# jrectorb/decagon

Measured on AMD Instinct MI355X. Metric: GCN-layer edges/sec + achieved HBM GB/s, 5-relation synthetic, 1/2/4/8 GPU, higher is better.
Workload: dtype f32; 1 GPU; S: main.py 5-relation / 10-matrix synthetic (reference-normalised, 105,974 nnz per relation set), 2 GCN layers d=64/32 + DEDICOM decoder B=512+512; nnz_per_layer_total=105974, parallelism=1 GPU, hipgraph=True, launch=one hipGraph per 30 steps, steps_per_graph=30

## Files before the change

decagon_amd/_lib.py:

```python
from __future__ import annotations

import ctypes
import threading
from pathlib import Path
from ctypes import POINTER, c_float, c_int32, c_int64, c_uint64, c_void_p

from . import _build
from .tuning import knob

DG_OK = 0
DG_EINVAL = -1
DG_EALIGN = -2
DG_ETOOMANY = -3
DG_MAX_GROUPS = 8
DG_STAGED_MAX_CHUNKS = 128
DG_EPI_L2NORM = 1
DG_EPI_RELU = 2
DG_EPI_CHUNK_RELU = 4
ABI_VERSION = 39
DG_HINGE_WS_BYTES = 16 + 4 * 256
DG_RANK_LOGIT, DG_RANK_SIGMOID64, DG_RANK_SIGMOID32 = 0, 1, 2
DG_TOPK_MAX_K, DG_TOPK_UPPER, DG_TOPK_NO_DIAG = 1024, 1, 2
DG_GROUP_SHARED_PATTERN = 1
DG_GROUP_DROPOUT = 2
# ... 35 lines not shown
    _fields_ = [
        ("pairs", c_void_p),
        ("jm", c_void_p),
        ("jmoff", c_void_p),
        ("slab", c_void_p),
        ("x", c_void_p),
        ("out", c_void_p),
        ("x_ld", c_int64),
        ("n_rows", c_int32),
        ("n_cols", c_int32),
        ("n_rels", c_int32),
        ("out_chunk", c_int32),
        ("x_rows", c_int32),
        ("jm_len", c_int32),
        ("chunk_start", c_void_p),
        ("n_chunks", c_int32),
        ("pad", c_int32),
    ]


class DgSegGroup(ctypes.Structure):
    _fields_ = [
        ("rowptr", c_void_p),
        ("seg", c_void_p),
        ("vcol", c_void_p),
        ("val", c_void_p),
        ("slab", c_void_p),
        ("x", c_void_p),
        ("w", c_void_p),
        ("out", c_void_p),
        ("x_ld", c_int64),
        ("n_rows", c_int32),
        ("n_cols", c_int32),
        ("n_chunks", c_int32),
        ("chunk", c_int32),
        ("n_rels", c_int32),
        ("x_rows", c_int32),
    ]


class DgTabDesc(ctypes.Structure):
    _fields_ = [("x", c_void_p), ("w", c_void_p), ("orow", c_void_p), ("cnt", c_int32), ("x_ld", c_int32),
                ("ovf", c_int32), ("role", ctypes.c_uint32), ("wr", ctypes.c_uint32), ("pad", c_int32 * 5)]


class DgWaveTable(ctypes.Structure):
    _fields_ = [("pairs", c_void_p), ("ovf", c_void_p), ("desc", c_void_p), ("n_blocks", c_int32),
                ("nw", c_int32), ("nw_stride", c_int32), ("slot_pairs", c_int32)]


class DgStagedProj(ctypes.Structure):
    _fields_ = [("h", c_void_p), ("w", c_void_p), ("h_ld", c_int64), ("din", c_int32), ("pad", c_int32)]


class DgProj(ctypes.Structure):
    _fields_ = [("w", c_void_p), ("rel_map", c_void_p), ("out", c_void_p), ("n_rels", c_int32),
                ("target", c_int32), ("d_out", c_int32), ("reserved", c_int32)]


class DgFusedTarget(ctypes.Structure):
    _fields_ = [("out", c_void_p), ("n_rows", c_int32), ("g_begin", c_int32), ("g_count", c_int32),
                ("flags", c_int32)]


class DgEpiGroup(ctypes.Structure):
    _fields_ = [("partial", c_void_p), ("sum_out", c_void_p), ("n_chunks", c_int32), ("group_flags", c_int32)]


class DgEpiTarget(ctypes.Structure):
    _fields_ = [
        ("groups", POINTER(DgEpiGroup)),
        ("n_groups", c_int32),
        ("reserved0", c_int32),
        ("out", c_void_p),
        ("n_rows", c_int32),
        ("target_flags", c_int32),
        ("reserved", c_int32 * 2),
    ]


class DgPeerXchg(ctypes.Structure):
    _fields_ = [
        ("delta", c_int64 * DG_PEER_MAX),
        ("flags", c_void_p * DG_PEER_MAX),
        ("state", c_void_p),
        ("timeout_ticks", c_int64),
        ("rank", c_int32),
        ("world", c_int32),
        ("slot", c_int32),
        ("loopback", c_int32),
    ]


class DgGemmDesc(ctypes.Structure):
    _fields_ = [
        ("a", c_void_p),
        ("b", c_void_p),
        ("c", c_void_p),
        ("sa", c_void_p),
        ("sc", c_void_p),
        ("b_map", c_void_p),
        ("a_bs", c_int64),
        ("a_sm", c_int64),
        ("a_sk", c_int64),
        ("b_bs", c_int64),
        ("b_sk", c_int64),
        ("b_sn", c_int64),
        ("c_bs", c_int64),
        ("c_sm", c_int64),
        ("c_sn", c_int64),
        ("m", c_int32),
        ("n", c_int32),
        ("k", c_int32),
        ("batch", c_int32),
        ("reduce", c_int32),
        ("drop_tag", ctypes.c_uint32),
        ("drop_state", c_void_p),
        ("drop_keep", c_float),
        ("reserved", c_int32),
    ]


class DgL2gGroup(ctypes.Structure):
    _fields_ = [("s", c_void_p), ("ds", c_void_p)]


class DgAdamSeg(ctypes.Structure):
    _fields_ = [("param", c_void_p), ("grad", c_void_p), ("m", c_void_p), ("v", c_void_p), ("n", c_int64)]


SIGNATURES = {
    "dg_abi_version": (c_int32, []),
    "dg_spmm_groups_f32": (c_int32, [POINTER(DgRelGroup), c_int32, c_int32, c_void_p]),
    "dg_spmm_groups_lds_f32": (c_int32, [POINTER(DgRelGroup), c_int32, c_int32, c_void_p]),
    "dg_spmm_seg_f32": (c_int32, [POINTER(DgSegGroup), c_int32, c_int32, c_int32, c_void_p]),
    "dg_gcn_fused_seg_f32": (c_int32, [POINTER(DgSegGroup), c_int32, POINTER(DgFusedTarget), c_int32, c_int32,
                                       c_int32, c_void_p]),
    "dg_spmm_csr_f32": (
        c_int32,
        [c_void_p, c_void_p, c_void_p, c_int32, c_int32, c_void_p, c_int64, c_void_p, c_int64, c_int32,
         c_float, c_void_p],
    ),
    "dg_rownorm_l2_f32": (c_int32, [c_void_p, c_void_p, c_int32, c_int32, c_int32, c_void_p]),
    "dg_gcn_fused_f32": (
        c_int32,
        [POINTER(DgRelGroup), c_int32, POINTER(DgFusedTarget), c_int32, POINTER(DgProj), c_int32, c_int32,
         c_int32, c_void_p],
    ),
    "dg_gcn_epilogue_multi_f32": (c_int32, [POINTER(DgEpiTarget), c_int32, c_int32, c_int32, c_void_p]),
    "dg_gcn_epilogue_peer_f32": (c_int32, [POINTER(DgEpiTarget), c_int32, c_int32, c_int32, POINTER(DgPeerXchg),
                                           c_void_p]),
    "dg_gcn_fused_tab_f32": (c_int32, [POINTER(DgWaveTable), c_int32, c_int32, c_void_p]),
    "dg_gcn_fused_tab_post_f32": (c_int32, [POINTER(DgWaveTable), c_int32, c_int32, c_void_p]),
    "dg_gcn_fused_tab_peer_f32": (c_int32, [POINTER(DgWaveTable), c_int32, c_int32, POINTER(DgPeerXchg), c_void_p]),
    "dg_spmm_seg_tab_f32": (c_int32, [POINTER(DgWaveTable), c_int32, c_int32, c_void_p]),
    "dg_gcn_epilogue_tab_f32": (c_int32, [c_void_p, c_int32, c_int32, c_int32, POINTER(DgPeerXchg), c_void_p]),
    "dg_gcn_fused_seg_peer_f32": (c_int32, [POINTER(DgSegGroup), c_int32, POINTER(DgFusedTarget), c_int32, c_int32,
                                            c_int32, POINTER(DgPeerXchg), c_void_p]),
    "dg_peer_alloc": (c_int32, [c_int64, c_int32, POINTER(c_void_p)]),
    "dg_peer_free": (c_int32, [c_void_p]),
    "dg_ipc_get_handle": (c_int32, [c_void_p, c_void_p, POINTER(c_int64)]),
    "dg_ipc_open": (c_int32, [c_void_p, POINTER(c_void_p)]),
    "dg_ipc_close": (c_int32, [c_void_p]),
    "dg_peer_read": (c_int32, [c_void_p, c_void_p, c_int64]),
    "dg_peer_allgather": (c_int32, [POINTER(DgPeerXchg), c_void_p, POINTER(c_int64), POINTER(c_int64), c_int32,
                                    c_void_p]),
    "dg_gcn_epilogue_f32": (
        c_int32,
        [POINTER(DgEpiGroup), c_int32, c_void_p, c_int32, c_int32, c_int32, c_void_p],
    ),
    "dg_gemm_f32": (c_int32, [POINTER(DgGemmDesc), c_int32, c_void_p]),
    "dg_gemm_tn_f32": (c_int32, [c_void_p, c_int64, c_int64, c_void_p, c_int64, c_int64, c_void_p, c_int32,
                                 c_int32, c_int32, c_int32, c_int32, c_void_p, c_void_p]),
    "dg_dropout_rows_f32": (c_int32, [c_void_p, c_void_p, c_int64, c_int32, c_void_p, ctypes.c_uint32, c_float,
                                      c_void_p]),
    "dg_dropout_elems_f32": (c_int32, [c_void_p, c_void_p, c_int32, c_int32, c_int32, c_void_p,
                                       ctypes.c_uint32, c_float, c_void_p]),
    "dg_dropout_rows_map_f32": (c_int32, [c_void_p, c_void_p, c_void_p, c_int32, c_int64, c_int32, c_int32, c_void_p,
                                          ctypes.c_uint32, ctypes.c_float, c_void_p]),
    "dg_dropout_elems_map_f32": (c_int32, [c_void_p, c_void_p, c_void_p, c_int32, c_int32, c_int32, c_void_p,
                                           ctypes.c_uint32, ctypes.c_float, c_void_p]),
    "dg_dropout_advance": (c_int32, [c_void_p, c_void_p]),
    "dg_spmm_staged_f32": (c_int32, [POINTER(DgStagedGroup), c_int32, c_int32, c_void_p]),
    "dg_spmm_staged_proj_f32": (c_int32, [POINTER(DgStagedGroup), POINTER(DgStagedProj), c_int32, c_int32, c_void_p]),
    "dg_staged_block": (c_int32, [c_void_p, c_void_p, c_void_p, c_int32, c_void_p, c_int32, c_void_p]),
    "dg_decoder_score_bf16": (c_int32, [c_void_p, c_int64, c_void_p, c_int64, c_void_p, c_void_p, c_void_p,
                                        c_int32, c_void_p, c_void_p, c_int32, c_void_p, c_void_p]),
    "dg_slot_score_hinge_bf16": (c_int32, [c_void_p, c_int64, c_int64, c_void_p, c_int64, c_int64, c_void_p, c_void_p,
                                           c_void_p, c_int32,
                                           c_int64, c_int32, c_int32, c_int32, c_uint64, c_void_p, c_void_p,
                                           c_int32, c_float, c_void_p, c_void_p, c_void_p, c_void_p, c_void_p]),
    "dg_decoder_score_bf16_paired": (c_int32, [c_void_p, c_int64, c_int64, c_void_p, c_int64, c_int64, c_void_p,
                                               c_void_p, c_void_p, c_int32, c_void_p, c_void_p, c_int32, c_void_p,
                                               c_void_p]),
    "dg_decoder_hinge_f32": (
        c_int32,
        [c_void_p, c_int64, c_void_p, c_int64, c_void_p, c_void_p, c_void_p, c_void_p, c_int32,
         c_uint64, c_uint64, c_int32, c_void_p, c_void_p, c_int32, c_float, c_void_p, c_void_p,
         c_void_p, c_void_p, c_void_p, c_void_p],
    ),
    "dg_decoder_score_f32": (
        c_int32,
        [c_void_p, c_int64, c_void_p, c_int64, c_void_p, c_void_p, c_int32, c_void_p, c_void_p,
         c_int32, c_void_p, c_void_p],
    ),
    "dg_hinge_loss_f32": (c_int32, [c_void_p, c_void_p, c_int32, c_float, c_void_p, c_void_p]),
    "dg_hinge_loss_ws_f32": (c_int32, [c_void_p, c_void_p, c_int32, c_float, c_void_p, c_void_p, c_void_p]),
    "dg_xent_loss_f32": (c_int32, [c_void_p, c_void_p, c_int32, c_float, c_void_p, c_void_p]),
    "dg_decoder_grad_workspace": (c_int64, [c_int32, c_int32]),
    "dg_decoder_grad_f32": (
        c_int32,
        [c_void_p, c_int64, c_void_p, c_int64, c_void_p, c_void_p, c_void_p, c_int32, c_void_p, c_void_p,
         c_void_p, c_void_p, c_int32, c_float, c_void_p, c_void_p, c_void_p, c_void_p, c_void_p, c_void_p,
         c_int64, c_void_p],
    ),
    "dg_scatter_rows_f32": (c_int32, [c_void_p, c_int32, c_void_p, c_int32, c_void_p, c_int64, c_int32,
                                      c_void_p]),
    "dg_l2norm_grad_f32": (c_int32, [POINTER(DgL2gGroup), c_int32, c_void_p, c_void_p, c_int32, c_int32,
                                     c_void_p]),
    "dg_adam_f32": (c_int32, [POINTER(DgAdamSeg), c_int32, c_float, c_float, c_float, c_float, c_void_p,
                              c_void_p]),
    "dg_adam_advance": (c_int32, [c_void_p, c_float, c_float, c_float, c_void_p]),
    "dg_rank_metrics_workspace": (c_int64, [c_int32]),
    "dg_rank_metrics_ex_workspace": (c_int64, [c_int32, c_int32]),
    "dg_rank_metrics_ex_f32": (c_int32, [c_void_p, c_int32, c_void_p, c_int32, c_int32, c_int32, c_void_p, c_void_p,
                                         c_int64, c_void_p]),
    "dg_rank_metrics_f32": (c_int32, [c_void_p, c_int32, c_void_p, c_int32, c_int32, c_void_p, c_void_p, c_int64,
                                      c_void_p]),
    "dg_decoder_topk_workspace": (c_int64, [c_int32, c_int32, c_int32, c_int32]),
    "dg_decoder_topk_f32": (
        c_int32,
        [c_void_p, c_int64, c_int32, c_void_p, c_int64, c_int32, c_void_p, c_int64, c_void_p, c_int64,
         c_int32, c_int32, c_int32, c_void_p, c_void_p, c_int32, c_void_p, c_void_p, c_void_p, c_void_p,
         c_void_p, c_int64, c_void_p],
    ),
    "dg_unigram_sample_slots": (c_int32, [c_void_p, c_int32, c_int64, c_int32, c_int32, c_int32, ctypes.c_uint64,
                                          c_void_p, c_void_p]),
    "dg_unigram_sample": (
        c_int32,
        [c_void_p, c_int32, c_int32, c_uint64, c_uint64, c_void_p, c_void_p],
    ),
}

_LIB = None
_LOAD_LOCK = threading.Lock()


class KernelError(RuntimeError):
    pass


def load(build_if_missing: bool = True) -> ctypes.CDLL:
    global _LIB
    if _LIB is not None:
        return _LIB
    with _LOAD_LOCK:
        if _LIB is None:
            _LIB = _load(build_if_missing)
    return _LIB


def _load(build_if_missing: bool) -> ctypes.CDLL:
    override = knob("DG_LIB", "")
    path = Path(override) if override else _build.lib_path()
    if not override and (not path.exists() or (build_if_missing and _build.needs_build())):
        if not build_if_missing:
            raise ImportError(f"{path} missing: run __graft_entry__.build() or python -m decagon_amd._build")
        _build.build()
    lib = ctypes.CDLL(str(path))
    for name, (res, args) in SIGNATURES.items():
        fn = getattr(lib, name)
        fn.restype = res
        fn.argtypes = args
    got = lib.dg_abi_version()
    if got != ABI_VERSION:
        raise ImportError(f"libdecagon_hip ABI {got} != expected {ABI_VERSION}; rebuild")
    return lib


def check(rc: int, what: str) -> None:
    if rc != DG_OK:
        name = _ERRS.get(rc, f"hipError_t {rc}")
        raise KernelError(f"{what} failed: {name}")
```

decagon_amd/csrc/decoder.hip:

```cpp
#include "common.h"
#include "decoder_tile.h"

namespace {

using dg::DecTab;
using dg::f32x16;
using dg::score_tile;
using dg::splitmix64;
using dg::unigram_draw;

struct DecArgs {
    DecTab t;
    const int32_t* row_idx;
    const int32_t* col_idx;
    float* out;
    int32_t n_pairs;
};

__global__ __launch_bounds__(256) void decoder_score_kernel(const DecArgs a) {
    const int lane = threadIdx.x & 63;
    const int wave = threadIdx.x >> 6;
    const int p0 = (blockIdx.x * 4 + wave) * 32;
    if (p0 >= a.n_pairs) return;
    const int i = lane & 31;
    const int h = lane >> 5;
    const int p = p0 + i;
    const bool valid = p < a.n_pairs;
    float part[16];
    score_tile(a.t, valid ? a.row_idx[p] : 0, valid ? a.col_idx[p] : 0, valid, part);
    if ((i & 1) == 0) {
        const int r = i >> 1;
        const int pp = p0 + (r & 3) + 8 * (r >> 2) + 4 * h;
        if (pp < a.n_pairs) a.out[pp] = part[0];
    }
}

#ifdef DG_DEC_PROF
extern "C" int64_t dg_dec_prof_copy(unsigned long long* host) {
    if (hipDeviceSynchronize() != hipSuccess) return -1;
    if (hipMemcpyFromSymbol(host, HIP_SYMBOL(dg::g_dec_prof), sizeof(dg::g_dec_prof), 0, hipMemcpyDeviceToHost) !=
        hipSuccess)
        return -1;
    return 256;
}
#endif

struct HingeArgs {
    DecTab t;
    const int32_t* rows;
    const int32_t* cols;
    const int32_t* neg_given;
    const uint2* alias;
    float* pos;
    float* neg;
    int32_t* neg_rows_out;
    float* loss;
    float* partial;
    uint32_t* ticket;
    unsigned long long* word;
    uint64_t seed;
    uint64_t offset;
    int32_t range;
    int32_t n;
    float margin;
};

template <bool PACKED>
__global__ __launch_bounds__(128) void decoder_hinge_kernel(const HingeArgs a) {
    __shared__ float sc[2][32];
    __shared__ float red[128];
    __shared__ int last;
    __shared__ unsigned long long total;
    const int lane = threadIdx.x & 63;
    const int side = threadIdx.x >> 6;
    const int i = lane & 31;
    const int h = lane >> 5;
    const int b0 = blockIdx.x * 32;
    const int b = b0 + i;
    const bool valid = b < a.n;
    DG_DEC_STAMP(0);
    int ridx = 0, cidx = 0;
    if (valid) {
        cidx = a.cols[b];
        if (side == 0)
            ridx = a.rows[b];
        else if (a.neg_given)
            ridx = a.neg_given[b];
        else
            ridx = unigram_draw(a.alias, a.range, a.seed, a.offset + (uint64_t)b);
        if (side == 1 && a.neg_rows_out && h == 0) a.neg_rows_out[b] = ridx;
    }
    DG_DEC_STAMP(1);
    float part[16];
    score_tile(a.t, ridx, cidx, valid, part);
    if ((i & 1) == 0) {
        const int r = i >> 1;
        const int q = (r & 3) + 8 * (r >> 2) + 4 * h;
        const float v = (b0 + q < a.n) ? part[0] : 0.f;
        sc[side][q] = v;
        if (b0 + q < a.n) (side == 0 ? a.pos : a.neg)[b0 + q] = v;
    }
    __syncthreads();
    if (threadIdx.x < 64) {
        float term = 0.f;
        if (lane < 32 && b0 + lane < a.n) term = fmaxf(sc[1][lane] - (sc[0][lane] - a.margin), 0.f);
        term = dg::xor_add<1>(dg::xor_add<2>(dg::xor_add<4>(dg::xor_add<8>(dg::xor_add<16>(dg::xor_add<32>(term))))));
        if (lane == 0 && PACKED) {
            unsigned long long add = 1ull << 56;
            if (term < 256.0f) {
                add += static_cast<unsigned long long>(static_cast<double>(term) * 4294967296.0 + 0.5);
            } else {
                __hip_atomic_store(a.partial + blockIdx.x, term, __ATOMIC_RELAXED, __HIP_MEMORY_SCOPE_AGENT);
                asm volatile("s_waitcnt vmcnt(0)" ::: "memory");
                add += 1ull << 48;
            }
            const unsigned long long old =
                __hip_atomic_fetch_add(a.word, add, __ATOMIC_RELAXED, __HIP_MEMORY_SCOPE_AGENT);
            last = (old >> 56) == gridDim.x - 1 ? 1 : 0;
            total = old + add;
        } else if (lane == 0) {
            __hip_atomic_store(a.partial + blockIdx.x, term, __ATOMIC_RELAXED, __HIP_MEMORY_SCOPE_AGENT);
            asm volatile("s_waitcnt vmcnt(0)" ::: "memory");
            const uint32_t t = __hip_atomic_fetch_add(a.ticket, 1u, __ATOMIC_RELAXED, __HIP_MEMORY_SCOPE_AGENT);
            last = (t == gridDim.x - 1) ? 1 : 0;
        }
    }
    __syncthreads();
    DG_DEC_STAMP(5);
    if (!last) return;
    if constexpr (PACKED) {
        if (threadIdx.x == 0) {
            double s = static_cast<double>(total & ((1ull << 48) - 1)) * (1.0 / 4294967296.0);
            if ((total >> 48) & 0xFF) {
                for (int k = 0; k < (int)gridDim.x; ++k) {
                    const float v = __hip_atomic_load(a.partial + k, __ATOMIC_RELAXED, __HIP_MEMORY_SCOPE_AGENT);
                    if (v != 0.f) {
                        s += static_cast<double>(v);
                        __hip_atomic_store(a.partial + k, 0.f, __ATOMIC_RELAXED, __HIP_MEMORY_SCOPE_AGENT);
                    }
                }
            }
            a.loss[0] = static_cast<float>(s);
            __hip_atomic_store(a.word, 0ull, __ATOMIC_RELAXED, __HIP_MEMORY_SCOPE_AGENT);
        }
        DG_DEC_STAMP(6);
        return;
    }
    float s = 0.f;
    for (int k = threadIdx.x; k < (int)gridDim.x; k += 128)
        s += __hip_atomic_load(a.partial + k, __ATOMIC_RELAXED, __HIP_MEMORY_SCOPE_AGENT);
    red[threadIdx.x] = s;
    __syncthreads();
#pragma unroll
    for (int w = 64; w > 0; w >>= 1) {
        if (threadIdx.x < w) red[threadIdx.x] += red[threadIdx.x + w];
        __syncthreads();
    }
    for (int k = threadIdx.x; k < (int)gridDim.x; k += 128) a.partial[k] = 0.f;
    if (threadIdx.x == 0) {
        a.loss[0] = red[0];
        atomicExch(a.ticket, 0u);
    }
}

template <typename F>
__device__ float block_sum_256(int n, F term) {
    __shared__ float red[256];
    float s = 0.f;
    for (int idx = threadIdx.x; idx < n; idx += 256) s += term(idx);
    __syncthreads();
    red[threadIdx.x] = s;
    __syncthreads();
#pragma unroll
    for (int w = 128; w > 0; w >>= 1) {
        if (threadIdx.x < w) red[threadIdx.x] += red[threadIdx.x + w];
        __syncthreads();
    }
    return red[0];
}

__global__ __launch_bounds__(256) void hinge_kernel(const float* pos, const float* neg, int n,
                                                    float margin, float* loss) {
    const float s = block_sum_256(n, [&](int p) { return fmaxf(neg[p] - (pos[p] - margin), 0.f); });
    if (threadIdx.x == 0) loss[0] = s;
}

__global__ __launch_bounds__(256) void hinge_multi_kernel(const float* pos, const float* neg, int n,
                                                          float margin, float* loss, float* partial,
                                                          uint32_t* ticket) {
    __shared__ int last;
    const int chunk = (n + (int)gridDim.x - 1) / (int)gridDim.x;
    const int p0 = blockIdx.x * chunk;
    const int cnt = max(0, min(n, p0 + chunk) - p0);
    const float s = block_sum_256(cnt, [&](int q) {
        return fmaxf(neg[p0 + q] - (pos[p0 + q] - margin), 0.f);
    });
    if (threadIdx.x == 0) {
        __hip_atomic_store(partial + blockIdx.x, s, __ATOMIC_RELAXED, __HIP_MEMORY_SCOPE_AGENT);
        asm volatile("s_waitcnt vmcnt(0)" ::: "memory");
        last = __hip_atomic_fetch_add(ticket, 1u, __ATOMIC_RELAXED, __HIP_MEMORY_SCOPE_AGENT) == gridDim.x - 1;
    }
    __syncthreads();
    if (!last) return;
    const float t = block_sum_256((int)gridDim.x, [&](int b) {
        return __hip_atomic_load(partial + b, __ATOMIC_RELAXED, __HIP_MEMORY_SCOPE_AGENT);
    });
    if (threadIdx.x == 0) {
        loss[0] = t;
        atomicExch(ticket, 0u);
    }
}

__device__ __forceinline__ float softplus_neg_abs(float x) { return (float)log1p((double)expf(-fabsf(x))); }

__global__ __launch_bounds__(256) void xent_kernel(const float* pos, const float* neg, int n,
                                                   float w, float* loss) {
    const float sp = block_sum_256(n, [&](int p) {
        const float x = pos[p];
        return fmaxf(x, 0.f) - x + softplus_neg_abs(x);
    });
    const float sn = block_sum_256(n, [&](int p) {
        const float x = neg[p];
        return fmaxf(x, 0.f) + softplus_neg_abs(x);
    });
    if (threadIdx.x == 0) loss[0] = sp + w * sn;
}

__global__ __launch_bounds__(256) void unigram_sample_kernel(const uint2* table, int range, int n,
                                                             uint64_t seed, uint64_t offset,
                                                             int32_t* out) {
    const int idx = blockIdx.x * 256 + threadIdx.x;
    if (idx >= n) return;
    out[idx] = unigram_draw(table, range, seed, offset + (uint64_t)idx);
}

__global__ __launch_bounds__(256) void unigram_sample_slots_kernel(const uint2* table, int range, int64_t stride,
                                                                   int slot0, int batch, int n, uint64_t seed,
                                                                   int32_t* out) {
    const int idx = blockIdx.x * 256 + threadIdx.x;
    if (idx >= n) return;
    const int slot = slot0 + idx / batch;
    out[idx] = unigram_draw(table + (int64_t)slot * stride, range, seed,
                            (uint64_t)slot0 * (uint64_t)batch + (uint64_t)idx);
}

}

extern "C" int dg_decoder_score_f32(const float* row_table, int64_t ld_row, const float* col_table,
                                    int64_t ld_col, const int32_t* row_idx, const int32_t* col_idx,
                                    int32_t n_pairs, const float* G, const float* l, int32_t d,
                                    float* out, void* stream) {
    if (n_pairs < 0 || d <= 0 || (d % 32) || d > 256) return DG_EINVAL;
    if (n_pairs == 0) return DG_OK;
    if (!row_table || !col_table || !row_idx || !col_idx || !G || !out) return DG_EINVAL;
    if (ld_row < d || ld_col < d) return DG_EINVAL;
    DecArgs a{};
    a.t = DecTab{row_table, col_table, G, l, ld_row, ld_col, d,
                 dg::aligned16(row_table) && (ld_row & 3) == 0 && (!l || dg::aligned16(l))};
    a.row_idx = row_idx;
    a.col_idx = col_idx;
    a.out = out;
    a.n_pairs = n_pairs;
    dim3 grid(dg::ceil_div(n_pairs, 128)), block(256);
    hipLaunchKernelGGL(decoder_score_kernel, grid, block, 0, reinterpret_cast<hipStream_t>(stream), a);
    return dg::launch_status();
}

extern "C" int dg_hinge_loss_f32(const float* pos, const float* neg, int32_t n, float margin,
                                 float* loss, void* stream) {
    if (n < 0 || !loss || (n > 0 && (!pos || !neg))) return DG_EINVAL;
    hipLaunchKernelGGL(hinge_kernel, dim3(1), dim3(256), 0, reinterpret_cast<hipStream_t>(stream),
                       pos, neg, n, margin, loss);
    return dg::launch_status();
}

extern "C" int dg_hinge_loss_ws_f32(const float* pos, const float* neg, int32_t n, float margin,
                                    float* loss, void* workspace, void* stream) {
    if (n < 0 || !loss || !workspace || (n > 0 && (!pos || !neg))) return DG_EINVAL;
    if (!dg::aligned16(workspace)) return DG_EALIGN;
    const int blocks = max(1, min(DG_HINGE_WS_BLOCKS, dg::ceil_div(n, 4096)));
    hipLaunchKernelGGL(hinge_multi_kernel, dim3(blocks), dim3(256), 0, reinterpret_cast<hipStream_t>(stream),
                       pos, neg, n, margin, loss, reinterpret_cast<float*>(workspace) + 4,
                       reinterpret_cast<uint32_t*>(workspace));
    return dg::launch_status();
}

extern "C" int dg_xent_loss_f32(const float* pos, const float* neg, int32_t n, float neg_weight,
                                float* loss, void* stream) {
    if (n < 0 || !loss || (n > 0 && (!pos || !neg))) return DG_EINVAL;
    hipLaunchKernelGGL(xent_kernel, dim3(1), dim3(256), 0, reinterpret_cast<hipStream_t>(stream),
                       pos, neg, n, neg_weight, loss);
    return dg::launch_status();
}

extern "C" int dg_unigram_sample(const uint32_t* alias_table, int32_t range, int32_t n,
                                 uint64_t seed, uint64_t offset, int32_t* out, void* stream) {
    if (range < 1 || n < 0 || !alias_table || (n > 0 && !out)) return DG_EINVAL;
    if (n == 0) return DG_OK;
    hipLaunchKernelGGL(unigram_sample_kernel, dim3(dg::ceil_div(n, 256)), dim3(256), 0,
                       reinterpret_cast<hipStream_t>(stream),
                       reinterpret_cast<const uint2*>(alias_table), range, n, seed, offset, out);
    return dg::launch_status();
}

extern "C" int dg_unigram_sample_slots(const uint32_t* alias_table, int32_t range, int64_t alias_stride,
                                       int32_t slot0, int32_t batch, int32_t n, uint64_t seed, int32_t* out,
                                       void* stream) {
    if (range < 1 || n < 0 || batch < 1 || slot0 < 0 || alias_stride < 0 || !alias_table || (n > 0 && !out))
        return DG_EINVAL;
    if (alias_stride > 0 && alias_stride < range) return DG_EINVAL;
    if (n == 0) return DG_OK;
    hipLaunchKernelGGL(unigram_sample_slots_kernel, dim3(dg::ceil_div(n, 256)), dim3(256), 0,
                       reinterpret_cast<hipStream_t>(stream), reinterpret_cast<const uint2*>(alias_table), range,
                       alias_stride, slot0, batch, n, seed, out);
    return dg::launch_status();
}

extern "C" int dg_decoder_hinge_f32(const float* row_table, int64_t ld_row, const float* col_table,
                                    int64_t ld_col, const int32_t* rows, const int32_t* cols,
                                    const int32_t* neg_rows, const uint32_t* alias_table,
                                    int32_t range, uint64_t seed, uint64_t offset, int32_t n,
                                    const float* G, const float* l, int32_t d, float margin,
                                    float* pos, float* neg, int32_t* neg_rows_out, float* loss,
                                    void* workspace, void* stream) {
    if (n < 1 || d <= 0 || (d % 32) || d > 256) return DG_EINVAL;
    if (!row_table || !col_table || !rows || !cols || !G || !pos || !neg || !loss || !workspace)
        return DG_EINVAL;
    if (!neg_rows && (!alias_table || range < 1)) return DG_EINVAL;
    if (ld_row < d || ld_col < d) return DG_EINVAL;
    if (!dg::aligned16(workspace)) return DG_EALIGN;
    const int blocks = dg::ceil_div(n, 32);
    HingeArgs a{};
    a.t = DecTab{row_table, col_table, G, l, ld_row, ld_col, d,
                 dg::aligned16(row_table) && (ld_row & 3) == 0 && (!l || dg::aligned16(l))};
    a.rows = rows;
    a.cols = cols;
    a.neg_given = neg_rows;
    a.alias = reinterpret_cast<const uint2*>(alias_table);
    a.pos = pos;
    a.neg = neg;
    a.neg_rows_out = neg_rows_out;
    a.loss = loss;
    a.ticket = reinterpret_cast<uint32_t*>(workspace);
    a.word = reinterpret_cast<unsigned long long*>(workspace) + 1;
    a.partial = reinterpret_cast<float*>(workspace) + 4;
    a.seed = seed;
    a.offset = offset;
    a.range = range;
    a.n = n;
    a.margin = margin;
    if (blocks <= 255)
        hipLaunchKernelGGL(decoder_hinge_kernel<true>, dim3(blocks), dim3(128), 0,
                           reinterpret_cast<hipStream_t>(stream), a);
    else
        hipLaunchKernelGGL(decoder_hinge_kernel<false>, dim3(blocks), dim3(128), 0,
                           reinterpret_cast<hipStream_t>(stream), a);
    return dg::launch_status();
}
```

decagon_amd/csrc/segspmm.hip:

```cpp
#include <vector>

#include "common.h"
#include "peer.h"

constexpr int kSegU = 8;
constexpr int kSegUP = 4;
constexpr int kFsegU = 4;
constexpr int kFsegUP = 4;
constexpr int kSegMinNW = 1;
constexpr int kTabU = 4;
constexpr int kTabUP = 4;

namespace {

struct SegGroupK {
    const int32_t* rowptr;
    const int32_t* seg;
    const int32_t* vcol;
    const float* val;
    const int32_t* slab;
    const float* x;
    const float* w;
    float* out;
    int32_t x_ld;
// ... 348 lines not shown
    }
#ifdef DG_FSEG_PROF
    asm volatile("s_waitcnt vmcnt(0)" ::: "memory");
    DG_FS_STAMP(6);
    if (lane == 0 && blockIdx.x < kFsProfMaxBlocks) {
        uint32_t xcc;
        asm volatile("s_getreg_b32 %0, hwreg(HW_REG_XCC_ID)" : "=s"(xcc));
        g_fs_prof[kFsForm][blockIdx.x][wave][7] = xcc;
    }
#endif
    if constexpr (PEER) dg::peer_arrive(a.P);
}

static_assert(sizeof(dg_tab_desc) == 64, "dg_tab_desc: one s_load_dwordx16");
template <bool PROJ, int U, int LP = 16>
__device__ __forceinline__ float4 tab_wave(const dg_tab_desc& D, const uint2 first, const uint2* __restrict__ ovf,
                                           float4* ybuf, const int S) {
    static_assert(LP == 16 || (LP == 8 && !PROJ), "tab_wave: 64-float rows, or 32-float plain sums");
    constexpr int G = dg::kWave / LP;
    [[maybe_unused]] constexpr int kFsForm = 1;
    const int lane = threadIdx.x & 63;
    float4 res = make_float4(0.f, 0.f, 0.f, 0.f);
    if (D.cnt > 0) {
        const float* xq = D.x + (lane % LP) * 4;
        const int sub = lane / LP;
        int vc = (int)first.x;
        int vb = (int)first.y;
        const uint2* nx = ovf + D.ovf;
        float4 acc = make_float4(0.f, 0.f, 0.f, 0.f);
        int bsz = S;
#pragma unroll 1
        for (int base = 0; base < D.cnt; base += bsz, bsz = 64) {
            const int n = min(bsz, D.cnt - base);
            const int eoff = vc * D.x_ld;
            const int vbits = vb;
            vc = 0;
            vb = 0;
            if (base + bsz < D.cnt) {
                const uint2 q = nx[lane];
                vc = (int)q.x;
                vb = (int)q.y;
                nx += 64;
            }
            constexpr int S = dg::kWave / G;
            static_assert(U >= 1 && U <= S && S % U == 0, "tab_wave: the unroll must divide the steps of a batch");
#pragma unroll
            for (int it = 0; it < S / U; ++it) {
                if (it * U * G >= n) break;
                int o[U];
                float w[U];
#pragma unroll
                for (int u = 0; u < U; ++u) {
                    const int m = it * U + u;
                    if constexpr (LP == 16) {
                        o[u] = row_bcast_rt(eoff, m);
                        w[u] = __int_as_float(row_bcast_rt(vbits, m));
                    } else {
                        const bool odd = (lane >> 3) & 1;
                        const int o0 = row_bcast_rt(eoff, m), o1 = row_bcast_rt(eoff, 8 + m);
                        const int w0 = row_bcast_rt(vbits, m), w1 = row_bcast_rt(vbits, 8 + m);
                        o[u] = odd ? o1 : o0;
                        w[u] = __int_as_float(odd ? w1 : w0);
                    }
                }
                float4 xv[U];
#pragma unroll
                for (int u = 0; u < U; ++u) {
                    const bool ok = (it * U + u) * G + sub < n;
                    xv[u] = ok ? *reinterpret_cast<const float4*>(xq + o[u]) : make_float4(0.f, 0.f, 0.f, 0.f);
                    if (!ok) w[u] = 0.f;
                }
#pragma unroll
                for (int u = 0; u < U; ++u) dg::fma4(acc, w[u], xv[u]);
            }
        }
        acc = dg::xor_sum4_from<LP>(acc);
#ifdef DG_FSEG_PROF
        if constexpr (PROJ) {
            asm volatile("s_waitcnt vmcnt(0) lgkmcnt(0)" ::: "memory");
            const int wave = __builtin_amdgcn_readfirstlane(threadIdx.x >> 6);
            DG_FS_STAMP(2);
        }
#endif
        if constexpr (PROJ) {
            const int ms = lane >> 3;
            const float4* w = reinterpret_cast<const float4*>(D.w) + (8 * ms) * 8 + (lane & 7);
            float4 wv[8];
#pragma unroll
            for (int i = 0; i < 8; ++i) wv[i] = w[8 * i];
            if (lane < 16) ybuf[lane] = acc;
            __builtin_amdgcn_wave_barrier();
            const float4 ya = ybuf[2 * ms];
            const float4 yb = ybuf[2 * ms + 1];
            float4 z = make_float4(0.f, 0.f, 0.f, 0.f);
            dg::fma4(z, ya.x, wv[0]);
            dg::fma4(z, ya.y, wv[1]);
            dg::fma4(z, ya.z, wv[2]);
            dg::fma4(z, ya.w, wv[3]);
            dg::fma4(z, yb.x, wv[4]);
            dg::fma4(z, yb.y, wv[5]);
            dg::fma4(z, yb.z, wv[6]);
            dg::fma4(z, yb.w, wv[7]);
            z = dg::xor_sum4_from<8>(z);
            res = z;
        } else {
            res = acc;
        }
    }
    return res;
}

template <int M>
__device__ __forceinline__ float xor_get_any(float x) {
    if constexpr (M == 0) {
        return x;
    } else {
        constexpr int LOW = M & -M;
        return xor_get_any<M - LOW>(dg::xor_get<LOW>(x));
    }
}
template <int M>
__device__ __forceinline__ float4 xor_get4_any(const float4& v) {
    return make_float4(xor_get_any<M>(v.x), xor_get_any<M>(v.y), xor_get_any<M>(v.z), xor_get_any<M>(v.w));
}
template <int W, int V, int SETS>
__device__ __forceinline__ void add_lane_sets(float4& tot, const float4& v, int n) {
    if constexpr (V < SETS) {
        if (V < n) dg::add4(tot, xor_get4_any<W * V>(v));
        add_lane_sets<W, V + 1, SETS>(tot, v, n);
    }
}

template <int W>
__device__ __forceinline__ float4 lds_ordered_sum(const float4 (*rows)[W], int K, int q) {
    float4 s = rows[0][q];
#pragma unroll 1
    for (int u = 1; u < K; ++u) dg::add4(s, rows[u][q]);
    return s;
}

template <int LP = 16>
__device__ __forceinline__ uint32_t slot_lane_offset(int lane, int S) {
    constexpr int G = dg::kWave / LP;
    const int q = S / G, m = lane & (LP - 1);
    return 8u * (uint32_t)((lane / LP) * q + (m < q ? m : q - 1));
}

__device__ __forceinline__ float4 load4_global(const float* p) {
    typedef float v4f __attribute__((ext_vector_type(4)));
    const v4f v = *(const v4f __attribute__((address_space(1)))*)(uintptr_t)p;
    return make_float4(v.x, v.y, v.z, v.w);
}

template <bool PROJ, int NW, bool PEER, int LP = 16, bool POST = false>
__global__ __launch_bounds__(64 * NW) void gcn_tab_kernel(const uint2* __restrict__ pairs,
                                                          const dg_tab_desc* __restrict__ desc,
                                                          const uint2* __restrict__ ovf, const int S,
                                                          const dg::PeerK P) {
    static_assert(LP == 16 || (LP == 8 && !PROJ && !PEER), "gcn_tab_kernel: 32-float rows in the plain one-GPU form");
    static_assert(!POST || (LP == 16 && !PROJ && !PEER), "gcn_tab_kernel: the projecting tail follows a 64 -> 64 layer");
    constexpr int DOUT4 = PROJ ? 8 : LP;
    [[maybe_unused]] constexpr int kFsForm = (PROJ || LP == 8) ? 1 : 0;
    __shared__ float4 ybuf[NW][16];
    __shared__ float4 zbuf[NW][DOUT4];
    __shared__ float4 hbuf[POST ? kFsMaxRpb : 1][16];
    const int lane = threadIdx.x & 63;
    const int wave = __builtin_amdgcn_readfirstlane(threadIdx.x >> 6);
    const int64_t wi = (int64_t)blockIdx.x * NW + wave;
    DG_FS_STAMP(0);
    const dg_tab_desc D = desc[wi];
    uint2 first;
    asm volatile("global_load_dwordx2 %0, %1, %2\n\ts_waitcnt vmcnt(0)"
                 : "=&v"(first) : "v"(slot_lane_offset<LP>(lane, S)), "s"(pairs + wi * S) : "memory");
    asm volatile("" ::"s"(D.x), "s"(D.w), "s"(D.orow), "s"(D.cnt), "s"(D.x_ld), "s"(D.ovf), "s"(D.role), "s"(D.wr),
                 "s"(ovf));
    if constexpr (POST) asm volatile("" ::"s"(D.pad[0]), "s"(D.pad[1]));
#ifdef DG_FSEG_PROF
    asm volatile("s_waitcnt vmcnt(0) lgkmcnt(0)" ::: "memory");
#endif
    DG_FS_STAMP(1);
    if constexpr (!PROJ) DG_FS_STAMP(2);
    const float4 res = tab_wave<PROJ, PROJ ? kTabUP : kTabU, LP>(D, first, ovf, ybuf[wave], S);
    const bool pjob = POST && ((D.role >> 30) & 1u);
    const int ms = lane >> 3;
    float4 wv[POST ? 8 : 1];
    if constexpr (POST) {
        if (pjob) {
            const float* w = D.w + 4 * ((8 * ms) * 8 + (lane & 7));
#pragma unroll
            for (int i = 0; i < 8; ++i) wv[i] = load4_global(w + 4 * 8 * i);
        }
    }
#ifdef DG_FSEG_PROF
    asm volatile("s_waitcnt vmcnt(0) lgkmcnt(0)" ::: "memory");
#endif
    DG_FS_STAMP(3);
    if (lane < DOUT4) zbuf[wave][lane] = res;
    __syncthreads();
    DG_FS_STAMP(4);
    if (D.orow != nullptr) {
        constexpr int SETS = 64 / DOUT4;
        const int gc = D.wr & 0xff;
        const uint32_t kc = (uint32_t)D.pad[2];
        const int u = lane / DOUT4, q = lane % DOUT4;
        int gb = D.pad[3];
#pragma unroll
        for (int v = 0; v + 1 < SETS; ++v)
            if (v < u && v < gc) gb += (int)((kc >> (4 * v)) & 15u) + 1;
        const bool mine = u < gc;
        const int K = mine ? (int)((kc >> (4 * u)) & 15u) + 1 : 1;
        const float4 sum = lds_ordered_sum<DOUT4>(&zbuf[mine ? gb : 0], K, q);
        float ss = sum.x * sum.x + sum.y * sum.y + sum.z * sum.z + sum.w * sum.w;
        ss = dg::xor_sum_below<DOUT4>(ss);
        const float inv = 1.0f / sqrtf(fmaxf(ss, 1e-12f));
        const float4 nv = make_float4(sum.x * inv, sum.y * inv, sum.z * inv, sum.w * inv);
        float4 tot = nv;
        add_lane_sets<DOUT4, 1, SETS>(tot, nv, gc);
        DG_FS_STAMP(5);
        if (lane < DOUT4) {
            if ((D.wr >> 8) & 1) {
                tot.x = fmaxf(tot.x, 0.f);
                tot.y = fmaxf(tot.y, 0.f);
                tot.z = fmaxf(tot.z, 0.f);
                tot.w = fmaxf(tot.w, 0.f);
            }
            reinterpret_cast<float4*>(D.orow)[lane] = tot;
            if constexpr (POST) hbuf[(D.wr >> 16) & (kFsMaxRpb - 1)][lane] = tot;
            if constexpr (PEER)
                dg::peer_store4(P, reinterpret_cast<const float*>(reinterpret_cast<const char*>(D.orow) - D.pad[0]),
                                (uint32_t)D.pad[1], (uint32_t)D.pad[0] + 16u * lane, tot);
        }
    }
    if constexpr (POST) {
        __syncthreads();
        if (pjob) {
            float4* prow = reinterpret_cast<float4*>(((uint64_t)(uint32_t)D.pad[1] << 32) | (uint32_t)D.pad[0]);
            const uint32_t slots = (D.role >> 24) & ((1u << kFsMaxRpb) - 1u);
#pragma unroll
            for (int sl = 0; sl < kFsMaxRpb; ++sl) {
                if (!((slots >> sl) & 1u)) continue;
                const float4 ya = hbuf[sl][2 * ms];
                const float4 yb = hbuf[sl][2 * ms + 1];
                float4 z = make_float4(0.f, 0.f, 0.f, 0.f);
                dg::fma4(z, ya.x, wv[0]);
                dg::fma4(z, ya.y, wv[1]);
                dg::fma4(z, ya.z, wv[2]);
                dg::fma4(z, ya.w, wv[3]);
                dg::fma4(z, yb.x, wv[4]);
                dg::fma4(z, yb.y, wv[5]);
                dg::fma4(z, yb.z, wv[6]);
                dg::fma4(z, yb.w, wv[7]);
                z = dg::xor_sum4_from<8>(z);
                if (lane < 8) prow[8 * sl + lane] = z;
            }
        }
    }
#ifdef DG_FSEG_PROF
    asm volatile("s_waitcnt vmcnt(0)" ::: "memory");
    DG_FS_STAMP(6);
    if (lane == 0 && blockIdx.x < kFsProfMaxBlocks) {
        uint32_t xcc;
        asm volatile("s_getreg_b32 %0, hwreg(HW_REG_XCC_ID)" : "=s"(xcc));
        g_fs_prof[kFsForm][blockIdx.x][wave][7] = xcc;
    }
#endif
    if constexpr (PEER) dg::peer_arrive(P);
}

template <bool PROJ, int NW>
__global__ __launch_bounds__(64 * NW) void seg_tab_kernel(const uint2* __restrict__ pairs,
                                                          const dg_tab_desc* __restrict__ desc,
                                                          const uint2* __restrict__ ovf, const int S) {
    constexpr int DOUT4 = PROJ ? 8 : 16;
    __shared__ float4 ybuf[NW][16];
    __shared__ float4 zbuf[NW][DOUT4];
    const int lane = threadIdx.x & 63;
    const int wave = __builtin_amdgcn_readfirstlane(threadIdx.x >> 6);
    const int64_t wi = (int64_t)blockIdx.x * NW + wave;
    const dg_tab_desc D = desc[wi];
    uint2 first;
    asm volatile("global_load_dwordx2 %0, %1, %2\n\ts_waitcnt vmcnt(0)"
                 : "=&v"(first) : "v"(slot_lane_offset(lane, S)), "s"(pairs + wi * S) : "memory");
    asm volatile("" ::"s"(D.x), "s"(D.w), "s"(D.orow), "s"(D.cnt), "s"(D.x_ld), "s"(D.ovf), "s"(D.role), "s"(ovf));
    const float4 res = tab_wave<PROJ, PROJ ? kSegUP : kSegU>(D, first, ovf, ybuf[wave], S);
    if (lane < DOUT4) zbuf[wave][lane] = res;
    __syncthreads();
    if (D.orow != nullptr && lane < DOUT4) {
        const int K = (D.role >> 8) & 0xff;
        reinterpret_cast<float4*>(D.orow)[lane] = lds_ordered_sum<DOUT4>(&zbuf[wave], K, lane);
    }
}

}

namespace {
int convert_seg(const dg_seg_group& s, bool proj, int d_in, SegGroupK& k, bool& skip) {
    if (s.n_rows < 0 || s.n_chunks < 1 || s.chunk < 1 || s.chunk > 16 || s.n_rels < 0 || s.n_cols < 0 ||
        s.x_rows < 0)
        return DG_EINVAL;
    if ((int64_t)s.n_chunks * s.chunk < s.n_rels || (int64_t)(s.n_chunks - 1) * s.chunk >= s.n_rels)
        return DG_EINVAL;
    if ((s.w != nullptr) != proj) return DG_EINVAL;
    skip = s.n_rows == 0 || s.n_rels == 0;
    if (skip) return DG_OK;
    if (!s.rowptr || !s.seg || !s.x) return DG_EINVAL;
    if (!dg::aligned16(s.x) || (s.x_ld & 3)) return DG_EALIGN;
    if (proj && !dg::aligned16(s.w)) return DG_EALIGN;
    if (s.x_ld < d_in) return DG_EINVAL;
    if ((int64_t)s.x_rows * s.x_ld > 0x7fffffffLL) return DG_EINVAL;
    k = SegGroupK{};
    k.rowptr = s.rowptr;
    k.seg = s.seg;
    k.vcol = s.vcol;
    k.val = s.val;
    k.slab = s.slab;
    k.x = s.x;
    k.w = s.w;
    k.out = s.out;
    k.x_ld = static_cast<int32_t>(s.x_ld);
    k.n_rows = s.n_rows;
    k.n_cols = s.n_cols;
    k.n_chunks = s.n_chunks;
    k.chunk = s.chunk;
    k.n_rels = s.n_rels;
    return DG_OK;
}

int seg_shape(int32_t d_in, int32_t d_out, bool& proj) {
    proj = d_in == 64 && d_out == 32;
    return proj || (d_in == d_out && (d_in == 32 || d_in == 64)) ? DG_OK : DG_EINVAL;
}
}

namespace {
template <int NW>
void launch_seg(bool proj, int d_in, dim3 grid, dim3 block, hipStream_t st, const SegArgs& a) {
    if (proj)
        hipLaunchKernelGGL((spmm_seg_kernel<16, true, NW>), grid, block, 0, st, a);
    else if (d_in == 64)
        hipLaunchKernelGGL((spmm_seg_kernel<16, false, NW>), grid, block, 0, st, a);
    else
        hipLaunchKernelGGL((spmm_seg_kernel<8, false, NW>), grid, block, 0, st, a);
}

template <int NW, bool PEER>
void launch_fs(bool proj, int d_in, dim3 grid, dim3 block, hipStream_t st, const FsArgs& a) {
    if (proj)
        hipLaunchKernelGGL((gcn_fused_seg_kernel<16, true, NW, PEER>), grid, block, 0, st, a);
    else if (d_in == 64)
        hipLaunchKernelGGL((gcn_fused_seg_kernel<16, false, NW, PEER>), grid, block, 0, st, a);
    else
        hipLaunchKernelGGL((gcn_fused_seg_kernel<8, false, NW, PEER>), grid, block, 0, st, a);
}

int seg_launch(const dg_seg_group* groups, int32_t n_groups, int32_t d_in, int32_t d_out, void* stream) {
    if (n_groups < 0 || (n_groups > 0 && groups == nullptr)) return DG_EINVAL;
    if (n_groups > DG_MAX_GROUPS) return DG_ETOOMANY;
    bool proj = false;
    if (seg_shape(d_in, d_out, proj) != DG_OK) return DG_EINVAL;
    SegArgs args{};
    int64_t blocks = 0;
    int ng = 0;
    int nw = kSegMinNW;
    for (int i = 0; i < n_groups; ++i)
        if (groups[i].chunk > nw && groups[i].n_rows > 0 && groups[i].n_rels > 0) nw = groups[i].chunk;
    if (nw > 16) return DG_EINVAL;
    args.nw = nw;
    for (int i = 0; i < n_groups; ++i) {
        const dg_seg_group& s = groups[i];
        bool skip = false;
        const int rc = convert_seg(s, proj, d_in, args.g[ng], skip);
        if (rc != DG_OK) return rc;
        if (skip) continue;
        SegGroupK& k = args.g[ng++];
        if (!s.out) return DG_EINVAL;
        if (!dg::aligned16(s.out)) return DG_EALIGN;
        k.rpb = nw / s.chunk;
        k.row_blocks = dg::ceil_div(s.n_rows, k.rpb);
        const int64_t items = (int64_t)s.n_chunks * k.row_blocks;
        k.n_blocks = static_cast<int32_t>(8 * ((items + 7) / 8));
        k.block_begin = static_cast<int32_t>(blocks);
        blocks += k.n_blocks;
        if (blocks > 0x7fffffff) return DG_EINVAL;
    }
    args.n_groups = ng;
    if (blocks == 0) return DG_OK;
    hipStream_t st = reinterpret_cast<hipStream_t>(stream);
    dim3 grid(static_cast<unsigned>(blocks)), block(64 * nw);
    if (nw <= 8)
        launch_seg<8>(proj, d_in, grid, block, st, args);
    else
        launch_seg<16>(proj, d_in, grid, block, st, args);
    return dg::launch_status();
}

int fused_seg_launch(const dg_seg_group* groups, int32_t n_groups, const dg_fused_target* targets, int32_t n_targets,
                     int32_t d_in, int32_t d_out, const dg_peer_xchg* xchg, void* stream) {
    if (n_groups < 1 || !groups || n_targets < 1 || !targets) return DG_EINVAL;
    if (n_groups > DG_MAX_GROUPS || n_targets > DG_MAX_GROUPS) return DG_ETOOMANY;
    bool proj = false;
    if (seg_shape(d_in, d_out, proj) != DG_OK) return DG_EINVAL;
    FsArgs a{};
    for (int i = 0; i < n_groups; ++i) {
        bool skip = false;
        const int rc = convert_seg(groups[i], proj, d_in, a.g[i], skip);
        if (rc != DG_OK) return rc;
        if (groups[i].n_rels < 1 || groups[i].n_rows < 1) return DG_EINVAL;
    }
    int64_t blocks = 0;
    int nw = 1;
    for (int t = 0; t < n_targets; ++t) {
        const dg_fused_target& s = targets[t];
        if (!s.out || !dg::aligned16(s.out) || s.n_rows < 0 || s.g_count < 1 || s.g_begin < 0 ||
            s.g_begin + s.g_count > n_groups || (s.flags & ~DG_EPI_RELU))
            return DG_EINVAL;
        int items = 0;
        for (int g = s.g_begin; g < s.g_begin + s.g_count; ++g) {
            if (groups[g].n_rows != s.n_rows) return DG_EINVAL;
            items += groups[g].n_rels;
        }
        if (items > 16) return DG_EINVAL;
        const int waves = items;
        nw = waves > nw ? waves : nw;
        FsTargetK& k = a.t[t];
        k.out = s.out;
        k.n_rows = s.n_rows;
        k.g_begin = s.g_begin;
        k.g_count = s.g_count;
        k.relu = (s.flags & DG_EPI_RELU) ? 1 : 0;
        k.waves = waves;
    }
    for (int t = 0; t < n_targets; ++t) {
        FsTargetK& k = a.t[t];
        k.rpb = nw / k.waves < kFsMaxRpb ? nw / k.waves : kFsMaxRpb;
        k.block_begin = static_cast<int32_t>(blocks);
        blocks += dg::ceil_div(k.n_rows, k.rpb);
    }
    if (blocks > 0x7fffffff) return DG_EINVAL;
    a.n_targets = n_targets;
    a.nw = nw;
    if (xchg) {
        const int rc = dg::peer_convert(xchg, a.P);
        if (rc != DG_OK) return rc;
        for (int t = 0; t < n_targets; ++t)
            if ((int64_t)targets[t].n_rows * d_out * 4 > 0x7fffffffLL) return DG_EINVAL;
        if (blocks == 0) blocks = 1;
    }
    if (blocks == 0) return DG_OK;
    hipStream_t st = reinterpret_cast<hipStream_t>(stream);
    dim3 grid(static_cast<unsigned>(blocks)), block(64 * nw);
    if (xchg) {
        if (nw <= 8)
            launch_fs<8, true>(proj, d_in, grid, block, st, a);
        else
            launch_fs<16, true>(proj, d_in, grid, block, st, a);
    } else if (nw <= 8) {
        launch_fs<8, false>(proj, d_in, grid, block, st, a);
    } else {
        launch_fs<16, false>(proj, d_in, grid, block, st, a);
    }
    return dg::launch_status();
}
}

#ifdef DG_FSEG_PROF
extern "C" int64_t dg_fseg_prof_copy(int proj, unsigned long long* host, int64_t max_blocks) {
    const int64_t n = max_blocks < kFsProfMaxBlocks ? max_blocks : kFsProfMaxBlocks;
    if (hipDeviceSynchronize() != hipSuccess) return -1;
    if (hipMemcpyFromSymbol(host, HIP_SYMBOL(g_fs_prof), n * 16 * kFsProfSlots * 8, (size_t)(proj ? 1 : 0) *
                            kFsProfMaxBlocks * 16 * kFsProfSlots * 8, hipMemcpyDeviceToHost) != hipSuccess)
        return -1;
    return n;
}
extern "C" int dg_fseg_prof_clear() {
    static unsigned long long zero[2 * kFsProfMaxBlocks * 16 * kFsProfSlots] = {};
    return hipMemcpyToSymbol(HIP_SYMBOL(g_fs_prof), zero, sizeof(zero)) == hipSuccess ? 0 : -1;
}
#endif

extern "C" int dg_spmm_seg_f32(const dg_seg_group* groups, int32_t n_groups, int32_t d_in, int32_t d_out,
                               void* stream) {
    return seg_launch(groups, n_groups, d_in, d_out, stream);
}

extern "C" int dg_gcn_fused_seg_f32(const dg_seg_group* groups, int32_t n_groups, const dg_fused_target* targets,
                                    int32_t n_targets, int32_t d_in, int32_t d_out, void* stream) {
    return fused_seg_launch(groups, n_groups, targets, n_targets, d_in, d_out, nullptr, stream);
}

namespace {
int fused_tab_launch(const dg_wave_table* t, int32_t d_in, int32_t d_out, const dg_peer_xchg* xchg, bool post,
                     void* stream) {
    if (!t) return DG_EINVAL;
    bool proj = false;
    if (seg_shape(d_in, d_out, proj) != DG_OK) return DG_EINVAL;
    const bool narrow = !proj && d_in == 32;
    if (narrow && xchg) return DG_EINVAL;
    if (post && (xchg || proj || d_in != 64)) return DG_EINVAL;
    if (t->n_blocks < 0 || t->nw < 1 || t->nw > 16 || t->nw_stride != (t->nw <= 8 ? 8 : 16)) return DG_EINVAL;
    if (t->n_blocks == 0) return xchg ? DG_EINVAL : DG_OK;
    if (!t->pairs || !t->desc || !dg::aligned16(t->pairs) || (reinterpret_cast<uintptr_t>(t->desc) & 63))
        return DG_EALIGN;
    const int S = t->slot_pairs ? t->slot_pairs : 64;
    if (S != 16 && S != 32 && S != 48 && S != 64) return DG_EINVAL;
    if ((int64_t)t->n_blocks * t->nw_stride * S > 0x7fffffffLL) return DG_EINVAL;
    dg::PeerK P{};
    if (xchg) {
        const int rc = dg::peer_convert(xchg, P);
        if (rc != DG_OK) return rc;
    }
    const uint2* pr = reinterpret_cast<const uint2*>(t->pairs);
    const uint2* ov = reinterpret_cast<const uint2*>(t->ovf);
    hipStream_t st = reinterpret_cast<hipStream_t>(stream);
    dim3 grid(static_cast<unsigned>(t->n_blocks)), block(64 * t->nw);
#define DG_TAB_LAUNCH(PR, NWV, PE, ...) \
    hipLaunchKernelGGL((gcn_tab_kernel<PR, NWV, PE, ##__VA_ARGS__>), grid, block, 0, st, pr, t->desc, ov, S, P)
    if (narrow) {
        if (t->nw_stride == 8) DG_TAB_LAUNCH(false, 8, false, 8); else DG_TAB_LAUNCH(false, 16, false, 8);
    } else if (post) {
        if (t->nw_stride == 8) DG_TAB_LAUNCH(false, 8, false, 16, true); else DG_TAB_LAUNCH(false, 16, false, 16, true);
    } else if (xchg) {
        if (t->nw_stride == 8) {
            if (proj) DG_TAB_LAUNCH(true, 8, true); else DG_TAB_LAUNCH(false, 8, true);
        } else {
            if (proj) DG_TAB_LAUNCH(true, 16, true); else DG_TAB_LAUNCH(false, 16, true);
        }
    } else {
        if (t->nw_stride == 8) {
            if (proj) DG_TAB_LAUNCH(true, 8, false); else DG_TAB_LAUNCH(false, 8, false);
        } else {
            if (proj) DG_TAB_LAUNCH(true, 16, false); else DG_TAB_LAUNCH(false, 16, false);
        }
    }
#undef DG_TAB_LAUNCH
    return dg::launch_status();
}
}

extern "C" int dg_gcn_fused_tab_f32(const dg_wave_table* t, int32_t d_in, int32_t d_out, void* stream) {
    return fused_tab_launch(t, d_in, d_out, nullptr, false, stream);
}

extern "C" int dg_gcn_fused_tab_post_f32(const dg_wave_table* t, int32_t d_in, int32_t d_out, void* stream) {
    return fused_tab_launch(t, d_in, d_out, nullptr, true, stream);
}

extern "C" int dg_gcn_fused_tab_peer_f32(const dg_wave_table* t, int32_t d_in, int32_t d_out,
                                         const dg_peer_xchg* xchg, void* stream) {
    if (!xchg) return DG_EINVAL;
    return fused_tab_launch(t, d_in, d_out, xchg, false, stream);
}

extern "C" int dg_spmm_seg_tab_f32(const dg_wave_table* t, int32_t d_in, int32_t d_out, void* stream) {
    if (!t) return DG_EINVAL;
    bool proj = false;
    if (seg_shape(d_in, d_out, proj) != DG_OK || (!proj && d_in != 64)) return DG_EINVAL;
    if (t->n_blocks < 0 || t->nw < 1 || t->nw > 16 || t->nw_stride != (t->nw <= 8 ? 8 : 16)) return DG_EINVAL;
    if (t->n_blocks == 0) return DG_OK;
    if (!t->pairs || !t->desc || !dg::aligned16(t->pairs) || (reinterpret_cast<uintptr_t>(t->desc) & 63))
        return DG_EALIGN;
    const int S = t->slot_pairs ? t->slot_pairs : 64;
    if (S != 16 && S != 32 && S != 48 && S != 64) return DG_EINVAL;
    if ((int64_t)t->n_blocks * t->nw_stride * S > 0x7fffffffLL) return DG_EINVAL;
    const uint2* pr = reinterpret_cast<const uint2*>(t->pairs);
    const uint2* ov = reinterpret_cast<const uint2*>(t->ovf);
    hipStream_t st = reinterpret_cast<hipStream_t>(stream);
    dim3 grid(static_cast<unsigned>(t->n_blocks)), block(64 * t->nw);
    if (t->nw_stride == 8) {
        if (proj)
            hipLaunchKernelGGL((seg_tab_kernel<true, 8>), grid, block, 0, st, pr, t->desc, ov, S);
        else
            hipLaunchKernelGGL((seg_tab_kernel<false, 8>), grid, block, 0, st, pr, t->desc, ov, S);
    } else {
        if (proj)
            hipLaunchKernelGGL((seg_tab_kernel<true, 16>), grid, block, 0, st, pr, t->desc, ov, S);
        else
            hipLaunchKernelGGL((seg_tab_kernel<false, 16>), grid, block, 0, st, pr, t->desc, ov, S);
    }
    return dg::launch_status();
}

extern "C" int dg_gcn_fused_seg_peer_f32(const dg_seg_group* groups, int32_t n_groups,
                                         const dg_fused_target* targets, int32_t n_targets, int32_t d_in,
                                         int32_t d_out, const dg_peer_xchg* xchg, void* stream) {
    if (!xchg) return DG_EINVAL;
    return fused_seg_launch(groups, n_groups, targets, n_targets, d_in, d_out, xchg, stream);
}
```

decagon_amd/engine.py:

```python
from __future__ import annotations

import heapq
import math
from dataclasses import dataclass
from typing import Callable, Dict, List, Optional, Sequence, Tuple

import numpy as np
import torch

from . import kernels
from ._lib import DG_EPI_L2NORM, DG_EPI_RELU, DG_MAX_GROUPS
from .sparse import HostCSR, MergedCSR, chunk_segments, merge_chunks, merge_windows, staged_layout
from .tuning import knob

EdgeType = Tuple[int, int]


STAGED_MIN_RELS = knob("DG_STAGED_MIN_RELS", 32)
STAGED_MAX_COLS = 1024
STAGED_MAX_ROWS = 1022
STAGED_BINS = knob("DG_STAGED_BINS", 128)


def drop_tag(layer: int, group: int) -> int:
# ... 229 lines not shown
    rel_map: Optional[torch.Tensor] = None
    staged: bool = False
    out_chunk: int = 1
    var_chunks: Optional[Tuple[np.ndarray, np.ndarray]] = None
    staged_slab: Optional[torch.Tensor] = None
    layout: Optional["kernels.StagedDevice"] = None
    host: Optional[List[HostCSR]] = None
    seg: Optional[torch.Tensor] = None
    seg2: Optional[tuple] = None

    @property
    def n_rels(self) -> int:
        return int(self.rel_ids.shape[0])


class DeviceGraph:

    def __init__(self, edge_types: Dict[EdgeType, int], adj: Dict[EdgeType, Sequence[Optional[HostCSR]]],
                 device: torch.device, local: Optional[Dict[EdgeType, Sequence[int]]] = None,
                 chunk=None, target_waves: int = 32768, d_policy: int = 64,
                 row_block: Optional[Dict[int, Tuple[int, int, int]]] = None, segments: bool = True):
        self.edge_types = dict(edge_types)
        self.device = device
        self.groups: Dict[EdgeType, DeviceGroup] = {}
        self.n_nodes: Dict[int, int] = {}
        self.sharded = local is not None
        self.row_block = dict(row_block or {})
        for et, K in self.edge_types.items():
            rels = list(adj[et])
            if len(rels) != K:
                raise ValueError(f"edge type {et}: {len(rels)} matrices fed, {K} expected")
            known = [r for r in rels if r is not None]
            if not known:
                raise ValueError(f"edge type {et}: no relation given")
            n_r, n_c = known[0].shape
            for t, n in ((et[0], n_r), (et[1], n_c)):
                if self.n_nodes.setdefault(t, n) != n:
                    raise ValueError(f"node type {t}: inconsistent sizes {self.n_nodes[t]} vs {n}")
            ids = np.arange(K, dtype=np.int32) if local is None else np.asarray(local[et], np.int32)
            if any(rels[k] is None for k in ids):
                raise ValueError(f"edge type {et}: a local relation was not given")
            loc = [rels[k] for k in ids]
            if et[0] in self.row_block:
                a, b, _ = self.row_block[et[0]]
                loc = [row_slice(c, a, b) for c in loc]
                n_r = b - a
            nnz = int(sum(c.nnz for c in loc))
            ch = chunk.get(et) if isinstance(chunk, dict) else chunk
            staged = ch is None and stageable(len(loc), n_r, n_c)
            out_chunk = 1
            if staged:
                out_chunk = max(1, -(-len(loc) // STAGED_BINS))
                costs = [c.nnz + STAGED_REL_OVERHEAD for c in loc]
                var, pieces = None, None
                n_top = max(1, STAGED_TARGET_BLOCKS // -(-d_policy // 16))
                if STAGED_VAR:
                    pieces = staged_pieces(loc, costs, n_top, STAGED_PIECE)
                    if len(pieces) == len(loc):
                        pieces = None
                n_v = len(pieces) if pieces is not None else len(loc)
                if STAGED_VAR and n_v <= 65535 and n_v <= 64 * n_top:
                    vcosts = costs if pieces is None else [c.nnz + STAGED_REL_OVERHEAD for _, c in pieces]
                    perm, tops, subs = staged_var_chunks(vcosts, n_top)
                    var = (tops, subs)
                else:
                    pieces = None
                    perm = snake_bins(costs, out_chunk)
                if pieces is None:
                    ids = ids[perm]
                    loc = [loc[i] for i in perm]
                    stage_loc, stage_slab = loc, None
                else:
                    stage_loc = [pieces[i][1] for i in perm]
                    stage_slab = ids[np.asarray([pieces[i][0] for i in perm], np.int64)].astype(np.int32)
                ch = 1
            if ch is None:
                ch = choose_chunk(len(loc), n_r, nnz, d_policy, target_waves)
            windows = (not staged and loc and ch >= len(loc) and n_r >= WINDOW_MIN_ROWS
                       and N_WINDOWS > 1 and (chunk is None))
            if windows:
                m = merge_windows(loc, ids, N_WINDOWS if n_r >= WINDOW_FULL_ROWS else 2 * N_WINDOWS, K)
            elif loc:
                m = merge_chunks(loc, ids, ch, K)
            else:
                m = MergedCSR(np.zeros(n_r + 1, np.int32), np.zeros(0, np.int32), np.zeros(0, np.float32),
                              n_r, n_c, 1, 1, K * n_c)
            g = DeviceGroup(
                et, n_r, n_c, K, ids, m.chunk, m.n_chunks,
                torch.from_numpy(m.rowptr).to(device), torch.from_numpy(m.vcol).to(device),
                torch.from_numpy(m.val).to(device), m.nnz,
                int(m.vcol.max()) if m.nnz else -1)
            if ids.size and not np.array_equal(ids, np.arange(K)):
                g.rel_map = torch.from_numpy(ids).to(device)
            g.staged, g.out_chunk = staged, out_chunk
            if staged:
                g.var_chunks = var
                if stage_slab is not None:
                    g.staged_slab = torch.from_numpy(stage_slab).to(device)
            g.host = loc
            if segments and loc and not staged and not windows and m.chunk <= 16:
                g.seg = torch.from_numpy(chunk_segments(loc, m)).to(device)
            elif windows and et[0] in self.row_block and len(loc) <= 16 and REASSOC_ROWS:
                m2 = merge_chunks(loc, ids, len(loc), K)
                up = lambda a: torch.from_numpy(a).to(device)
                g.seg2 = (up(m2.rowptr), up(m2.vcol), up(m2.val), up(chunk_segments(loc, m2)), m2.chunk, m2.n_chunks,
                          int(m2.vcol.max()) if m2.nnz else -1)
            if staged:
                lay = staged_layout(stage_loc, kernels.staged_block,
                                    lanes=knob("DG_STAGED_LANES", 1024),
                                    split=knob("DG_STAGED_SPLIT", True))
                g.layout = kernels.StagedDevice.upload(lay, device)
            self.groups[et] = g

    @property
    def total_nnz(self) -> int:
        return sum(g.nnz for g in self.groups.values())


@dataclass
class LayerWeights:

    stacks: Dict[EdgeType, torch.Tensor]


class ForwardPlan:

    FUSED_PROJ_MAX_RELS = knob("DG_FUSED_PROJ_MAX", 64)

    def __init__(self, dgraph: DeviceGraph, features: Dict[int, Optional[HostCSR]],
                 w1: LayerWeights, w2: LayerWeights, h1: int, h2: int,
                 allreduce: Optional[Callable[[torch.Tensor], None]] = None, keep_sums: bool = False,
                 dropout: Optional[Tuple[float, torch.Tensor]] = None, shard=None):
        self.g = dgraph
        self.h1, self.h2 = h1, h2
        self.shard = shard
        if shard is not None:
            allreduce = shard.allreduce
        self.allreduce = allreduce
        self.row_block = dict(dgraph.row_block)
        self.world = shard.world_size if shard is not None else 1
        self.allgather = shard.allgather if shard is not None else None
        if self.row_block and (shard is None or shard.row_block != self.row_block
                               or (self.allgather is None and getattr(shard, "peer", None) is None)):
            raise ValueError("a row-split device graph needs its RelationShard (with an all-gather or a peer exchange)")
        if shard is not None and allreduce is None:
            raise ValueError("a RelationShard needs its all-reduce")
        self.keep, self.drop_state = 1.0, None
        if dropout is not None and float(dropout[0]) < 1.0:
            self.keep, self.drop_state = float(dropout[0]), dropout[1]
        self.flat_mode = allreduce is not None or keep_sums
        self.keep_sums = keep_sums
        self.sums_mode = False
        self.launch_groups: Dict[int, List[EdgeType]] = {}
        dev = dgraph.device
        f32 = dict(device=dev, dtype=torch.float32)
        self.edge_types = list(dgraph.edge_types)
        self.targets: Dict[int, List[EdgeType]] = {}
        for et in self.edge_types:
            self.targets.setdefault(et[0], []).append(et)
        if any(len(v) > DG_MAX_GROUPS for v in self.targets.values()):
            raise ValueError(f"more than {DG_MAX_GROUPS} edge types into one node type")
        if keep_sums and allreduce is None:
            self.flat_mode = False
            if not self._fused_targets():
                self.sums_mode = True
            else:
                self.flat_mode = True
        n = dgraph.n_nodes
        self.seg_mode = (shard is not None and getattr(shard, "seg_rows", False) and not keep_sums
                         and self.drop_state is None and h1 == 64 and h2 == 32
                         and all(et[0] in self.row_block for et in self.edge_types)
                         and all(g.seg is not None or not g.n_rels for g in dgraph.groups.values()))

        self._pre: List[Callable[[], None]] = []
        x1: Dict[EdgeType, torch.Tensor] = {}
        self.et_index = {et: n for n, et in enumerate(self.edge_types)}
        if self.drop_state is not None:
            self._pre.append(lambda st=self.drop_state: kernels.dropout_advance(st))
        for et in self.edge_types:
            i, j = et
            grp = dgraph.groups[et]
            W = w1.stacks[et]
            K, F, dh = W.shape
            if dh != h1 or K != grp.K:
                raise ValueError(f"layer-1 weights of {et} are {tuple(W.shape)}, expected ({grp.K}, *, {h1})")
            fj = features.get(j)
            if fj is None:
                if F != n[j]:
                    raise ValueError(f"identity features of type {j} need {n[j]} weight rows, got {F}")
                x1[et] = W
                if self.drop_state is not None:
                    xd = torch.empty_like(W)
                    t = drop_tag(1, self.et_index[et])
                    if grp.rel_map is None:
                        self._pre.append(lambda W=W, xd=xd, t=t: kernels.dropout_rows(W, xd, self.drop_state, t,
                                                                                      self.keep))
                    elif grp.n_rels:
                        self._pre.append(lambda W=W, xd=xd, t=t, m=grp.rel_map, F=F, mx=int(grp.rel_ids.max()):
                                         kernels.dropout_rows_map(W, xd, m, F, self.drop_state, t, self.keep, True,
                                                                  True, rel_map_max=mx))
                    x1[et] = xd
                continue
            if fj.shape[0] != n[j] or fj.shape[1] != F:
                raise ValueError(f"features of type {j} have shape {fj.shape}, weights expect (*, {F})")
            xw = torch.empty((K, n[j], h1), **f32)
            drop = (None if self.drop_state is None
                    else (self.drop_state, drop_tag(1, self.et_index[et]), self.keep))
            spec = kernels.RelGroupSpec(torch.from_numpy(fj.rowptr).to(dev), torch.from_numpy(fj.col).to(dev),
                                        torch.from_numpy(fj.val).to(dev), W, xw, n[j], K, h1, F,
                                        vcol_max=int(fj.col.max()) if fj.nnz else -1, shared=True, drop=drop)
            self._pre.append(kernels.PreparedSpmm([spec], h1))
            x1[et] = xw

        self._pad: Dict[Tuple[int, int], torch.Tensor] = {}
        self.xregion: Optional[torch.Tensor] = None
        self.peer = None
        split_nodes = [i for i in self.targets if i in self.row_block]
        pc = getattr(shard, "peer", None)
        self.peer_reduce = (pc is not None and pc.mode == "fused" and self.flat_mode and not keep_sums
                            and self.drop_state is None and bool(split_nodes) and not self.seg_mode
                            and not self._fused_targets() and self._peer_reduce_fits(dgraph, split_nodes))
        self._red_slots: Dict[Tuple[int, EdgeType], torch.Tensor] = {}
        if split_nodes:
            layout, off = {}, 0
            for layer, d in ((1, h1), (2, h2)):
                for i in split_nodes:
                    nb = self.world * self.row_block[i][2] * d
                    layout[i, layer] = (off, nb, d)
                    off += -(-nb // 64) * 64
            red_layout = {}
            if self.peer_reduce:
                for layer, d in ((1, h1), (2, h2)):
                    red = [et for et in self.edge_types if et[0] not in self.row_block]
                    per = sum(n[et[0]] * d for et in red)
                    per = -(-per // 64) * 64
                    o2 = 0
                    for et in red:
                        red_layout[layer, et] = (off, o2, per, n[et[0]], d)
                        o2 += n[et[0]] * d
                    off += self.world * per
            if pc is not None and pc.region_kind:
                from .peer import device_tensor

                self.xregion = device_tensor(max(off, 64), pc.region_kind, dev)
            else:
                self.xregion = torch.zeros(max(off, 64), **f32)
            for (i, layer), (o, nb, d) in layout.items():
                self._pad[i, layer] = self.xregion[o:o + nb].view(-1, d)
            for key, (base, o2, per, rows, d) in red_layout.items():
                self._red_slots[key] = torch.as_strided(self.xregion, (self.world, rows, d), (per, d, 1),
                                                        base + o2)
            if pc is not None:
                from .peer import PeerExchange

                self.peer = PeerExchange(self.xregion, shard.rank, self.world, pc)

        def out_buf(i, d, layer):
            if i not in self.row_block:
                return torch.empty((n[i], d), **f32)
            return self._pad[i, layer][:n[i]]

        self.hidden1 = {i: out_buf(i, h1, 1) for i in self.targets}
        self.embeddings = {i: out_buf(i, h2, 2) for i in self.targets}

        self.staged_proj = {et for et in self.edge_types
                            if dgraph.groups[et].staged and dgraph.groups[et].n_rels and h1 == 64
                            and self.drop_state is None and STAGED_PROJ}
        self.fused_seg = (FUSED_SEG and not self.flat_mode and not self.row_block and self.drop_state is None
                          and h1 == 64 and h2 == 32
                          and all(g.seg is not None and g.n_chunks == 1 and g.chunk == g.n_rels >= 1
                                  and not g.staged for g in dgraph.groups.values())
                          and all(sum(dgraph.groups[et].n_rels for et in ets) <= 16
                                  for ets in self.targets.values()))
        self.preproj = set(self.edge_types) if self._preproject_fits(keep_sums) else set()
        self.seg_proj = {et for et in self.edge_types
                         if (self.seg_mode or self.fused_seg) and dgraph.groups[et].n_rels and h1 == 64 and h2 == 32
                         and et not in self.preproj}
        self.seg_proj |= {et for et in self.edge_types
                          if REASSOC_ROWS and shard is not None and not keep_sums and self.drop_state is None
                          and h1 == 64 and h2 == 32 and dgraph.groups[et].n_rels and not dgraph.groups[et].staged
                          and (dgraph.groups[et].seg is not None or dgraph.groups[et].seg2 is not None)}
        self.seg_l1 = {et for et in self.edge_types
                       if SEG_ROWS_L1 and shard is not None and not self.seg_mode and not keep_sums
                       and self.drop_state is None and h1 in (32, 64) and et[0] in self.row_block
                       and dgraph.groups[et].n_rels and not dgraph.groups[et].staged
                       and dgraph.groups[et].seg is not None}
        self.proj: Dict[EdgeType, torch.Tensor] = {}
        for et in self.edge_types:
            grp = dgraph.groups[et]
            K, din, dout = w2.stacks[et].shape
            if din != h1 or dout != h2 or K != grp.K:
                raise ValueError(f"layer-2 weights of {et} are {(K, din, dout)}, expected ({grp.K}, {h1}, {h2})")
            if et[1] not in self.hidden1:
                raise ValueError(f"node type {et[1]} has no incoming edge type; layer 2 needs hidden1[{et[1]}]")
            if et not in self.staged_proj and et not in self.seg_proj:
                self.proj[et] = torch.empty((K, n[et[1]], h2), **f32)

        self.side_stream = (torch.cuda.Stream(dev) if dev.type == "cuda" and CONCURRENT_LAUNCHES else None)

        self.fused = list(self.targets) if self.fused_seg else self._fused_targets()
        rels_from: Dict[int, int] = {}
        for et in self.edge_types:
            rels_from[et[1]] = rels_from.get(et[1], 0) + dgraph.groups[et].n_rels
        finished = (set(self.targets) - set(self.row_block)) if self.flat_mode else set(self.fused)
        proj_fused = [et for et in self.edge_types
                      if dgraph.groups[et].n_rels and et[1] in finished and et not in self.staged_proj
                      and et not in self.seg_proj and et not in self.preproj
                      and rels_from[et[1]] <= self.FUSED_PROJ_MAX_RELS and self.drop_state is None]
        if len(proj_fused) > DG_MAX_GROUPS:
            proj_fused = []
        projs = []
        for et in proj_fused:
            grp = dgraph.groups[et]
            projs.append((et[1], kernels.ProjSpec(
                w2.stacks[et], self.proj[et], grp.n_rels, -1, rel_map=grp.rel_map,
                rel_map_max=int(grp.rel_ids.max()) if grp.rel_map is not None else None)))
        self._layer1 = self._build_layer(x1, h1, True, f32, projs,
                                         post={et: w2.stacks[et] for et in self.edge_types if et in self.preproj})

        gemms, drops = [], []
        self.hdrop: Dict[EdgeType, torch.Tensor] = {}
        for et in self.edge_types:
            grp = dgraph.groups[et]
            if not grp.n_rels or et in proj_fused or et in self.staged_proj or et in self.seg_proj \
                    or et in self.preproj:
                continue
            j = et[1]
            W = w2.stacks[et]
            if self.drop_state is not None:
                hd = torch.empty((grp.n_rels, n[j], h1), **f32)
                self.hdrop[et] = hd
                t = drop_tag(2, self.et_index[et])
                sids = np.sort(grp.rel_ids).astype(np.int32)
                smap = None if np.array_equal(sids, np.arange(grp.K)) else torch.from_numpy(sids).to(dev)
                if smap is None:
                    drops.append(lambda j=j, hd=hd, t=t: kernels.dropout_elems(self.hidden1[j], hd, self.drop_state,
                                                                               t, self.keep))
                else:
                    drops.append(lambda j=j, hd=hd, t=t, m=smap, mx=int(sids.max()): kernels.dropout_elems_map(
                        self.hidden1[j], hd, m, self.drop_state, t, self.keep, rel_map_max=mx))
                gemms.append(kernels.PreparedGemm(
                    hd, (n[j] * h1, h1, 1), W, (h1 * h2, h2, 1), self.proj[et], (n[j] * h2, h2, 1),
                    n[j], h2, h1, grp.n_rels, b_map=smap, b_batches=W.shape[0],
                    b_map_max=int(sids.max()) if smap is not None else None))
                continue
            gemms.append(kernels.PreparedGemm(
                self.hidden1[j], (0, h1, 1), W, (h1 * h2, h2, 1), self.proj[et], (n[j] * h2, h2, 1),
                n[j], h2, h1, grp.n_rels, b_map=grp.rel_map, b_batches=W.shape[0],
                b_map_max=int(grp.rel_ids.max()) if grp.rel_map is not None else None))
        self._gemm2 = drops + [kernels.PreparedGemmMulti(gemms[s:s + DG_MAX_GROUPS])
                               for s in range(0, len(gemms), DG_MAX_GROUPS)]
        self._layer2 = self._build_layer(self.proj, h2, False, f32,
                                         staged_proj={et: (self.hidden1[et[1]], w2.stacks[et])
                                                      for et in self.staged_proj},
                                         seg_w={et: (self.hidden1[et[1]], w2.stacks[et]) for et in self.seg_proj})

    def _fused_targets(self) -> List[int]:
        if self.flat_mode and (self.keep_sums or not self.row_block
                               or not getattr(self.shard, "fused_rows", False)):
            return []

        def rows(i):
            if i in self.row_block:
                return self.row_block[i][1] - self.row_block[i][0]
            return self.g.n_nodes[i]

        return [i for i, ets in self.targets.items()
                if (not self.flat_mode or i in self.row_block)
                and 0 < rows(i) <= FUSED_MAX_ROWS
                and all(self.g.groups[et].n_chunks == 1 and self.g.groups[et].n_rels > 0
                        and not self.g.groups[et].staged for et in ets)]

    def _preproject_fits(self, keep_sums: bool) -> bool:
        if not (L2_PREPROJECT and self.fused_seg and WAVE_TABLE and not keep_sums and self.drop_state is None
                and self.shard is None):
            return False
        order = list(self.targets)
        if any(et[1] not in self.targets for et in self.edge_types):
            return False
        if any(len(self.targets[i]) > 64 // (self.h1 // 4) for i in order):
            return False
        rels = {et: self.g.groups[et].n_rels for et in self.edge_types}
        waves_t = [sum(rels[et] for et in self.targets[i]) for i in order]
        sourced_t = [sum(k for et, k in rels.items() if et[1] == i) for i in order]
        return kernels.tab_proj_fit(waves_t, sourced_t, _tab_balance(self.h1, self.h1), L2_PREPROJECT_SHARE)

    def _spec(self, et, x: torch.Tensor, out, d) -> kernels.RelGroupSpec:
        grp = self.g.groups[et]
        return kernels.RelGroupSpec(grp.rowptr, grp.vcol, grp.val, x, out, grp.n_rows, grp.n_chunks, d,
                                    grp.K * grp.n_cols, vcol_max=grp.vcol_max)

    def _seg_spec(self, et, x: torch.Tensor, out=None, w=None) -> kernels.SegSpec:
        grp = self.g.groups[et]
        if grp.seg is None and grp.seg2 is not None:
            rp, vc, vv, sg, ch, nc, vmax = grp.seg2
        else:
            rp, vc, vv, sg, ch, nc, vmax = grp.rowptr, grp.vcol, grp.val, grp.seg, grp.chunk, grp.n_chunks, grp.vcol_max
        return kernels.SegSpec(rp, sg, vc, vv, x, out, grp.n_rows, grp.n_cols, nc, ch, grp.n_rels, x.stride(-2),
                               grp.K * grp.n_cols, vcol_max=vmax, w=w, slab=grp.rel_map,
                               slab_max=int(grp.rel_ids.max()) if grp.n_rels else -1)

    def _seg_chunks(self, et) -> int:
        grp = self.g.groups[et]
        return grp.seg2[5] if (grp.seg is None and grp.seg2 is not None) else grp.n_chunks

    def _build_layer(self, xs: Dict[EdgeType, torch.Tensor], d, relu, f32, projs=(), staged_proj=None, seg_w=None,
                     post=None):
        g = self.g
        n = g.n_nodes
        outs = self.hidden1 if relu else self.embeddings
        launches: List[Callable[[], None]] = []
        fused_t = self.fused
        gathers = []
        if self.seg_mode and SEG_FUSED and all(sum(g.groups[et].n_rels for et in ets) <= SEG_FUSED_MAX_ITEMS
                                               for ets in self.targets.values()):
            seg_w = seg_w or {}
            tgts = []
            for i in self.targets:
                a, b, blk = self.row_block[i]
                pad = self._pad[i, 1 if relu else 2]
                r0 = self.shard.rank * blk
                gathers.append((pad, pad[r0:r0 + blk]))
                tgts.append((pad[r0:r0 + (b - a)], b - a,
                             [self._seg_spec(et, seg_w[et][0], None, seg_w[et][1]) if et in seg_w
                              else self._seg_spec(et, xs[et]) for et in self.targets[i]], relu))
            fused_peer = self._peer_fused(relu)
            d_in = self.h1 if seg_w else d
            if WAVE_TABLE and d_in == 64 and (d == 64 or seg_w) and _tab_groups_fit(tgts, d):
                launches.append(kernels.PreparedFusedTab(tgts, d_in, d, peer=fused_peer, balance=False))
            else:
                launches.append(kernels.PreparedFusedSeg(tgts, d_in, d, peer=fused_peer))
            self.launch_groups[id(launches[-1])] = [et for i in self.targets for et in self.targets[i]]
            if fused_peer is not None:
                gathers = []
            return _Layer(launches, None, False, self.allreduce, [], [], {}, self.side_stream, None, (), gathers,
                          self.allgather, self._peer_gather_all(gathers, relu))
        if self.fused_seg:
            seg_w = seg_w or {}
            tgts = [(outs[i], n[i], [self._seg_spec(et, seg_w[et][0], None, seg_w[et][1]) if et in seg_w
                                     else self._seg_spec(et, xs[et]) for et in self.targets[i]], relu)
                    for i in fused_t]
            d_in = self.h1 if seg_w else d
            if WAVE_TABLE and d_in == 64 and (d == 64 or seg_w) and _tab_groups_fit(tgts, d):
                pj = []
                for et, W2 in (post or {}).items():
                    grp = g.groups[et]
                    pj.append(kernels.TabProjSpec(fused_t.index(et[1]), W2, self.proj[et], grp.n_rels,
                                                  None if grp.rel_map is None else grp.rel_map.cpu().numpy()))
                launches.append(kernels.PreparedFusedTab(tgts, d_in, d, balance=_tab_balance(d_in, d), projs=pj,
                                                         share_proj=L2_PREPROJECT_SHARE))
            elif WAVE_TABLE and self.preproj and d_in == d == 32 and _tab_groups_fit(tgts, d):
                launches.append(kernels.PreparedFusedTab(tgts, d_in, d, balance=_tab_balance(d_in, d)))
            else:
                launches.append(kernels.PreparedFusedSeg(tgts, d_in, d))
            self.launch_groups[id(launches[-1])] = [et for i in fused_t for et in self.targets[i]]
        elif fused_t:
            avg = max(g.groups[et].nnz / max(1, g.groups[et].n_rows) for i in fused_t for et in self.targets[i])
            max_groups = max(len(self.targets[i]) for i in fused_t)
            rows = sum(g.groups[self.targets[i][0]].n_rows for i in fused_t)
            cap = 16 // max_groups if self.row_block else 2
            wpg = 1 if rows >= 4096 else int(max(1, min(cap, 16 // max_groups, math.ceil(avg / 64.0))))
            if knob("DG_WPG", 0):
                wpg = max(1, min(knob("DG_WPG", 0), 16 // max_groups))
            pspecs = []
            for tgt_node, pj in projs:
                if tgt_node in fused_t:
                    pj.target = fused_t.index(tgt_node)
                    pspecs.append(pj)
            tgts = []
            for i in fused_t:
                out, rows_i = outs[i], n[i]
                if i in self.row_block:
                    a, b, blk = self.row_block[i]
                    pad = self._pad[i, 1 if relu else 2]
                    r0 = self.shard.rank * blk
                    out, rows_i = pad[r0:r0 + (b - a)], b - a
                    gathers.append((pad, pad[r0:r0 + blk]))
                tgts.append((out, rows_i, [self._spec(et, xs[et], None, d) for et in self.targets[i]], relu))
            launches.append(kernels.PreparedFused(tgts, d, pspecs, wpg))
            self.launch_groups[id(launches[-1])] = [et for i in fused_t for et in self.targets[i]]
        rest = [et for et in self.edge_types if et[0] not in fused_t]
        flags = DG_EPI_L2NORM | (DG_EPI_RELU if relu else 0)
        split_t = [i for i in self.targets if i in self.row_block and i not in fused_t]
        red = [et for et in rest if et[0] not in self.row_block]
        flat, views, send, sviews = None, {}, None, {}
        layer_no = 1 if relu else 2
        peer_red = self.peer_reduce and bool(red) and bool(split_t)
        if peer_red:
            for et in red:
                sviews[et] = self._red_slots[layer_no, et][self.shard.rank]
        elif self.flat_mode and red:
            sizes = [g.groups[et].n_rows * d for et in red]
            flat = torch.zeros(int(sum(sizes)), **f32)
            send = torch.zeros_like(flat) if self.allreduce is not None else flat
            off = 0
            for et, sz in zip(red, sizes):
                views[et] = flat[off:off + sz]
                sviews[et] = send[off:off + sz]
                off += sz
        partials, specs, staged, reduces, segs = {}, [], [], [], []
        reassoc = (set(seg_w or {}) | (self.seg_l1 if relu else set())) if not self.seg_mode else set()
        for et in rest:
            grp = g.groups[et]
            cst = staged_chunk_starts(grp, d) if grp.staged else None
            n_out = ((len(cst) - 1 if cst is not None else -(-_staged_n(grp) // staged_out_chunk(grp, d)))
                     if grp.staged else grp.n_chunks)
            if et in reassoc:
                n_out = self._seg_chunks(et)
            if flat is not None and et in views and n_out == 1:
                part = sviews[et]
            else:
                part = torch.zeros((max(1, n_out), grp.n_rows, d), **f32)
                if flat is not None and et in views and grp.n_rels:
                    reduces.append(kernels.PreparedEpilogue([(part, n_out)], sviews[et], grp.n_rows, d, 0))
            partials[et] = (part, max(1, n_out))
            if not grp.n_rels:
                continue
            if grp.staged:
                sp = (staged_proj or {}).get(et)
                staged.append(kernels.StagedSpec(
                    grp.layout, grp.staged_slab if grp.staged_slab is not None else grp.rel_map, xs.get(et), part, staged_out_chunk(grp, d), d, grp.K * grp.n_cols,
                    slab_max=int(grp.rel_ids.max()), proj=sp, chunk_start=cst))
            elif self.seg_mode or et in reassoc:
                if et in (seg_w or {}):
                    segs.append(self._seg_spec(et, seg_w[et][0], part, seg_w[et][1]))
                else:
                    segs.append(self._seg_spec(et, xs[et], part))
            else:
                specs.append(self._spec(et, xs[et], part, d))
        spmm_ets = [et for et in rest if g.groups[et].n_rels and not g.groups[et].staged
                    and not (self.seg_mode or et in reassoc)]
        seg_ets = [et for et in rest if g.groups[et].n_rels and not g.groups[et].staged
                   and (self.seg_mode or et in reassoc)]
        if segs:
            d_in = self.h1 if seg_w else d
            for s in range(0, len(segs), DG_MAX_GROUPS):
                part = segs[s:s + DG_MAX_GROUPS]
                if WAVE_TABLE and kernels._tab_shape(d_in, d, part):
                    launches.append(kernels.PreparedSegTab(part, d_in, d))
                else:
                    launches.append(kernels.PreparedSeg(part, d_in, d))
                self.launch_groups[id(launches[-1])] = seg_ets[s:s + DG_MAX_GROUPS]
        staged_ets = [et for et in rest if g.groups[et].n_rels and g.groups[et].staged]
        for s in range(0, len(staged), DG_MAX_GROUPS):
            launches.append(kernels.PreparedStaged(staged[s:s + DG_MAX_GROUPS], d))
            self.launch_groups[id(launches[-1])] = staged_ets[s:s + DG_MAX_GROUPS]
        for s in range(0, len(specs), DG_MAX_GROUPS):
            launches.append(kernels.PreparedSpmm(specs[s:s + DG_MAX_GROUPS], d))
            self.launch_groups[id(launches[-1])] = spmm_ets[s:s + DG_MAX_GROUPS]
        need_zero = send is flat and flat is not None and any(g.groups[et].n_rels == 0 for et in red)
        epis, local_epis = [], []
        epi_peer = self._peer_fused(relu) if split_t else None
        if split_t:
            blocks = []
            for i in split_t:
                a, b, blk = self.row_block[i]
                pad = self._pad[i, 1 if relu else 2]
                r0 = self.shard.rank * blk
                parts = [partials[et] for et in self.targets[i]]
                if self.keep_sums:
                    for n_, et in enumerate(self.targets[i]):
                        views[et] = torch.empty((b - a) * d, **f32)
                        parts[n_] = (parts[n_][0], parts[n_][1], views[et])
                blocks.append((parts, pad[r0:r0 + (b - a)], b - a))
                if epi_peer is None:
                    gathers.append((pad, pad[r0:r0 + blk]))
            n_push = len(blocks)
            if peer_red:
                red_t = [i for i in self.targets if i not in self.row_block
                         and any(g.groups[et].n_rels for et in self.targets[i])]
            else:
                red_t = [i for i in self.targets if i not in self.row_block
                         and any(et in views and g.groups[et].n_rels and partials[et][1] > 1
                                 for et in self.targets[i])]
            n_groups = sum(len(self.targets[i]) for i in split_t + red_t)
            fits = len(split_t) + len(red_t) <= 8 and n_groups <= DG_MAX_GROUPS
            assert fits or not peer_red
            if (reduces or peer_red) and fits:
                for i in red_t:
                    grp_parts = []
                    for et in self.targets[i]:
                        part, nc = partials[et][:2]
                        if peer_red:
                            grp_parts.append((part, nc, sviews[et] if g.groups[et].n_rels else None, True))
                            continue
                        reduced = et in views and g.groups[et].n_rels and nc > 1
                        grp_parts.append((part, nc, sviews[et] if reduced else None))
                    blocks.append((grp_parts, torch.empty((n[i], d), **f32), n[i]))
                reduces = []
            local_epis.append(_epilogue(blocks, d, flags, peer=epi_peer, push=[t < n_push for t in range(len(blocks))]))
        launches += reduces
        if peer_red:
            tl = [i for i in self.targets if i not in self.row_block]
            pspecs = []
            for tgt_node, pj in projs:
                pj.target = tl.index(tgt_node)
                pspecs.append(pj)

            def slots_spec(i, et):
                sl = self._red_slots[layer_no, et]
                per = sl.stride(0)
                x = torch.as_strided(self.xregion, ((self.world - 1) * per + n[i] * d,), (1,), sl.storage_offset())
                return kernels.RelGroupSpec(None, None, None, x, None, n[i], self.world, d, per // d, dense=True)

            epis.append(kernels.PreparedFused(
                [(outs[i], n[i], [slots_spec(i, et) for et in self.targets[i]], relu) for i in tl], d, pspecs, 1))
        elif flat is not None:
            tl = [i for i in self.targets if i not in self.row_block]
            pspecs = []
            for tgt_node, pj in projs:
                pj.target = tl.index(tgt_node)
                pspecs.append(pj)
            epis.append(kernels.PreparedFused(
                [(outs[i], n[i], [self._identity_spec(i, views[et], d) for et in self.targets[i]], relu)
                 for i in tl], d, pspecs, 1))
        elif not split_t:
            if self.sums_mode:
                for et in rest:
                    views[et] = torch.empty(g.groups[et].n_rows * d, **f32)
                    partials[et] = partials[et] + (views[et],)
            tl = [i for i in self.targets if i not in fused_t]
            tl.sort(key=lambda i: -sum(partials[et][1] for et in self.targets[i]))
            if tl:
                epis.append(_epilogue([([partials[et] for et in self.targets[i]], outs[i], n[i]) for i in tl], d, flags))
        return _Layer(launches, flat, need_zero, self.allreduce, epis, fused_t, views, self.side_stream, send,
                      local_epis, gathers, self.allgather, self._peer_gather_all(gathers, relu))

    def _peer_reduce_fits(self, dgraph, split_nodes) -> bool:
        red_t = [i for i in self.targets if i not in self.row_block
                 and any(dgraph.groups[et].n_rels for et in self.targets[i])]
        t = list(split_nodes) + red_t
        return len(t) <= 8 and sum(len(self.targets[i]) for i in t) <= DG_MAX_GROUPS

    def _peer_fused(self, layer1: bool):
        if self.peer is None or self.peer.cfg.mode != "fused":
            return None
        from .peer import SLOT_FUSED

        return self.peer, SLOT_FUSED + (0 if layer1 else 1)

    def _peer_gather_all(self, gathers, layer1: bool):
        if self.peer is None or not gathers:
            return None
        from .peer import SLOT_KERNEL

        return self.peer.allgather_fn([blk for _, blk in gathers], SLOT_KERNEL + (0 if layer1 else 1))

    def peer_probe(self):
        from .peer import SLOT_PROBE

        out = []
        for layer in (1, 2):
            blks = [self._pad[i, layer][self.shard.rank * self.row_block[i][2]:
                                        (self.shard.rank + 1) * self.row_block[i][2]]
                    for i in self.targets if i in self.row_block]
            if blks:
                out.append(self.peer.allgather_fn(blks, SLOT_PROBE + layer - 1))
        return out

    def _identity_spec(self, i: int, x: torch.Tensor, d: int) -> kernels.RelGroupSpec:
        n_i = self.g.n_nodes[i]
        return kernels.RelGroupSpec(None, None, None, x, None, n_i, 1, d, n_i, dense=True)

    def run_layer1(self) -> None:
        for p in self._pre:
            p()
        self._layer1.run()

    def run_layer2(self) -> None:
        for gm in self._gemm2:
            gm()
        self._layer2.run()

    def run(self) -> None:
        if self.peer is not None:
            self.peer.ensure_ok()
        self.run_layer1()
        self.run_layer2()

    def phases(self) -> List[Tuple[str, Callable[[], None]]]:
        out: List[Tuple[str, Callable[[], None]]] = []
        cur: List[Callable[[], None]] = []

        def close():
            if cur:
                fns = list(cur)
                out.append(("compute", lambda: [f() for f in fns]))
                cur.clear()

        cur.extend(self._pre)
        for layer, before in ((self._layer1, []), (self._layer2, self._gemm2)):
            cur.extend(before)
            if layer.need_zero:
                cur.append(layer.flat.zero_)
            cur.append(layer.run_spmm)
            cur.extend(layer.local_epilogues)
            if layer.has_exchange:
                close()
                out.append(("exchange", layer.exchange))
            cur.extend(layer.epilogues)
        close()
        return out

    def parallelism(self, backend: str = "nccl") -> str:
        return "1 GPU" if self.shard is None else self.shard.describe(backend)

    @property
    def spmm_launches(self):
        kinds = (kernels.PreparedSpmm, kernels.PreparedFused, kernels.PreparedStaged, kernels.PreparedSeg,
                 kernels.PreparedFusedSeg)
        pick = lambda L: [l for l in L.launches if isinstance(l, kinds)]
        return pick(self._layer1), pick(self._layer2)

    def _out_rows(self, i: int) -> int:
        if i in self.row_block:
            return self.row_block[i][1] - self.row_block[i][0]
        return self.g.n_nodes[i]

    def group_bytes(self, et: EdgeType, d: int, fused: bool, layer: int = 1) -> int:
        grp = self.g.groups[et]
        if not grp.n_rels:
            return 0
        tot = 4 * (grp.n_rels * grp.n_rows + 1) + 8 * grp.nnz
        if layer == 2 and (et in self.staged_proj or et in self.seg_proj):
            tot += 4 * self.h1 * (grp.n_cols + d * grp.n_rels)
        else:
            tot += 4 * d * grp.n_cols * grp.n_rels
        return tot if fused else tot + 4 * d * grp.n_rows

    def launch_bytes(self, launch, layer: int) -> int:
        L = self._layer1 if layer == 1 else self._layer2
        d = self.h1 if layer == 1 else self.h2
        ets = self.launch_groups.get(id(launch), [])
        fused = isinstance(launch, (kernels.PreparedFused, kernels.PreparedFusedSeg))
        tot = sum(self.group_bytes(et, d, fused, layer) for et in ets)
        if fused:
            tot += sum(4 * d * self._out_rows(i) for i in L.fused_targets)
            if layer == 1 and isinstance(launch, kernels.PreparedFused):
                for pj in launch._keep[2]:
                    K, din, dout = pj.w.shape
                    tot += 4 * pj.n_rels * (din * dout + pj.out.shape[1] * dout)
            if layer == 1:
                tot += self._post_bytes(launch)
        return tot

    @staticmethod
    def _post_bytes(launch) -> int:
        tot = 0
        for pj in getattr(launch, "projs", ()):
            K, din, dout = pj.w.shape
            tot += 4 * pj.n_rels * (din * dout + pj.out.shape[1] * dout)
        return tot

    def layer_bytes(self, layer: int) -> int:
        L = self._layer1 if layer == 1 else self._layer2
        d = self.h1 if layer == 1 else self.h2
        tot = 0
        for et, grp in self.g.groups.items():
            if not grp.n_rels:
                continue
            tot += 4 * (grp.n_rels * grp.n_rows + 1) + 8 * grp.nnz
            if layer == 2 and (et in self.staged_proj or et in self.seg_proj):
                tot += 4 * self.h1 * (grp.n_cols + d * grp.n_rels)
            else:
                tot += 4 * d * grp.n_cols * grp.n_rels
            if et[0] not in L.fused_targets:
                tot += 4 * d * grp.n_rows
        for i in L.fused_targets:
            tot += 4 * d * self._out_rows(i)
        if layer == 1:
            for f in L.launches:
                if isinstance(f, kernels.PreparedFused):
                    for pj in f._keep[2]:
                        K, din, dout = pj.w.shape
                        rows = pj.out.shape[1]
                        tot += 4 * pj.n_rels * (din * dout + rows * dout)
                tot += self._post_bytes(f)
        return tot


class _Layer:

    def __init__(self, launches, flat, need_zero, allreduce, epilogues, fused_targets, views=None,
                 side_stream=None, send=None, local_epilogues=(), gathers=(), allgather=None, gather_all=None):
        self.launches = launches
        self.side_stream = side_stream
        self.flat = flat
        self.send = flat if send is None else send
        self.views = views or {}
        self.need_zero = need_zero
        self.allreduce = allreduce
        self.epilogues = epilogues
        self.fused_targets = fused_targets
        self.local_epilogues = list(local_epilogues)
        self.gathers = list(gathers)
        self.allgather = allgather
        self.gather_all = gather_all

    @property
    def has_exchange(self) -> bool:
        return (self.flat is not None and self.allreduce is not None) or bool(self.gathers)

    def exchange(self) -> None:
        if self.flat is not None and self.allreduce is not None:
            self.allreduce(self.send, self.flat)
        if self.gather_all is not None:
            self.gather_all()
            return
        for out, blk in self.gathers:
            self.allgather(out, blk)

    def run(self) -> None:
        if self.need_zero:
            self.flat.zero_()
        self.run_spmm()
        for e in self.local_epilogues:
            e()
        if self.has_exchange:
            self.exchange()
        for e in self.epilogues:
            e()

    def run_spmm(self) -> None:
        side = [l for l in self.launches if isinstance(l, kernels.PreparedSpmm)]
        main = [l for l in self.launches if not isinstance(l, kernels.PreparedSpmm)]
        if (self.side_stream is not None and side
                and any(isinstance(l, kernels.PreparedStaged) for l in main)):
            cur = torch.cuda.current_stream()
            self.side_stream.wait_stream(cur)
            if STAGED_FIRST:
                for l in main:
                    if not isinstance(l, kernels.PreparedEpilogue):
                        l()
            with torch.cuda.stream(self.side_stream):
                for l in side:
                    l()
            if not STAGED_FIRST:
                for l in main:
                    if not isinstance(l, kernels.PreparedEpilogue):
                        l()
            cur.wait_stream(self.side_stream)
            for l in main:
                if isinstance(l, kernels.PreparedEpilogue):
                    l()
        else:
            for l in self.launches:
                l()
```

decagon_amd/kernels.py:

```python
from __future__ import annotations

import ctypes
from dataclasses import dataclass
from typing import List, Optional, Sequence, Tuple

import numpy as np
import torch

from . import _lib
from .tuning import knob
from ._lib import (DgAdamSeg, DgEpiGroup, DgFusedTarget, DgGemmDesc, DgL2gGroup, DgProj, DgRelGroup,
                   DgStagedGroup, DgStagedProj, check)


def _stream_ptr(stream: Optional[torch.cuda.Stream] = None) -> int:
    s = torch.cuda.current_stream() if stream is None else stream
    return s.cuda_stream


def _dev(t: torch.Tensor, dtype: torch.dtype, what: str) -> torch.Tensor:
    if not isinstance(t, torch.Tensor):
        raise TypeError(f"{what}: expected a torch.Tensor, got {type(t).__name__}")
    if not t.is_cuda:
        raise ValueError(f"{what}: must be a device (HIP) tensor")
# ... 246 lines not shown
            tarr[t].out, tarr[t].n_rows = out.data_ptr(), n_rows
            tarr[t].g_begin, tarr[t].g_count = len(specs), len(gspecs)
            tarr[t].flags = _lib.DG_EPI_RELU if relu else 0
            for s in gspecs:
                if s.n_rows != n_rows or s.n_rels < 1:
                    raise ValueError("fused seg groups: the target's rows, at least one relation")
                specs.append(s)
        if len(targets) > _lib.DG_MAX_GROUPS:
            raise ValueError(f"at most {_lib.DG_MAX_GROUPS} targets per launch")
        self._garr = _seg_array(specs, d_in, d_out, False)
        self._keep = (specs, [t[0] for t in targets])
        self._tarr, self._ng, self._nt, self.d_in, self.d_out = tarr, len(specs), len(targets), d_in, d_out
        self._xchg = None
        if peer is not None:
            ex, slot = peer
            for out, *_ in targets:
                ex.offset(out)
            self._xchg = ctypes.byref(ex.xchg(slot))
            self._keep = self._keep + (ex,)
            self._fn = _lib.load().dg_gcn_fused_seg_peer_f32
        else:
            self._fn = _lib.load().dg_gcn_fused_seg_f32

    def __call__(self, stream=None) -> None:
        if self._xchg is not None:
            check(self._fn(self._garr, self._ng, self._tarr, self._nt, self.d_in, self.d_out, self._xchg,
                           _stream_ptr(stream)), "dg_gcn_fused_seg_peer_f32")
            return
        check(self._fn(self._garr, self._ng, self._tarr, self._nt, self.d_in, self.d_out, _stream_ptr(stream)),
              "dg_gcn_fused_seg_f32")


class _WaveTable:

    SLOT_COVER = 0.97

    DESC = np.dtype([("x", "<u8"), ("w", "<u8"), ("orow", "<u8"), ("cnt", "<i4"), ("x_ld", "<i4"), ("ovf", "<i4"),
                     ("role", "<u4"), ("wr", "<u4"), ("pad", "<i4", 5)])

    def __init__(self, specs: Sequence[SegSpec], n_slots: int, proj: bool, lp: int = 16):
        assert self.DESC.itemsize == 64 and lp in (8, 16) and not (proj and lp == 8)
        self.specs, self.proj = list(specs), proj
        self.G = 64 // lp
        self.host = [(s.rowptr.cpu().numpy(), s.seg.cpu().numpy(), s.vcol.cpu().numpy(), s.val.cpu().numpy(),
                      None if s.slab is None else s.slab.cpu().numpy()) for s in specs]
        self.n_slots = n_slots
        self.pv: dict = {}
        self.desc = np.zeros(n_slots, self.DESC)
        m = np.arange(64)
        self.lane_of = (64 // self.G) * (m % self.G) + m // self.G

    def bounds(self, g: int, k: int, r: int) -> Tuple[int, int]:
        s = self.specs[g]
        rowptr, seg = self.host[g][:2]
        c, t = divmod(k, s.chunk)
        si = (c * s.n_rows + r) * s.chunk + t
        beg = int(seg[si])
        end = int(seg[si + 1]) if t + 1 < s.chunk else int(rowptr[c * s.n_rows + r + 1])
        return beg, end

    def seg_len(self, g: int, k: int, r: int) -> int:
        beg, end = self.bounds(g, k, r)
        return end - beg

    def relation(self, i: int, g: int, k: int, r: int) -> None:
        beg, end = self.bounds(g, k, r)
        self.wave(i, g, r, [(k, 0, end - beg)])

    def wave(self, i: int, g: int, r: int, pieces) -> None:
        s = self.specs[g]
        vcol, val, slab = self.host[g][2:]
        d = self.desc
        vcs, vvs = [], []
        for k, a, b in pieces:
            beg, _ = self.bounds(g, k, r)
            vc = vcol[beg + a:beg + b].astype(np.int64)
            if self.proj:
                sl = int(slab[k]) if slab is not None else k
                vc = vc - sl * s.n_cols
                d["w"][i] = s.w.data_ptr() + sl * 64 * 32 * 4
            vcs.append(vc)
            vvs.append(val[beg + a:beg + b])
        if self.proj and len({k for k, _, _ in pieces}) > 1:
            raise ValueError("a reassociated wave gathers one relation")
        vc = np.concatenate(vcs) if vcs else np.zeros(0, np.int64)
        vv = np.concatenate(vvs) if vvs else np.zeros(0, np.float32)
        cnt = len(vc)
        d["x"][i], d["x_ld"][i], d["cnt"][i] = s.x.data_ptr(), s.x_ld, cnt
        self.pv[i] = np.stack([vc.astype(np.int32), vv.astype(np.float32).view(np.int32)], 1)

    def slot_pairs(self) -> int:
        fixed = knob("DG_TAB_SLOT", 0)
        if fixed:
            if fixed not in (16, 32, 48, 64):
                raise ValueError("DG_TAB_SLOT: 16, 32, 48 or 64")
            return fixed
        cnts = np.array([len(p) for p in self.pv.values() if len(p)], np.int64)
        if not len(cnts):
            return 16
        need = float(np.quantile(cnts, self.SLOT_COVER))
        return next(S for S in (16, 32, 48, 64) if S >= need or S == 64)

    def layout(self, S: int):
        pairs = np.zeros((self.n_slots * S, 2), np.int32)
        ovf: List[np.ndarray] = []
        n_ovf = 0
        m = np.arange(S)
        compact = (m % self.G) * (S // self.G) + m // self.G
        for i, pv in self.pv.items():
            cnt = len(pv)
            m0 = min(cnt, S)
            pairs[i * S + compact[:m0]] = pv[:m0]
            if cnt > S:
                self.desc["ovf"][i] = n_ovf
                for q0 in range(S, cnt, 64):
                    blk = np.zeros((64, 2), np.int32)
                    n = min(64, cnt - q0)
                    blk[self.lane_of[:n]] = pv[q0:q0 + n]
                    ovf.append(blk)
                    n_ovf += 64
        return pairs, (np.concatenate(ovf) if ovf else np.zeros((64, 2), np.int32))

    def upload(self, owner, n_blocks: int, nw: int, stride: int, dev) -> "_lib.DgWaveTable":
        S = self.slot_pairs()
        pairs, ovf = self.layout(S)
        owner._pairs = torch.from_numpy(pairs).to(dev)
        owner._ovf = torch.from_numpy(ovf).to(dev)
        owner.slot_pairs = S
        raw = torch.from_numpy(self.desc.view(np.uint8).copy())
        owner._desc = torch.empty(raw.numel() + 64, dtype=torch.uint8, device=dev)
        off = (-owner._desc.data_ptr()) % 64
        owner._desc_v = owner._desc[off:off + raw.numel()]
        owner._desc_v.copy_(raw.to(dev))
        tab = _lib.DgWaveTable()
        tab.pairs, tab.ovf, tab.desc = owner._pairs.data_ptr(), owner._ovf.data_ptr(), owner._desc_v.data_ptr()
        tab.n_blocks, tab.nw, tab.nw_stride, tab.slot_pairs = n_blocks, nw, stride, S
        return tab


def _tab_shape(d_in: int, d_out: int, specs) -> bool:
    return d_in == 64 and (d_out == 64 or (d_out == 32 and all(s.w is not None for s in specs)))


@dataclass
class TabProjSpec:

    target: int
    w: torch.Tensor
    out: torch.Tensor
    n_rels: int
    slab: Optional[Sequence[int]] = None


def _tab_geometry(waves_t: Sequence[int], balance: bool) -> Tuple[int, int, List[int]]:
    nw = max([1] + list(waves_t))
    stride = 8 if nw <= 8 else 16
    if balance:
        nw = stride
    return nw, stride, [min(nw // max(1, w), 4) for w in waves_t]


def _proj_jobs(rows_present: Sequence[bool], n_rels: int, nw: int, share: bool = False):
    rpb = len(rows_present)
    if (n_rels if share else rpb * n_rels) > nw:
        return None
    jobs: List[Optional[Tuple[Tuple[int, ...], int]]] = [None] * nw
    order = list(range(rpb, nw)) + list(range(min(rpb, nw)))
    present = tuple(slot for slot in range(rpb) if rows_present[slot])
    if share:
        todo = [(present, k) for k in range(n_rels)] if present else []
    else:
        todo = [((slot,), k) for slot in present for k in range(n_rels)]
    for w, job in zip(order, todo):
        jobs[w] = job
    return jobs


def tab_proj_fit(waves_t: Sequence[int], sourced_t: Sequence[int], balance: bool, share: bool = False) -> bool:
    nw, _, rpbs = _tab_geometry(waves_t, balance)
    return all(_proj_jobs([True] * rpb, k, nw, share) is not None for rpb, k in zip(rpbs, sourced_t))


class PreparedFusedTab(PreparedFusedSeg):

    def __init__(self, targets, d_in: int, d_out: int, peer=None, balance: bool = False,
                 projs: Sequence[TabProjSpec] = (), share_proj: bool = True):
        super().__init__(targets, d_in, d_out, peer=peer)
        specs = self._keep[0]
        narrow = d_in == d_out == 32 and all(s.w is None for s in specs) and peer is None
        if not (_tab_shape(d_in, d_out, specs) or narrow):
            raise ValueError("dg_gcn_fused_tab_f32: d_in = d_out = 64, 64 -> 32 with weight stacks, or "
                             "d_in = d_out = 32 without an exchange")
        proj = d_out != d_in
        if any(len(gs) > 64 // (d_out // 4) for _, _, gs, _ in targets):
            raise ValueError("dg_gcn_fused_tab_f32: at most 64 / (d_out / 4) groups a target (one lane set each)")
        self.projs = list(projs)
        if self.projs and (d_in != 64 or d_out != 64 or peer is not None):
            raise ValueError("dg_gcn_fused_tab_post_f32: projection jobs follow a 64 -> 64 layer without an exchange")
        for pj in self.projs:
            _dev(pj.w, torch.float32, "w")
            _dev(pj.out, torch.float32, "P")
            K, rows = pj.w.shape[0], targets[pj.target][1]
            slabs = list(range(pj.n_rels)) if pj.slab is None else [int(x) for x in pj.slab[:pj.n_rels]]
            if (tuple(pj.w.shape[1:]) != (64, 32) or tuple(pj.out.shape) != (K, rows, 32) or len(slabs) != pj.n_rels
                    or any(not 0 <= x < K for x in slabs) or pj.out.data_ptr() % 16 or pj.w.data_ptr() % 16):
                raise ValueError("projection jobs: w [K, 64, 32], P [K, target rows, 32], slabs inside both")
        waves_t = [sum(s.n_rels for s in gs) for _, _, gs, _ in targets]
        nw, stride, rpbs = _tab_geometry(waves_t, balance)
        self.balance = balance
        plan = []
        for t, (_, n_rows, _, _) in enumerate(targets):
            rpb = rpbs[t]
            plan += [(t, r0, rpb) for r0 in range(0, n_rows, rpb)]
        tb = _WaveTable(specs, len(plan) * stride, proj, lp=d_in // 4)
        g_first = np.cumsum([0] + [len(gs) for _, _, gs, _ in targets])
        for b, (t, r0, rpb) in enumerate(plan):
            out, n_rows, gspecs, relu = targets[t]
            gc = len(gspecs)
            nr = [s.n_rels for s in gspecs]
            per_row = nw // rpb if balance else waves_t[t]
            counts = [[1] * gc for _ in range(rpb)]
            for slot in range(rpb):
                r = r0 + slot
                if r >= n_rows:
                    continue
                gs = [int(g_first[t]) + gl for gl in range(gc)]
                if balance:
                    waves = _balanced_waves(tb, gs, nr, r, per_row, proj)
                else:
                    waves = [[[(k, 0, None)] for k in range(nr[gl])] for gl in range(gc)]
                counts[slot] = [len(wg) for wg in waves]
                w = slot * per_row
                for gl, wg in enumerate(waves):
                    for pieces in wg:
                        tb.wave(b * stride + w, gs[gl], r,
                                [(k, a, e if e is not None else tb.seg_len(gs[gl], k, r)) for k, a, e in pieces])
                        w += 1
            for w in range(nw):
                i = b * stride + w
                if w < rpb * gc:
                    s2, gg = divmod(w, gc)
                    gb = s2 * per_row + sum(counts[s2][:gg])
                    tb.desc["role"][i] = ((1 << 31) | ((s2 * DG_MAX_GROUPS_TAB + gg) << 16) | (counts[s2][gg] << 8)
                                          | gb)
                if w < rpb and r0 + w < n_rows:
                    tb.desc["orow"][i] = out.data_ptr() + (r0 + w) * d_out * 4
                    tb.desc["wr"][i] = gc | ((1 if relu else 0) << 8) | (w << 16)
                    tb.desc["pad"][i, 0] = (r0 + w) * d_out * 4
                    tb.desc["pad"][i, 1] = n_rows * d_out * 4
                    tb.desc["pad"][i, 2] = np.int32(np.uint32(sum((c - 1) << (4 * u)
                                                                  for u, c in enumerate(counts[w]))))
                    tb.desc["pad"][i, 3] = w * per_row
            rels = [(pj, k) for pj in self.projs if pj.target == t for k in range(pj.n_rels)]
            if rels:
                jobs = _proj_jobs([r0 + slot < n_rows for slot in range(rpb)], len(rels), nw, share_proj)
                if jobs is None:
                    raise ValueError(f"{rpb} rows x {len(rels)} projection jobs for {nw} wave slots")
                for w, job in enumerate(jobs):
                    if job is None:
                        continue
                    slots, (pj, k) = job[0], rels[job[1]]
                    sl = k if pj.slab is None else int(pj.slab[k])
                    i = b * stride + w
                    addr = pj.out.data_ptr() + (sl * n_rows + r0) * 32 * 4
                    tb.desc["role"][i] |= np.uint32((1 << 30) | (sum(1 << x for x in slots) << 24))
                    tb.desc["w"][i] = pj.w.data_ptr() + sl * 64 * 32 * 4
                    tb.desc["pad"][i, 0] = np.uint32(addr & 0xffffffff).astype(np.int32)
                    tb.desc["pad"][i, 1] = np.uint32(addr >> 32).astype(np.int32)
        if not plan and peer is not None:
            raise ValueError("dg_gcn_fused_tab_peer_f32: the exchange needs at least one row a rank")
        self._tab = tb.upload(self, len(plan), nw, stride, specs[0].x.device)
        self.n_blocks, self.nw = len(plan), nw
        if self._xchg is not None:
            self._tfn, self._tname = _lib.load().dg_gcn_fused_tab_peer_f32, "dg_gcn_fused_tab_peer_f32"
        elif self.projs:
            self._keep = self._keep + (self.projs,)
            self._tfn, self._tname = _lib.load().dg_gcn_fused_tab_post_f32, "dg_gcn_fused_tab_post_f32"
        else:
            self._tfn, self._tname = _lib.load().dg_gcn_fused_tab_f32, "dg_gcn_fused_tab_f32"

    def __call__(self, stream=None) -> None:
        if self._xchg is not None:
            check(self._tfn(ctypes.byref(self._tab), self.d_in, self.d_out, self._xchg, _stream_ptr(stream)),
                  self._tname)
        else:
            check(self._tfn(ctypes.byref(self._tab), self.d_in, self.d_out, _stream_ptr(stream)), self._tname)

    def seg_form(self, stream=None) -> None:
        PreparedFusedSeg.__call__(self, stream)


def _split_even(n: int, parts: int) -> List[Tuple[int, int]]:
    q, rem = divmod(n, parts)
    out, a = [], 0
    for p in range(parts):
        e = a + q + (1 if p < rem else 0)
        out.append((a, e))
        a = e
    return out


def _balanced_waves(tb: "_WaveTable", gs, nr, r: int, slots: int, proj: bool):
    if proj:
        jobs = [(gl, k) for gl in range(len(gs)) for k in range(nr[gl])]
        sizes = [tb.seg_len(gs[gl], k, r) for gl, k in jobs]
    else:
        jobs = [(gl, None) for gl in range(len(gs))]
        sizes = [sum(tb.seg_len(gs[gl], k, r) for k in range(nr[gl])) for gl in range(len(gs))]
    if len(jobs) > slots:
        raise ValueError(f"{len(jobs)} jobs for {slots} wave slots")
    parts = [1] * len(jobs)
    for _ in range(slots - len(jobs)):
        j = max(range(len(jobs)), key=lambda x: (-(-sizes[x] // parts[x]), -x))
        if sizes[j] <= parts[j]:
            break
        parts[j] += 1
    waves = [[] for _ in gs]
    for (gl, k), n, p in zip(jobs, sizes, parts):
        if k is not None:
            waves[gl] += [[(k, a, e)] for a, e in _split_even(n, p)]
            continue
        lens = [tb.seg_len(gs[gl], kk, r) for kk in range(nr[gl])]
        starts = np.cumsum([0] + lens)
        for a, e in _split_even(n, p):
            pieces = []
            for kk in range(nr[gl]):
                lo, hi = max(a, starts[kk]), min(e, starts[kk + 1])
                if lo < hi:
                    pieces.append((kk, int(lo - starts[kk]), int(hi - starts[kk])))
            waves[gl].append(pieces)
    return waves


class PreparedSegTab(PreparedSeg):

    def __init__(self, specs: Sequence[SegSpec], d_in: int, d_out: int):
        super().__init__(specs, d_in, d_out)
        if not _tab_shape(d_in, d_out, specs):
            raise ValueError("dg_spmm_seg_tab_f32: d_in = d_out = 64, or 64 -> 32 with weight stacks")
        live = [g for g, s in enumerate(specs) if s.n_rows > 0 and s.n_rels > 0]
        nw = max([1] + [specs[g].chunk for g in live])
        stride = 8 if nw <= 8 else 16
        blocks = []
        for g in live:
            s = specs[g]
            rpb = nw // s.chunk
            row_blocks = -(-s.n_rows // rpb)
            items = s.n_chunks * row_blocks
            n_blocks = 8 * (-(-items // 8))
            per = n_blocks >> 3
            for lb in range(n_blocks):
                item = (lb & 7) * per + (lb >> 3)
                blocks.append(None if item >= items else (g, item // row_blocks, (item % row_blocks) * rpb, rpb))
        tb = _WaveTable(specs, len(blocks) * stride, d_out != d_in)
        for b, blk in enumerate(blocks):
            if blk is None:
                continue
            g, c, r0, rpb = blk
            s = specs[g]
            for w in range(nw):
                i = b * stride + w
                slot, t = divmod(w, s.chunk)
                r = r0 + slot
                if not (slot < rpb and r < s.n_rows):
                    continue
                k = c * s.chunk + t
                if k < s.n_rels:
                    tb.relation(i, g, k, r)
                if t == 0:
                    tb.desc["orow"][i] = s.out.data_ptr() + (c * s.n_rows + r) * d_out * 4
                    tb.desc["role"][i] = s.chunk << 8
        self._tab = tb.upload(self, len(blocks), nw, stride, specs[0].x.device)
        self.n_blocks, self.nw = len(blocks), nw
        self._tfn = _lib.load().dg_spmm_seg_tab_f32

    def __call__(self, stream=None) -> None:
        check(self._tfn(ctypes.byref(self._tab), self.d_in, self.d_out, _stream_ptr(stream)), "dg_spmm_seg_tab_f32")

    def seg_form(self, stream=None) -> None:
        PreparedSeg.__call__(self, stream)


DG_MAX_GROUPS_TAB = 8


@dataclass
class ProjSpec:

    w: torch.Tensor
    out: torch.Tensor
    n_rels: int
    target: int
    rel_map: Optional[torch.Tensor] = None
    rel_map_max: Optional[int] = None


class PreparedFused:

    def __init__(self, targets, d: int, projs: Sequence[ProjSpec] = (), waves_per_group: int = 1):
        specs, tarr = [], (DgFusedTarget * len(targets))()
        max_groups = 1
        for t, (out, n_rows, gspecs, relu) in enumerate(targets):
            _dev(out, torch.float32, "out")
            if out.numel() < n_rows * d:
                raise ValueError("fused output too small")
            tarr[t].out = out.data_ptr()
            tarr[t].n_rows = n_rows
            tarr[t].g_begin = len(specs)
            tarr[t].g_count = len(gspecs)
            tarr[t].flags = _lib.DG_EPI_RELU if relu else 0
            max_groups = max(max_groups, len(gspecs))
            for s in gspecs:
                if s.n_rows != n_rows:
                    raise ValueError("group rows != target rows")
                s.validate(d, need_out=False)
                specs.append(s)
        if len(specs) > _lib.DG_MAX_GROUPS or len(targets) > _lib.DG_MAX_GROUPS:
            raise ValueError(f"at most {_lib.DG_MAX_GROUPS} groups / targets per fused launch")
        if not 1 <= waves_per_group or max_groups * waves_per_group > 16:
            raise ValueError("groups x waves_per_group must be <= 16")
        if len(projs) > _lib.DG_MAX_GROUPS:
            raise ValueError(f"at most {_lib.DG_MAX_GROUPS} projections per fused launch")
        parr = (DgProj * max(1, len(projs)))()
        for i, pj in enumerate(projs):
            _dev(pj.w, torch.float32, "proj w")
            _dev(pj.out, torch.float32, "proj out")
            K, din, dout = pj.w.shape
            n_rows = targets[pj.target][1]
            if din != d or pj.out.numel() < pj.n_rels * n_rows * dout:
                raise ValueError("projection shapes do not match the fused layer")
            if pj.rel_map is not None:
                _dev(pj.rel_map, torch.int32, "proj rel_map")
                if pj.rel_map_max is None or not 0 <= pj.rel_map_max < K:
                    raise ValueError("proj rel_map_max must index inside w")
            elif pj.n_rels > K:
# ... 594 lines not shown
        raise ValueError("paired scoring needs an even number of pairs, cols / rel of the same length")
    d = G.shape[0]
    for t, nm in ((row_table, "row_table"), (col_table, "col_table"), (G, "G")):
        _dev(t, torch.bfloat16, nm)
    if l_table is not None:
        _dev(l_table, torch.bfloat16, "l_table")
        if l_table.shape[-1] != d or l_table.stride(-1) != 1 or (l_table.dim() == 2 and l_table.stride(0) != d):
            raise ValueError("l_table must be a contiguous [n_rel, d] bf16 tensor")
    for t, nm in ((rows, "rows"), (cols, "cols")):
        _dev(t, torch.int32, nm)
    if rel is not None:
        _dev(rel, torch.int32, "rel")
    if G.shape != (d, d) or not G.is_contiguous():
        raise ValueError("G must be a contiguous d×d bf16 matrix")
    if row_table.shape[1] != d or col_table.shape[1] != d or row_table.stride(1) != 1 or col_table.stride(1) != 1:
        raise ValueError("tables must have d contiguous columns")
    if out is None:
        out = torch.empty(n, device=rows.device, dtype=torch.float32)
    if paired:
        name = "dg_decoder_score_bf16_paired"
        tabs = (row_table.data_ptr(), row_table.stride(0), row_table.shape[0], col_table.data_ptr(),
                col_table.stride(0), col_table.shape[0])
    else:
        name = "dg_decoder_score_bf16"
        tabs = (row_table.data_ptr(), row_table.stride(0), col_table.data_ptr(), col_table.stride(0))
    check(getattr(_lib.load(), name)(
        *tabs, rows.data_ptr(), cols.data_ptr(), rel.data_ptr() if rel is not None else None,
        n // 2 if paired else n, G.data_ptr(), l_table.data_ptr() if l_table is not None else None, d,
        out.data_ptr(), _stream_ptr(stream)), name)
    return out


def hinge_loss(pos: torch.Tensor, neg: torch.Tensor, margin: float,
               out: Optional[torch.Tensor] = None, stream=None,
               workspace: Optional[torch.Tensor] = None) -> torch.Tensor:
    _dev(pos, torch.float32, "pos")
    _dev(neg, torch.float32, "neg")
    if pos.numel() != neg.numel():
        raise ValueError("pos/neg length mismatch")
    if out is None:
        out = torch.empty(1, device=pos.device, dtype=torch.float32)
    if workspace is not None:
        if workspace.numel() * workspace.element_size() < _lib.DG_HINGE_WS_BYTES or not workspace.is_cuda:
            raise ValueError("hinge workspace too small")
        check(_lib.load().dg_hinge_loss_ws_f32(pos.data_ptr(), neg.data_ptr(), pos.numel(), float(margin),
                                                out.data_ptr(), workspace.data_ptr(), _stream_ptr(stream)),
              "dg_hinge_loss_ws_f32")
        return out
    check(_lib.load().dg_hinge_loss_f32(pos.data_ptr(), neg.data_ptr(), pos.numel(), float(margin),
                                         out.data_ptr(), _stream_ptr(stream)), "dg_hinge_loss_f32")
    return out


def hinge_workspace(device) -> torch.Tensor:
    return torch.zeros(_lib.DG_HINGE_WS_BYTES // 4, dtype=torch.int32, device=device)


def xent_loss(pos: torch.Tensor, neg: torch.Tensor, neg_weight: float,
              out: Optional[torch.Tensor] = None, stream=None) -> torch.Tensor:
    _dev(pos, torch.float32, "pos")
    _dev(neg, torch.float32, "neg")
    if pos.numel() != neg.numel():
        raise ValueError("pos/neg length mismatch")
    if out is None:
        out = torch.empty(1, device=pos.device, dtype=torch.float32)
    check(_lib.load().dg_xent_loss_f32(pos.data_ptr(), neg.data_ptr(), pos.numel(), float(neg_weight),
                                        out.data_ptr(), _stream_ptr(stream)), "dg_xent_loss_f32")
    return out


def unigram_sample(table: torch.Tensor, n: int, seed: int, offset: int,
                   out: Optional[torch.Tensor] = None, stream=None) -> torch.Tensor:
    _dev(table, torch.int32, "alias table")
    if table.dim() != 2 or table.shape[1] != 2:
        raise ValueError("alias table must be [range, 2]")
    if out is None:
        out = torch.empty(n, device=table.device, dtype=torch.int32)
    _dev(out, torch.int32, "out")
    if out.numel() < n:
        raise ValueError("out too small")
    check(_lib.load().dg_unigram_sample(table.data_ptr(), table.shape[0], n, seed & (2**64 - 1),
                                         offset & (2**64 - 1), out.data_ptr(), _stream_ptr(stream)),
          "dg_unigram_sample")
    return out


def unigram_sample_slots(table: torch.Tensor, slot0: int, batch: int, n: int, seed: int,
                         out: Optional[torch.Tensor] = None, stream=None) -> torch.Tensor:
    _dev(table, torch.int32, "alias table")
    if table.dim() == 3 and table.shape[2] == 2 and table.is_contiguous():
        rng, stride = table.shape[1], table.shape[1]
        if slot0 + -(-n // batch) > table.shape[0]:
            raise ValueError("slot range outside the alias tables")
    elif table.dim() == 2 and table.shape[1] == 2:
        rng, stride = table.shape[0], 0
    else:
        raise ValueError("alias tables must be [n_slots, range, 2] (contiguous) or [range, 2]")
    if out is None:
        out = torch.empty(n, device=table.device, dtype=torch.int32)
    _dev(out, torch.int32, "out")
    if out.numel() < n:
        raise ValueError("out too small")
    check(_lib.load().dg_unigram_sample_slots(table.data_ptr(), rng, stride, slot0, batch, n, seed & (2**64 - 1),
                                               out.data_ptr(), _stream_ptr(stream)), "dg_unigram_sample_slots")
    return out


def slot_score_hinge_bf16(E_row: torch.Tensor, E_col: torch.Tensor, pos_rows: torch.Tensor, pos_cols: torch.Tensor,
                          table: torch.Tensor, slot0: int, n_slots: int, batch: int, seed: int, G: torch.Tensor,
                          D: torch.Tensor, margin: float, out: torch.Tensor, neg_rows: torch.Tensor,
                          loss: torch.Tensor, workspace: torch.Tensor, stream=None) -> None:
    n = n_slots * batch
    for t, nm in ((E_row, "E_row"), (E_col, "E_col"), (G, "G"), (D, "D")):
        _dev(t, torch.bfloat16, nm)
    for t, nm in ((pos_rows, "pos_rows"), (pos_cols, "pos_cols"), (neg_rows, "neg_rows"), (table, "alias table")):
        _dev(t, torch.int32, nm)
    _dev(out, torch.float32, "out")
    _dev(loss, torch.float32, "loss")
    d = G.shape[0]
    if d != 256 or G.shape != (256, 256) or D.dim() != 2 or D.shape[1] != d or E_row.shape[1] != d \
            or E_col.shape[1] != d:
        raise ValueError("slot scorer: d = 256 tables, G and D rows")
    if table.dim() == 3 and table.shape[2] == 2:
        rng, stride = table.shape[1], table.shape[1]
        if slot0 + n_slots > table.shape[0]:
            raise ValueError("slot range outside the alias tables")
    elif table.dim() == 2 and table.shape[1] == 2:
        rng, stride = table.shape[0], 0
    else:
        raise ValueError("alias tables must be [n_slots, range, 2] or [range, 2]")
    if rng > E_row.shape[0] or slot0 + n_slots > D.shape[0]:
        raise ValueError("sampler range exceeds the row table, or slots exceed D")
    if pos_rows.numel() < n or pos_cols.numel() < n or neg_rows.numel() < n or out.numel() < 2 * n:
        raise ValueError("pairs / outputs shorter than n_slots·batch")
    if workspace.numel() * workspace.element_size() < _lib.DG_HINGE_WS_BYTES or not workspace.is_cuda:
        raise ValueError("hinge workspace too small")
    check(_lib.load().dg_slot_score_hinge_bf16(
        E_row.data_ptr(), E_row.stride(0), E_row.shape[0], E_col.data_ptr(), E_col.stride(0), E_col.shape[0],
        pos_rows.data_ptr(), pos_cols.data_ptr(),
        table.data_ptr(), rng, stride, slot0, n_slots, batch, seed & (2**64 - 1), G.data_ptr(), D.data_ptr(), d,
        float(margin), out.data_ptr(), neg_rows.data_ptr(), loss.data_ptr(), workspace.data_ptr(),
        _stream_ptr(stream)), "dg_slot_score_hinge_bf16")


def upload_alias(degrees, device) -> torch.Tensor:
    from .sampling import alias_table

    if isinstance(degrees, (list, tuple)) or (isinstance(degrees, np.ndarray) and degrees.ndim == 2):
        tabs = np.stack([alias_table(d) for d in degrees])
        return torch.from_numpy(tabs.view(np.int32)).to(device)
    return torch.from_numpy(alias_table(degrees).view(np.int32)).to(device)


class PreparedDecoderHinge:

    def __init__(self, row_table: torch.Tensor, col_table: torch.Tensor, rows: torch.Tensor,
                 cols: torch.Tensor, G: torch.Tensor, l: Optional[torch.Tensor], margin: float,
                 alias: Optional[torch.Tensor] = None, neg_rows: Optional[torch.Tensor] = None,
                 seed: int = 0, offset: int = 0):
        for t, nm, dt in ((row_table, "row_table", torch.float32), (col_table, "col_table", torch.float32),
                          (rows, "rows", torch.int32), (cols, "cols", torch.int32), (G, "G", torch.float32)):
            _dev(t, dt, nm)
        d = G.shape[0]
        n = rows.numel()
        if n < 1:
            raise ValueError("empty batch")
        if G.shape != (d, d) or row_table.shape[1] != d or col_table.shape[1] != d or cols.numel() != n:
            raise ValueError("decoder_hinge: shape mismatch")
        if l is not None:
            _dev(l, torch.float32, "l")
        if neg_rows is None:
            if alias is None:
                raise ValueError("need either negatives or a sampler alias table")
            _dev(alias, torch.int32, "alias")
            if alias.shape[0] > row_table.shape[0]:
                raise ValueError("sampler range exceeds the row table")
        else:
            _dev(neg_rows, torch.int32, "neg_rows")
        dev = G.device
        self.pos = torch.empty(n, device=dev)
        self.neg = torch.empty(n, device=dev)
        self.neg_rows = torch.empty(n, device=dev, dtype=torch.int32)
        self.loss = torch.empty(1, device=dev)
        self._ws = torch.zeros(4 + -(-n // 32), device=dev)
        self._keep = (row_table, col_table, rows, cols, G, l, alias, neg_rows)
        self.seed, self.offset = seed, offset
        self._args = [row_table.data_ptr(), row_table.shape[1], col_table.data_ptr(), col_table.shape[1],
                      rows.data_ptr(), cols.data_ptr(), neg_rows.data_ptr() if neg_rows is not None else None,
                      alias.data_ptr() if alias is not None else None, alias.shape[0] if alias is not None else 0,
                      seed, offset, n, G.data_ptr(), l.data_ptr() if l is not None else None, d, float(margin),
                      self.pos.data_ptr(), self.neg.data_ptr(), self.neg_rows.data_ptr(), self.loss.data_ptr(),
                      self._ws.data_ptr()]
        self._fn = _lib.load().dg_decoder_hinge_f32

    def __call__(self, stream=None) -> None:
        a = list(self._args)
        a[9], a[10] = self.seed & (2**64 - 1), self.offset & (2**64 - 1)
        check(self._fn(*a, _stream_ptr(stream)), "dg_decoder_hinge_f32")


class PreparedDecoderGrad:

    def __init__(self, row_table, col_table, rows, cols, neg_rows, pos, neg, G, l, margin: float,
                 dG: Optional[torch.Tensor] = None, dl: Optional[torch.Tensor] = None,
                 dG_diag: Optional[torch.Tensor] = None):
        for t, nm, dt in ((row_table, "row_table", torch.float32), (col_table, "col_table", torch.float32),
                          (rows, "rows", torch.int32), (cols, "cols", torch.int32),
                          (neg_rows, "neg_rows", torch.int32), (pos, "pos", torch.float32),
                          (neg, "neg", torch.float32), (G, "G", torch.float32)):
            _dev(t, dt, nm)
        d = G.shape[0]
        n = rows.numel()
        if G.shape != (d, d) or row_table.shape[1] != d or col_table.shape[1] != d:
            raise ValueError("decoder_grad: shape mismatch")
        if cols.numel() != n or neg_rows.numel() != n or pos.numel() != n or neg.numel() != n:
            raise ValueError("decoder_grad: batch sizes differ")
        if l is not None:
            _dev(l, torch.float32, "l")
        if dl is not None and l is None:
            raise ValueError("dl needs a diagonal L")
        for t, nm, sz in ((dG, "dG", d * d), (dl, "dl", d), (dG_diag, "dG_diag", d)):
            if t is not None:
                _dev(t, torch.float32, nm)
                if t.numel() != sz:
                    raise ValueError(f"{nm} must have {sz} elements")
        dev = G.device
        self.grad_rows = torch.empty((2 * n, d), device=dev)
        self.grad_cols = torch.empty((n, d), device=dev)
        lib = _lib.load()
        nbytes = int(lib.dg_decoder_grad_workspace(n, d))
        self._ws = torch.empty(max(1, nbytes // 4), device=dev)
        self.row_idx = torch.empty(2 * n, device=dev, dtype=torch.int32)
        self._rows, self._negs = rows, neg_rows
        self._keep = (row_table, col_table, rows, cols, neg_rows, pos, neg, G, l, dG, dl, dG_diag)
        ptr = lambda t: t.data_ptr() if t is not None else None
        self._args = [row_table.data_ptr(), row_table.shape[1], col_table.data_ptr(), col_table.shape[1],
                      rows.data_ptr(), cols.data_ptr(), neg_rows.data_ptr(), n, pos.data_ptr(), neg.data_ptr(),
                      G.data_ptr(), ptr(l), d, float(margin), self.grad_rows.data_ptr(),
                      self.grad_cols.data_ptr(), ptr(dG), ptr(dl), ptr(dG_diag), self._ws.data_ptr(), nbytes]
        self._fn = lib.dg_decoder_grad_f32

    def __call__(self, stream=None) -> None:
        check(self._fn(*self._args, _stream_ptr(stream)), "dg_decoder_grad_f32")
        n = self._rows.numel()
        self.row_idx[:n].copy_(self._rows)
        self.row_idx[n:].copy_(self._negs)


def scatter_rows(idx: torch.Tensor, src: torch.Tensor, out: torch.Tensor, stream=None) -> None:
    _dev(idx, torch.int32, "idx")
    _dev(src, torch.float32, "src")
    _dev(out, torch.float32, "out")
    n = idx.numel()
    if src.dim() != 2 or src.shape[0] != n or out.dim() != 2 or out.shape[1] != src.shape[1]:
        raise ValueError("scatter_rows: shapes")
    check(_lib.load().dg_scatter_rows_f32(idx.data_ptr(), n, src.data_ptr(), src.shape[1], out.data_ptr(),
                                          out.stride(0), out.shape[0], _stream_ptr(stream)), "dg_scatter_rows_f32")


class PreparedL2Grad:

    def __init__(self, groups: Sequence[Tuple[torch.Tensor, torch.Tensor]], dy: torch.Tensor,
                 mask: Optional[torch.Tensor], n_rows: int, d: int):
        if not 1 <= len(groups) <= _lib.DG_MAX_GROUPS:
            raise ValueError("1..DG_MAX_GROUPS groups")
        for t, nm in [(dy, "dy")] + ([(mask, "mask")] if mask is not None else []):
            _dev(t, torch.float32, nm)
            if t.numel() < n_rows * d:
                raise ValueError(f"{nm} too small")
        arr = (DgL2gGroup * len(groups))()
        for i, (s_, ds) in enumerate(groups):
            _dev(s_, torch.float32, "s")
            _dev(ds, torch.float32, "ds")
            if s_.numel() < n_rows * d or ds.numel() < n_rows * d:
                raise ValueError("l2 grad group too small")
            arr[i].s, arr[i].ds = s_.data_ptr(), ds.data_ptr()
        self._arr, self._n = arr, len(groups)
        self._keep = (list(groups), dy, mask)
        self._args = (dy.data_ptr(), mask.data_ptr() if mask is not None else None, n_rows, d)
        self._fn = _lib.load().dg_l2norm_grad_f32

    def __call__(self, stream=None) -> None:
        check(self._fn(self._arr, self._n, *self._args, _stream_ptr(stream)), "dg_l2norm_grad_f32")


class PreparedAdam:

    def __init__(self, segs: Sequence[Tuple[torch.Tensor, Optional[torch.Tensor], torch.Tensor, torch.Tensor]]):
        self._arrs = []
        for s0 in range(0, len(segs), _lib.DG_MAX_ADAM_SEGS):
            chunk = segs[s0:s0 + _lib.DG_MAX_ADAM_SEGS]
            arr = (DgAdamSeg * len(chunk))()
            for i, (p, g, m, v) in enumerate(chunk):
                for t, nm in ((p, "param"), (m, "m"), (v, "v")) + (((g, "grad"),) if g is not None else ()):
                    _dev(t, torch.float32, nm)
                    if t.numel() != p.numel():
                        raise ValueError(f"adam {nm}: {t.numel()} elements, param has {p.numel()}")
                arr[i].param, arr[i].m, arr[i].v = p.data_ptr(), m.data_ptr(), v.data_ptr()
                arr[i].grad = g.data_ptr() if g is not None else None
                arr[i].n = p.numel()
            self._arrs.append((arr, len(chunk)))
        self._keep = list(segs)
        self._fn = _lib.load().dg_adam_f32

    def __call__(self, alpha: float, beta1: float, beta2: float, eps: float,
                 state: Optional[torch.Tensor] = None, stream=None) -> None:
        sp = None
        if state is not None:
            _dev(state, torch.float32, "adam state")
            sp = state.data_ptr()
        for arr, n in self._arrs:
            check(self._fn(arr, n, alpha, beta1, beta2, eps, sp, _stream_ptr(stream)), "dg_adam_f32")


def adam_advance(state: torch.Tensor, lr: float, beta1: float, beta2: float, stream=None) -> None:
    _dev(state, torch.float32, "adam state")
    check(_lib.load().dg_adam_advance(state.data_ptr(), lr, beta1, beta2, _stream_ptr(stream)), "dg_adam_advance")


def _drop_state(state: torch.Tensor) -> None:
    if not (isinstance(state, torch.Tensor) and state.is_cuda and state.dtype == torch.int64
            and state.numel() >= 2):
        raise ValueError("dropout state must be an int64 device tensor {seed, step}")


def dropout_rows(inp: torch.Tensor, out: torch.Tensor, state: torch.Tensor, tag: int, keep: float,
                 stream=None) -> None:
    _dev(inp, torch.float32, "in")
    _dev(out, torch.float32, "out")
    _drop_state(state)
    d = inp.shape[-1]
    n = inp.numel() // d
    if out.numel() != inp.numel():
        raise ValueError("dropout_rows: shapes")
    check(_lib.load().dg_dropout_rows_f32(inp.data_ptr(), out.data_ptr(), n, d, state.data_ptr(), tag, keep,
                                          _stream_ptr(stream)), "dg_dropout_rows_f32")


def dropout_elems(src: torch.Tensor, out: torch.Tensor, state: torch.Tensor, tag: int, keep: float,
                  stream=None) -> None:
    _dev(src, torch.float32, "src")
    _dev(out, torch.float32, "out")
    _drop_state(state)
    K, n, d = out.shape
    if tuple(src.shape) != (n, d):
        raise ValueError("dropout_elems: shapes")
    check(_lib.load().dg_dropout_elems_f32(src.data_ptr(), out.data_ptr(), K, n, d, state.data_ptr(), tag, keep,
                                           _stream_ptr(stream)), "dg_dropout_elems_f32")


def _map_max(rel_map: torch.Tensor, rel_map_max: Optional[int]) -> int:
# ... 48 lines not shown
```

decagon_amd/optimizer.py:

```python
from __future__ import annotations

from typing import Dict, List, Optional

import numpy as np
import torch

from . import kernels, runtime, train
from .flags import FLAGS
from .graph import InvalidArgumentError, Node, Operation, RunContext


class _Sampler:

    def __init__(self, degrees_list, device):
        self.tables = [kernels.upload_alias(deg, device) for deg in degrees_list]
        self.counter = 0


class DecagonOptimizer:
    def __init__(self, embeddings, latent_inters, latent_varies, degrees, edge_types,
                 edge_type2dim, placeholders, margin=0.1, neg_sample_weights=1., batch_size=100):
        self.embeddings = embeddings
        self.latent_inters = latent_inters
        self.latent_varies = latent_varies
        self.edge_types = edge_types
        self.degrees = degrees
        self.edge_type2dim = edge_type2dim
        self.obj_type2n = {i: self.edge_type2dim[i, j][0][0] for i, j in self.edge_types}
        self.margin = margin
        self.neg_sample_weights = neg_sample_weights
        self.batch_size = batch_size
        self.seed = 0

        self.placeholders = placeholders
        self.inputs = placeholders["batch"]
        self.batch_edge_type_idx = placeholders["batch_edge_type_idx"]
        self.batch_row_edge_type = placeholders["batch_row_edge_type"]
        self.batch_col_edge_type = placeholders["batch_col_edge_type"]

        self._rel_degrees = []
        self._rel_of = []
        for i, j in self.edge_types:
            for k in range(self.edge_types[i, j]):
                self._rel_of.append((i, j, k))
                self._rel_degrees.append(self.degrees[i][k])

        self.row_inputs = Node("optimizer/row_inputs", lambda ctx: self._batch(ctx)[:, 0])
        self.col_inputs = Node("optimizer/col_inputs", lambda ctx: self._batch(ctx)[:, 1])
        obj_type_n = [self.obj_type2n[i] for i in range(len(self.embeddings))]
        self.obj_type_lookup_start = np.cumsum([0] + obj_type_n[:-1])
        self.obj_type_lookup_end = np.cumsum(obj_type_n)

        self._decode = Node("optimizer/decode", self._decode_fn)
        self.neg_samples = Node("optimizer/neg_samples", lambda ctx: ctx.value(self._decode)[3])
        self.outputs = Node("optimizer/outputs", lambda ctx: ctx.value(self._decode)[0])
        self.neg_outputs = Node("optimizer/neg_outputs", lambda ctx: ctx.value(self._decode)[1])
        self.preds = Node("optimizer/preds", lambda ctx: self._full(ctx, self.row_inputs))
        self.neg_preds = Node("optimizer/neg_preds", lambda ctx: self._full(ctx, self.neg_samples))
        self.predict()
        self._build()

    def _batch(self, ctx: RunContext) -> np.ndarray:
        b = np.asarray(ctx.value(self.inputs))
        if b.ndim != 2 or b.shape[1] != 2:
            raise InvalidArgumentError(f"batch must be [B, 2], got {b.shape}")
        return b.astype(np.int32, copy=False)

    def _edge(self, ctx):
        e = int(np.asarray(ctx.value(self.batch_edge_type_idx)))
        rt = int(np.asarray(ctx.value(self.batch_row_edge_type)))
        ct = int(np.asarray(ctx.value(self.batch_col_edge_type)))
        if not 0 <= e < len(self._rel_of):
            raise InvalidArgumentError(f"batch_edge_type_idx {e} out of range")
        return e, rt, ct

    def _idx_dev(self, ctx, node: Node, n_max: int) -> torch.Tensor:
        v = ctx.value(node)
        if isinstance(v, torch.Tensor):
            t = v.to(device=ctx.session.device, dtype=torch.int32)
            if t.numel():
                lo, hi = int(t.min()), int(t.max())
                if lo < 0 or hi >= n_max:
                    raise InvalidArgumentError(f"{node.name}: index out of range [0, {n_max})")
            return t.contiguous()
        a = np.asarray(v).astype(np.int64).reshape(-1)
        if a.size and (a.min() < 0 or a.max() >= n_max):
            raise InvalidArgumentError(f"{node.name}: index out of range [0, {n_max})")
        return torch.from_numpy(a.astype(np.int32)).to(ctx.session.device)

    def _tables(self, ctx, rt, ct):
        row = runtime.as_device_f32(ctx.value(self.embeddings[rt]))
        col = runtime.as_device_f32(ctx.value(self.embeddings[ct]))
        return row, col

    def _latent(self, ctx, e):
        gi, gv = self.latent_inters[e], self.latent_varies[e]
        if hasattr(gi, "kind") and hasattr(gv, "kind"):
            return runtime.latent_operands(ctx, gi.kind, gi.var, gv.kind, gv.var, gi.d, gi, gv)
        G = runtime.as_device_f32(ctx.value(gi))
        L = runtime.as_device_f32(ctx.value(gv))
        return kernels.matmul(kernels.matmul(L, G), L), None

    def _sampler(self, ctx) -> _Sampler:
        key = ("sampler", id(self))
        cache = ctx.session.caches
        if key not in cache:
            cache[key] = _Sampler(self._rel_degrees, ctx.session.device)
        return cache[key]

    def _decode_fn(self, ctx: RunContext):
        e, rt, ct = self._edge(ctx)
        row_t, col_t = self._tables(ctx, rt, ct)
        rows = self._idx_dev(ctx, self.row_inputs, row_t.shape[0])
        cols = self._idx_dev(ctx, self.col_inputs, col_t.shape[0])
        G, l = self._latent(ctx, e)
        if ctx.is_fed(self.neg_samples):
            negs = self._idx_dev(ctx, self.neg_samples, row_t.shape[0])
            if negs.numel() != rows.numel():
                raise InvalidArgumentError("neg_samples must have one entry per batch edge")
            op = kernels.PreparedDecoderHinge(row_t, col_t, rows, cols, G, l, self.margin, neg_rows=negs)
        else:
            s = self._sampler(ctx)
            if s.tables[e].shape[0] > row_t.shape[0]:
                raise InvalidArgumentError("degrees list longer than the row embedding table")
            op = kernels.PreparedDecoderHinge(row_t, col_t, rows, cols, G, l, self.margin, alias=s.tables[e],
                                              seed=self.seed, offset=s.counter)
            s.counter += rows.numel()
        op()
        return op.pos, op.neg, op.loss[0], op.neg_rows

    def _scores(self, ctx: RunContext, rows_node: Node) -> torch.Tensor:
        e, rt, ct = self._edge(ctx)
        row_t, col_t = self._tables(ctx, rt, ct)
        rows = self._idx_dev(ctx, rows_node, row_t.shape[0])
        cols = self._idx_dev(ctx, self.col_inputs, col_t.shape[0])
        if rows.numel() != cols.numel():
            raise InvalidArgumentError("row / column index counts differ")
        G, l = self._latent(ctx, e)
        return kernels.decoder_score(row_t, col_t, rows, cols, G, l)

    def _full(self, ctx: RunContext, rows_node: Node) -> torch.Tensor:
        e, rt, ct = self._edge(ctx)
        row_t, col_t = self._tables(ctx, rt, ct)
        rows = self._idx_dev(ctx, rows_node, row_t.shape[0]).long()
        cols = self._idx_dev(ctx, self.col_inputs, col_t.shape[0]).long()
        G, l = self._latent(ctx, e)
        return runtime.full_scores(row_t.index_select(0, rows).contiguous(),
                                   col_t.index_select(0, cols).contiguous(), G, l)

    def batch_predict(self, row_inputs, col_inputs):
        return Node("optimizer/batch_predict", lambda ctx: self._full(ctx, row_inputs))

    def predict(self):
        def fn(ctx):
            e, rt, ct = self._edge(ctx)
            row_t, col_t = self._tables(ctx, rt, ct)
            G, l = self._latent(ctx, e)
            return runtime.full_scores(row_t, col_t, G, l)
        self.predictions = Node("optimizer/predictions", fn)

    def _build(self):
        self.cost = self._hinge_loss(self.outputs, self.neg_outputs)
        self.optimizer = "adam"
        self.opt_op = Operation("optimizer/opt_op", lambda ctx: self._train(ctx, apply=True), training=True)
        self.grads_vars = Node("optimizer/grads_vars", lambda ctx: self._train(ctx, apply=False))
        self.grads_vars.training = True

    def _model(self):
        for e in self.embeddings:
            m = getattr(e, "model", None)
            if m is not None:
                return m
        raise NotImplementedError("opt_op needs the embeddings of a DecagonModel")

    def _train_plan(self, ctx: RunContext, model):
        fwd = model._forward(ctx)
        plans = fwd.__dict__.setdefault("_train_plans", {})
        if id(self) not in plans:
            feats = {j: runtime.feature_csr(ctx, model.inputs[j]) if j in model.inputs else None
                     for j in fwd.g.n_nodes}
            w1, w2 = model.weight_stacks()
            before = torch.cuda.memory_allocated(ctx.session.device)
            plans[id(self)] = train.TrainPlan(fwd, w1, w2, feats)
            ref = getattr(fwd, "cache_ref", None)
            if ref is not None:
                ref[0].add_bytes(ref[1], torch.cuda.memory_allocated(ctx.session.device) - before)
        return fwd, plans[id(self)]

    def _decoder_grads(self, ctx: RunContext, model, e: int, rt: int, ct: int):
        key = ("dec_grads", id(self))
        cache = ctx.session.caches
        if key not in cache:
            cache[key] = {et: torch.zeros_like(d.flat) for et, d in model.edge_type2decoder.items()}
        grads = cache[key]
        for t in grads.values():
            t.zero_()
        i, j, k = self._rel_of[e]
        dec = model.edge_type2decoder[i, j]
        gflat = grads[i, j]

        def gview(var):
            off = (var.tensor.data_ptr() - dec.flat.data_ptr()) // 4
            return gflat[off:off + var.tensor.numel()]

        gk, gv, lk, lv = model._latent_spec[e]
        fed = ctx.is_fed(self.latent_inters[e]) or ctx.is_fed(self.latent_varies[e])
        out = {"dG": None, "dl": None, "dG_diag": None}
        if not fed:
            if gk == "dense":
                out["dG"] = gview(gv)
            elif gk == "diag":
                out["dG_diag"] = gview(gv)
            if lk == "diag":
                out["dl"] = gview(lv)
        return grads, out

    def _train(self, ctx: RunContext, apply: bool):
        if not ctx.training:
            raise RuntimeError("training ops must be fetched through Session.run")
        for nd in (self.outputs, self.neg_outputs, self.cost):
            if ctx.is_fed(nd):
                raise InvalidArgumentError(f"{nd.name} is fed: the cost's gradient does not reach the model")
        model = self._model()
        fwd, tp = self._train_plan(ctx, model)
        pos, neg, _, negs_dev = ctx.value(self._decode)
        e, rt, ct = self._edge(ctx)
        row_t, col_t = self._tables(ctx, rt, ct)
        rows = self._idx_dev(ctx, self.row_inputs, row_t.shape[0])
        cols = self._idx_dev(ctx, self.col_inputs, col_t.shape[0])
        negs = (self._idx_dev(ctx, self.neg_samples, row_t.shape[0]) if ctx.is_fed(self.neg_samples)
                else negs_dev)
        G, l = self._latent(ctx, e)
        dec_grads, outs = self._decoder_grads(ctx, model, e, rt, ct)
        if outs["dl"] is not None and l is None:
            raise RuntimeError("DEDICOM decoder without its diagonal")
        op = kernels.PreparedDecoderGrad(row_t, col_t, rows, cols, negs, pos, neg, G, l, self.margin, **outs)

        def decoder_grad(dE):
            op()
            kernels.scatter_rows(op.row_idx, op.grad_rows, dE[rt])
            kernels.scatter_rows(cols, op.grad_cols, dE[ct])

        tp.backward(decoder_grad)
        w1, w2 = model.weight_stacks()
        ets = list(model.edge_types)
        pairs = tp.adam_pairs(w1, w2)
        params = [p for p, _ in pairs] + [model.edge_type2decoder[et].flat for et in ets]
        grads = [g for _, g in pairs] + [dec_grads[et] for et in ets]
        if not apply:
            gW1, gW2 = tp.full_grads()
            return self._grads_vars(model, gW1, gW2, dec_grads)
        key = ("adam", id(self))
        cache = ctx.session.caches
        if key not in cache:
            cache[key] = train.AdamState(params, lr=float(FLAGS.learning_rate))
        st = cache[key]
        prep = getattr(tp, "adam_prepared", None)
        if prep is None or prep[0] is not st:
            tp.adam_prepared = prep = (st, st.prepared(grads))
        st.apply(prep[1])
        return None

    def _grads_vars(self, model, gW1, gW2, dec_grads):
        out = []
        for et, lay in model.layers1.items():
            for k in range(lay.num_types):
                out.append((gW1[et][k], lay.vars["weights_%d" % k].tensor))
        for et, lay in model.layers2.items():
            for k in range(lay.num_types):
                out.append((gW2[et][k], lay.vars["weights_%d" % k].tensor))
        for et, dec in model.edge_type2decoder.items():
            for var in dec.vars.values():
                off = (var.tensor.data_ptr() - dec.flat.data_ptr()) // 4
                out.append((dec_grads[et][off:off + var.tensor.numel()].view(var.tensor.shape).clone(),
                            var.tensor.clone()))
        return [(g.clone(), v.clone()) for g, v in out]

    def _hinge_loss(self, aff, neg_aff):
        def fn(ctx):
# ... 25 lines not shown
```

include/decagon_hip.h:

```cpp
#ifndef DECAGON_HIP_H
#define DECAGON_HIP_H

#include <stdint.h>

#ifdef __cplusplus
extern "C" {
#endif

#define DG_OK 0
#define DG_EINVAL (-1)
#define DG_EALIGN (-2)
#define DG_ETOOMANY (-3)

#define DG_MAX_GROUPS 8

int32_t dg_abi_version(void);

typedef struct dg_rel_group {
    const int32_t* rowptr;
    const int32_t* vcol;
    const float* val;
    const float* x;
    float* out;
    int64_t x_ld;
    int32_t n_rows;
    int32_t n_chunks;
    int32_t x_rows;
    int32_t flags;
    uint32_t drop_tag;
    float drop_keep;
    int32_t drop_stride;
    const uint64_t* drop_state;
    const int32_t* drop_index;
} dg_rel_group;

#define DG_GROUP_SHARED_PATTERN 1

#define DG_GROUP_DROPOUT 2

#define DG_GROUP_DENSE_ROWS 4

int dg_spmm_groups_f32(const dg_rel_group* groups , int32_t n_groups,
                       int32_t d, void* stream);

int dg_spmm_groups_lds_f32(const dg_rel_group* groups , int32_t n_groups, int32_t d,
                           void* stream);

int dg_spmm_csr_f32(const int32_t* rowptr, const int32_t* col, const float* val,
                    int32_t n_rows, int32_t n_cols, const float* x, int64_t ldx, float* y,
                    int64_t ldy, int32_t d, float beta, void* stream);

int dg_rownorm_l2_f32(const float* x, float* y, int32_t n_rows, int32_t d, int32_t flags, void* stream);

typedef struct dg_fused_target {
    float* out;
    int32_t n_rows;
    int32_t g_begin;
    int32_t g_count;
    int32_t flags;
} dg_fused_target;

typedef struct dg_proj {
    const float* w;
    const int32_t* rel_map;
    float* out;
    int32_t n_rels;
    int32_t target;
    int32_t d_out;
    int32_t reserved;
} dg_proj;

int dg_gcn_fused_f32(const dg_rel_group* groups , int32_t n_groups,
                     const dg_fused_target* targets , int32_t n_targets,
                     const dg_proj* projs , int32_t n_projs,
                     int32_t waves_per_group, int32_t d, void* stream);

typedef struct dg_seg_group {
    const int32_t* rowptr;
    const int32_t* seg;
    const int32_t* vcol;
    const float* val;
    const int32_t* slab;
    const float* x;
    const float* w;
    float* out;
    int64_t x_ld;
    int32_t n_rows;
    int32_t n_cols;
    int32_t n_chunks;
    int32_t chunk;
    int32_t n_rels;
    int32_t x_rows;
} dg_seg_group;

int dg_spmm_seg_f32(const dg_seg_group* groups , int32_t n_groups, int32_t d_in,
                    int32_t d_out, void* stream);

int dg_gcn_fused_seg_f32(const dg_seg_group* groups , int32_t n_groups,
                         const dg_fused_target* targets , int32_t n_targets, int32_t d_in,
                         int32_t d_out, void* stream);

typedef struct dg_tab_desc {
    const float* x;
    const float* w;
    float* orow;
    int32_t cnt;
    int32_t x_ld;
    int32_t ovf;
    uint32_t role;
    uint32_t wr;
    int32_t pad[5];
} dg_tab_desc;

typedef struct dg_wave_table {
    const int32_t* pairs;
    const int32_t* ovf;
    const dg_tab_desc* desc;
    int32_t n_blocks;
    int32_t nw;
    int32_t nw_stride;
    int32_t slot_pairs;
} dg_wave_table;

int dg_gcn_fused_tab_f32(const dg_wave_table* table , int32_t d_in, int32_t d_out, void* stream);

int dg_gcn_fused_tab_post_f32(const dg_wave_table* table , int32_t d_in, int32_t d_out, void* stream);

struct dg_peer_xchg;
int dg_gcn_fused_tab_peer_f32(const dg_wave_table* table , int32_t d_in, int32_t d_out,
                              const struct dg_peer_xchg* xchg , void* stream);

int dg_spmm_seg_tab_f32(const dg_wave_table* table , int32_t d_in, int32_t d_out, void* stream);

typedef struct dg_staged_group {
    const int32_t* pairs;
    const int32_t* jm;
    const int32_t* jmoff;
    const int32_t* slab;
    const float* x;
    float* out;
    int64_t x_ld;
    int32_t n_rows;
    int32_t n_cols;
    int32_t n_rels;
    int32_t out_chunk;
    int32_t x_rows;
    int32_t jm_len;
    const int32_t* chunk_start;
    int32_t n_chunks;
    int32_t pad;
} dg_staged_group;
#define DG_STAGED_MAX_CHUNKS 128

int dg_spmm_staged_f32(const dg_staged_group* groups , int32_t n_groups, int32_t d,
                       void* stream);

typedef struct dg_staged_proj {
    const float* h;
    const float* w;
    int64_t h_ld;
    int32_t din;
    int32_t pad;
} dg_staged_proj;

int dg_spmm_staged_proj_f32(const dg_staged_group* groups , const dg_staged_proj* projs ,
                            int32_t n_groups, int32_t d, void* stream);


int dg_staged_block(const int32_t* lrowptr, const int32_t* lcol, const float* lval, int32_t n_lanes,
                    const int32_t* rlw, int32_t n_cols, int32_t* pairs);

#define DG_EPI_L2NORM 1
#define DG_EPI_RELU 2
#define DG_EPI_CHUNK_RELU 4

typedef struct dg_epi_group {
    const float* partial;
    float* sum_out;
    int32_t n_chunks;
    int32_t group_flags;
} dg_epi_group;

int dg_gcn_epilogue_f32(const dg_epi_group* groups , int32_t n_groups,
                        float* out, int32_t n_rows, int32_t d, int32_t flags, void* stream);

#define DG_EPI_MAX_TARGETS 8
typedef struct dg_epi_target {
    const dg_epi_group* groups;
    int32_t n_groups;
    int32_t reserved0;
    float* out;
    int32_t n_rows;
    int32_t target_flags;
    int32_t reserved[2];
} dg_epi_target;

int dg_gcn_epilogue_multi_f32(const dg_epi_target* targets , int32_t n_targets,
                              int32_t d, int32_t flags, void* stream);

typedef struct dg_epi_row_desc {
    float* out;
    const float* part[4];
    int32_t off;
    int32_t plane;
    uint32_t n_chunks;
    uint32_t info;
    int32_t bytes;
    int32_t pad;
} dg_epi_row_desc;

struct dg_peer_xchg;
int dg_gcn_epilogue_tab_f32(const dg_epi_row_desc* rows, int32_t n_rows, int32_t d, int32_t flags,
                            const struct dg_peer_xchg* xchg , void* stream);

#define DG_PEER_MAX 8
#define DG_PEER_SLOTS 8
#define DG_PEER_SUB_BASE 64
#define DG_PEER_SUB_STRIDE 16
#define DG_PEER_STATE_WORDS (DG_PEER_SUB_BASE + DG_PEER_SLOTS * 8 * DG_PEER_SUB_STRIDE)
#define DG_PEER_ERROR_WORD (2 * DG_PEER_SLOTS)
#define DG_PEER_DIAG_BASE 24
#define DG_PEER_DIAG_WORDS 18
#define DG_PEER_SLOW_TICKS 10000
#define DG_IPC_HANDLE_BYTES 64
#define DG_EPI_PUSH 1

typedef struct dg_peer_xchg {
    int64_t delta[DG_PEER_MAX];
    uint32_t* flags[DG_PEER_MAX];
    uint32_t* state;
    int64_t timeout_ticks;
    int32_t rank, world;
    int32_t slot;
    int32_t loopback;
} dg_peer_xchg;

int dg_peer_alloc(int64_t bytes, int32_t kind, void** ptr );
int dg_peer_free(void* ptr);
int dg_ipc_get_handle(void* ptr, void* handle , int64_t* offset );
int dg_ipc_open(const void* handle , void** ptr );
int dg_ipc_close(void* ptr);
int dg_peer_read(const void* device, void* host , int64_t bytes);

int dg_peer_allgather(const dg_peer_xchg* xchg , const void* region, const int64_t* offsets ,
                      const int64_t* sizes , int32_t n_seg, void* stream);

int dg_gcn_epilogue_peer_f32(const dg_epi_target* targets , int32_t n_targets, int32_t d,
                             int32_t flags, const dg_peer_xchg* xchg , void* stream);

int dg_gcn_fused_seg_peer_f32(const dg_seg_group* groups , int32_t n_groups,
                              const dg_fused_target* targets , int32_t n_targets, int32_t d_in,
                              int32_t d_out, const dg_peer_xchg* xchg , void* stream);

typedef struct dg_gemm_desc {
    const float* a;
    const float* b;
    float* c;
    const float* sa;
    const float* sc;
    const int32_t* b_map;
    int64_t a_bs, a_sm, a_sk;
    int64_t b_bs, b_sk, b_sn;
    int64_t c_bs, c_sm, c_sn;
    int32_t m, n, k, batch;
    int32_t reduce;
    uint32_t drop_tag;
    const uint64_t* drop_state;
    float drop_keep;
    int32_t reserved;
} dg_gemm_desc;

int dg_gemm_f32(const dg_gemm_desc* descs , int32_t n_desc, void* stream);

int dg_gemm_tn_f32(const float* a, int64_t lda, int64_t a_bs, const float* b, int64_t ldb, int64_t b_bs,
                   float* c, int32_t rows, int32_t M, int32_t N, int32_t batch, int32_t n_split,
                   float* partial, void* stream);

int dg_decoder_score_f32(const float* row_table, int64_t ld_row, const float* col_table,
                         int64_t ld_col, const int32_t* row_idx, const int32_t* col_idx,
                         int32_t n_pairs, const float* G, const float* l, int32_t d,
                         float* out, void* stream);

int dg_decoder_score_bf16(const uint16_t* row_table, int64_t ld_row, const uint16_t* col_table,
                          int64_t ld_col, const int32_t* row_idx, const int32_t* col_idx,
                          const int32_t* rel_idx, int32_t n_pairs, const uint16_t* G,
                          const uint16_t* l_table, int32_t d, float* out, void* stream);

int dg_decoder_score_bf16_paired(const uint16_t* row_table, int64_t ld_row, int64_t n_row_table,
                                 const uint16_t* col_table, int64_t ld_col, int64_t n_col_table,
                                 const int32_t* row_idx, const int32_t* col_idx,
                                 const int32_t* rel_idx, int32_t n_half, const uint16_t* G,
                                 const uint16_t* l_table, int32_t d, float* out, void* stream);

int dg_slot_score_hinge_bf16(const uint16_t* row_table, int64_t ld_row, int64_t n_row_table,
                             const uint16_t* col_table, int64_t ld_col, int64_t n_col_table,
                             const int32_t* pos_rows, const int32_t* pos_cols,
                             const uint32_t* alias_table, int32_t range, int64_t alias_stride,
                             int32_t slot0, int32_t n_slots, int32_t batch, uint64_t seed,
                             const uint16_t* G, const uint16_t* l_table, int32_t d, float margin,
                             float* out, int32_t* neg_rows, float* loss, void* workspace, void* stream);

int dg_decoder_hinge_f32(const float* row_table, int64_t ld_row, const float* col_table,
                         int64_t ld_col, const int32_t* rows, const int32_t* cols,
                         const int32_t* neg_rows, const uint32_t* alias_table, int32_t range,
                         uint64_t seed, uint64_t offset, int32_t n, const float* G,
                         const float* l, int32_t d, float margin, float* pos, float* neg,
                         int32_t* neg_rows_out, float* loss, void* workspace, void* stream);

int dg_hinge_loss_f32(const float* pos, const float* neg, int32_t n, float margin,
                      float* loss, void* stream);

#define DG_HINGE_WS_BLOCKS 256
#define DG_HINGE_WS_BYTES (16 + 4 * DG_HINGE_WS_BLOCKS)
int dg_hinge_loss_ws_f32(const float* pos, const float* neg, int32_t n, float margin, float* loss,
                         void* workspace, void* stream);

int dg_xent_loss_f32(const float* pos, const float* neg, int32_t n, float neg_weight,
                     float* loss, void* stream);

int64_t dg_decoder_grad_workspace(int32_t n, int32_t d);
int dg_decoder_grad_f32(const float* row_table, int64_t ld_row, const float* col_table,
                        int64_t ld_col, const int32_t* rows, const int32_t* cols,
                        const int32_t* neg_rows, int32_t n, const float* pos, const float* neg,
                        const float* G, const float* l, int32_t d, float margin,
                        float* grad_rows, float* grad_cols, float* dG, float* dl, float* dG_diag,
                        void* workspace, int64_t workspace_bytes, void* stream);

int dg_scatter_rows_f32(const int32_t* idx, int32_t n, const float* src, int32_t d, float* out,
                        int64_t ld_out, int32_t n_out_rows, void* stream);

typedef struct dg_l2g_group {
    const float* s;
    float* ds;
} dg_l2g_group;

int dg_l2norm_grad_f32(const dg_l2g_group* groups , int32_t n_groups,
                       const float* dy, const float* mask, int32_t n_rows, int32_t d,
                       void* stream);

#define DG_MAX_ADAM_SEGS 32

typedef struct dg_adam_seg {
    float* param;
    const float* grad;
    float* m;
    float* v;
    int64_t n;
} dg_adam_seg;

int dg_adam_f32(const dg_adam_seg* segs , int32_t n_segs, float alpha, float beta1,
                float beta2, float eps, const float* state, void* stream);
int dg_adam_advance(float* state, float lr, float beta1, float beta2, void* stream);

int dg_dropout_rows_f32(const float* in, float* out, int64_t n_rows, int32_t d, const uint64_t* state,
                        uint32_t tag, float keep, void* stream);
int dg_dropout_elems_f32(const float* src, float* out, int32_t K, int32_t n_rows, int32_t d,
                         const uint64_t* state, uint32_t tag, float keep, void* stream);
int dg_dropout_rows_map_f32(const float* in, float* out, const int32_t* rel_map, int32_t n_map,
                            int64_t rows_per_slab, int32_t d, int32_t flags, const uint64_t* state,
                            uint32_t tag, float keep, void* stream);
int dg_dropout_elems_map_f32(const float* src, float* out, const int32_t* rel_map, int32_t K,
                             int32_t n_rows, int32_t d, const uint64_t* state, uint32_t tag, float keep,
                             void* stream);
int dg_dropout_advance(uint64_t* state, void* stream);

int64_t dg_rank_metrics_workspace(int32_t n_pos);
int dg_rank_metrics_f32(const float* pos, int32_t n_pos, const float* neg, int32_t n_neg, int32_t k,
                        double* out, void* workspace, int64_t workspace_bytes, void* stream);

#define DG_RANK_LOGIT 0
#define DG_RANK_SIGMOID64 1
#define DG_RANK_SIGMOID32 2
int64_t dg_rank_metrics_ex_workspace(int32_t n_pos, int32_t n_neg);
int dg_rank_metrics_ex_f32(const float* pos, int32_t n_pos, const float* neg, int32_t n_neg, int32_t k,
                           int32_t mode, double* out, void* workspace, int64_t workspace_bytes, void* stream);

#define DG_TOPK_MAX_K 1024
#define DG_TOPK_UPPER 1
#define DG_TOPK_NO_DIAG 2
int64_t dg_decoder_topk_workspace(int32_t n_rel, int32_t n_rows, int32_t n_cols, int32_t topk);
int dg_decoder_topk_f32(const float* row_table, int64_t ld_row, int32_t n_rows, const float* col_table,
                        int64_t ld_col, int32_t n_cols, const float* G, int64_t g_stride, const float* l,
                        int64_t l_stride, int32_t n_rel, int32_t d, int32_t topk,
                        const int32_t* excl_rowptr, const int32_t* excl_col, int32_t flags,
                        float* out_score, int32_t* out_row, int32_t* out_col, int32_t* out_count,
                        void* workspace, int64_t workspace_bytes, void* stream);

int dg_unigram_sample(const uint32_t* alias_table, int32_t range, int32_t n, uint64_t seed,
                      uint64_t offset, int32_t* out, void* stream);

int dg_unigram_sample_slots(const uint32_t* alias_table, int32_t range, int64_t alias_stride,
                            int32_t slot0, int32_t batch, int32_t n, uint64_t seed, int32_t* out,
                            void* stream);

#ifdef __cplusplus
}
#endif

#endif
```

Before: 14.98 billion edges/s.

## Pre-project decoder row operands inside the final GCN layer and add rows-hinge kernel

The last 32->32 wave-table GCN layer now also writes a decoder-projected row Q = diag(l) G diag(l) e for each output row it produces, using the freshly computed embedding held in LDS. A new hinge kernel then scores positive and negative pairs as plain 32-float dot products between Q rows and column embeddings, which removes the per-pair DEDICOM matrix work and the second gather of row embeddings. A registry links embedding tensors to the plan that produces them so the decoder can attach, and the optimizer path opts out. The cost is added per-row work and writes in the GCN kernel, plus more complex validity tracking for Q.

```diff
diff --git a/decagon_amd/_lib.py b/decagon_amd/_lib.py
--- a/decagon_amd/_lib.py
+++ b/decagon_amd/_lib.py
@@ -211,6 +211,7 @@
                                            c_void_p]),
     "dg_gcn_fused_tab_f32": (c_int32, [POINTER(DgWaveTable), c_int32, c_int32, c_void_p]),
     "dg_gcn_fused_tab_post_f32": (c_int32, [POINTER(DgWaveTable), c_int32, c_int32, c_void_p]),
+    "dg_gcn_fused_tab_dec_f32": (c_int32, [POINTER(DgWaveTable), c_int32, c_int32, c_void_p, c_void_p, c_void_p]),
     "dg_gcn_fused_tab_peer_f32": (c_int32, [POINTER(DgWaveTable), c_int32, c_int32, POINTER(DgPeerXchg), c_void_p]),
     "dg_spmm_seg_tab_f32": (c_int32, [POINTER(DgWaveTable), c_int32, c_int32, c_void_p]),
     "dg_gcn_epilogue_tab_f32": (c_int32, [c_void_p, c_int32, c_int32, c_int32, POINTER(DgPeerXchg), c_void_p]),
@@ -258,6 +259,12 @@
          c_uint64, c_uint64, c_int32, c_void_p, c_void_p, c_int32, c_float, c_void_p, c_void_p,
          c_void_p, c_void_p, c_void_p, c_void_p],
     ),
+    "dg_decoder_hinge_rows_f32": (
+        c_int32,
+        [c_void_p, c_int64, c_void_p, c_int64, c_void_p, c_void_p, c_void_p, c_void_p, c_int32,
+         c_uint64, c_uint64, c_int32, c_int32, c_float, c_void_p, c_void_p, c_void_p, c_void_p,
+         c_void_p, c_void_p],
+    ),
     "dg_decoder_score_f32": (
         c_int32,
         [c_void_p, c_int64, c_void_p, c_int64, c_void_p, c_void_p, c_int32, c_void_p, c_void_p,
diff --git a/decagon_amd/csrc/decoder.hip b/decagon_amd/csrc/decoder.hip
--- a/decagon_amd/csrc/decoder.hip
+++ b/decagon_amd/csrc/decoder.hip
@@ -159,6 +159,141 @@
     for (int k = threadIdx.x; k < (int)gridDim.x; k += 128) a.partial[k] = 0.f;
     if (threadIdx.x == 0) {
         a.loss[0] = red[0];
+        atomicExch(a.ticket, 0u);
+    }
+}
+
+struct RowsHingeArgs {
+    const float* Q;
+    const float* col_table;
+    int64_t ld_q;
+    int64_t ld_col;
+    const int32_t* rows;
+    const int32_t* cols;
+    const int32_t* neg_given;
+    const uint2* alias;
+    float* pos;
+    float* neg;
+    int32_t* neg_rows_out;
+    float* loss;
+    float* partial;
+    uint32_t* ticket;
+    unsigned long long* word;
+    uint64_t seed;
+    uint64_t offset;
+    int32_t range;
+    int32_t n;
+    float margin;
+};
+
+__device__ __forceinline__ float dot4(const float4& a, const float4& b) {
+    return fmaf(a.w, b.w, fmaf(a.z, b.z, fmaf(a.y, b.y, a.x * b.x)));
+}
+
+template <bool PACKED, int NW, int PPG>
+__global__ __launch_bounds__(64 * NW) void decoder_rows_hinge_kernel(const RowsHingeArgs a) {
+    __shared__ float wsum[NW];
+    __shared__ int last;
+    __shared__ unsigned long long total;
+    const int lane = threadIdx.x & 63;
+    const int wave = threadIdx.x >> 6;
+    const int g = lane >> 3, q = lane & 7;
+    const int b0 = (blockIdx.x * NW + wave) * (8 * PPG) + g;
+    int ridx[PPG], nidx[PPG], cidx[PPG];
+#pragma unroll
+    for (int u = 0; u < PPG; ++u) {
+        const int b = b0 + 8 * u;
+        ridx[u] = nidx[u] = cidx[u] = 0;
+        if (b < a.n) {
+            cidx[u] = a.cols[b];
+            ridx[u] = a.rows[b];
+            nidx[u] = a.neg_given ? a.neg_given[b] : unigram_draw(a.alias, a.range, a.seed, a.offset + (uint64_t)b);
+        }
+    }
+    float4 ev[PPG], qp[PPG], qn[PPG];
+#pragma unroll
+    for (int u = 0; u < PPG; ++u) {
+        ev[u] = *reinterpret_cast<const float4*>(a.col_table + (int64_t)cidx[u] * a.ld_col + 4 * q);
+        qp[u] = *reinterpret_cast<const float4*>(a.Q + (int64_t)ridx[u] * a.ld_q + 4 * q);
+        qn[u] = *reinterpret_cast<const float4*>(a.Q + (int64_t)nidx[u] * a.ld_q + 4 * q);
+    }
+    float term = 0.f;
+#pragma unroll
+    for (int u = 0; u < PPG; ++u) {
+        const int b = b0 + 8 * u;
+        float sp = dot4(qp[u], ev[u]), sn = dot4(qn[u], ev[u]);
+        sp = dg::xor_add<1>(dg::xor_add<2>(dg::xor_add<4>(sp)));
+        sn = dg::xor_add<1>(dg::xor_add<2>(dg::xor_add<4>(sn)));
+        if (b < a.n) {
+            if (q == 0) {
+                a.pos[b] = sp;
+                a.neg[b] = sn;
+                if (a.neg_rows_out) a.neg_rows_out[b] = nidx[u];
+            }
+            term += fmaxf(sn - (sp - a.margin), 0.f);
+        }
+    }
+    term = dg::xor_add<32>(dg::xor_add<16>(dg::xor_add<8>(term)));
+    if constexpr (NW > 1) {
+        if (lane == 0) wsum[wave] = term;
+        __syncthreads();
+        term = wsum[0];
+#pragma unroll
+        for (int w = 1; w < NW; ++w) {
+            float t = wsum[w];
+            asm volatile("" : "+v"(t));
+            term += t;
+        }
+    }
+    if (threadIdx.x == 0) {
+        if constexpr (PACKED) {
+            unsigned long long add = 1ull << 56;
+            if (term < 256.0f) {
+                add += static_cast<unsigned long long>(static_cast<double>(term) * 4294967296.0 + 0.5);
+            } else {
+                __hip_atomic_store(a.partial + blockIdx.x, term, __ATOMIC_RELAXED, __HIP_MEMORY_SCOPE_AGENT);
+                asm volatile("s_waitcnt vmcnt(0)" ::: "memory");
+                add += 1ull << 48;
+            }
+            const unsigned long long old =
+                __hip_atomic_fetch_add(a.word, add, __ATOMIC_RELAXED, __HIP_MEMORY_SCOPE_AGENT);
+            last = (old >> 56) == gridDim.x - 1 ? 1 : 0;
+            total = old + add;
+        } else {
+            __hip_atomic_store(a.partial + blockIdx.x, term, __ATOMIC_RELAXED, __HIP_MEMORY_SCOPE_AGENT);
+            asm volatile("s_waitcnt vmcnt(0)" ::: "memory");
+            const uint32_t t = __hip_atomic_fetch_add(a.ticket, 1u, __ATOMIC_RELAXED, __HIP_MEMORY_SCOPE_AGENT);
+            last = (t == gridDim.x - 1) ? 1 : 0;
+        }
+    }
+    __syncthreads();
+    if (!last) return;
+    if constexpr (PACKED) {
+        if (threadIdx.x == 0) {
+            double s = static_cast<double>(total & ((1ull << 48) - 1)) * (1.0 / 4294967296.0);
+            if ((total >> 48) & 0xFF) {
+                for (int k = 0; k < (int)gridDim.x; ++k) {
+                    const float v = __hip_atomic_load(a.partial + k, __ATOMIC_RELAXED, __HIP_MEMORY_SCOPE_AGENT);
+                    if (v != 0.f) {
+                        s += static_cast<double>(v);
+                        __hip_atomic_store(a.partial + k, 0.f, __ATOMIC_RELAXED, __HIP_MEMORY_SCOPE_AGENT);
+                    }
+                }
+            }
+            a.loss[0] = static_cast<float>(s);
+            __hip_atomic_store(a.word, 0ull, __ATOMIC_RELAXED, __HIP_MEMORY_SCOPE_AGENT);
+        }
+        return;
+    }
+    if (wave != 0) return;
+    float s = 0.f;
+    for (int k = lane; k < (int)gridDim.x; k += 64) {
+        s += __hip_atomic_load(a.partial + k, __ATOMIC_RELAXED, __HIP_MEMORY_SCOPE_AGENT);
+        a.partial[k] = 0.f;
+    }
+    s = dg::xor_add<32>(dg::xor_add<16>(dg::xor_add<8>(dg::xor_add<4>(dg::xor_add<2>(dg::xor_add<1>(s))))));
+    if (lane == 0) {
+        a.loss[0] = s;
         atomicExch(a.ticket, 0u);
     }
 }
@@ -357,3 +492,55 @@
                            reinterpret_cast<hipStream_t>(stream), a);
     return dg::launch_status();
 }
+
+#ifndef DG_DEC_ROWS_NW
+#define DG_DEC_ROWS_NW 2
+#endif
+#ifndef DG_DEC_ROWS_PPG
+#define DG_DEC_ROWS_PPG 1
+#endif
+static_assert(DG_DEC_ROWS_NW * DG_DEC_ROWS_PPG * 8 == DG_DEC_ROWS_PAIRS, "decagon_hip.h: pairs a workgroup");
+
+extern "C" int dg_decoder_hinge_rows_f32(const float* Q, int64_t ld_q, const float* col_table, int64_t ld_col,
+                                         const int32_t* rows, const int32_t* cols, const int32_t* neg_rows,
+                                         const uint32_t* alias_table, int32_t range, uint64_t seed,
+                                         uint64_t offset, int32_t n, int32_t d, float margin, float* pos,
+                                         float* neg, int32_t* neg_rows_out, float* loss, void* workspace,
+                                         void* stream) {
+    if (n < 1 || d != 32) return DG_EINVAL;
+    if (!Q || !col_table || !rows || !cols || !pos || !neg || !loss || !workspace) return DG_EINVAL;
+    if (!neg_rows && (!alias_table || range < 1)) return DG_EINVAL;
+    if (ld_q < d || ld_col < d) return DG_EINVAL;
+    if (!dg::aligned16(workspace) || !dg::aligned16(Q) || !dg::aligned16(col_table) || (ld_q & 3) || (ld_col & 3))
+        return DG_EALIGN;
+    const int blocks = dg::ceil_div(n, DG_DEC_ROWS_PAIRS);
+    RowsHingeArgs a{};
+    a.Q = Q;
+    a.col_table = col_table;
+    a.ld_q = ld_q;
+    a.ld_col = ld_col;
+    a.rows = rows;
+    a.cols = cols;
+    a.neg_given = neg_rows;
+    a.alias = reinterpret_cast<const uint2*>(alias_table);
+    a.pos = pos;
+    a.neg = neg;
+    a.neg_rows_out = neg_rows_out;
+    a.loss = loss;
+    a.ticket = reinterpret_cast<uint32_t*>(workspace);
+    a.word = reinterpret_cast<unsigned long long*>(workspace) + 1;
+    a.partial = reinterpret_cast<float*>(workspace) + 4;
+    a.seed = seed;
+    a.offset = offset;
+    a.range = range;
+    a.n = n;
+    a.margin = margin;
+    hipStream_t st = reinterpret_cast<hipStream_t>(stream);
+    if (blocks <= 255)
+        hipLaunchKernelGGL((decoder_rows_hinge_kernel<true, DG_DEC_ROWS_NW, DG_DEC_ROWS_PPG>), dim3(blocks),
+                           dim3(64 * DG_DEC_ROWS_NW), 0, st, a);
+    else
+        hipLaunchKernelGGL((decoder_rows_hinge_kernel<false, DG_DEC_ROWS_NW, DG_DEC_ROWS_PPG>), dim3(blocks),
+                           dim3(64 * DG_DEC_ROWS_NW), 0, st, a);
+    return dg::launch_status();
+}
diff --git a/decagon_amd/csrc/segspmm.hip b/decagon_amd/csrc/segspmm.hip
--- a/decagon_amd/csrc/segspmm.hip
+++ b/decagon_amd/csrc/segspmm.hip
@@ -524,13 +524,15 @@
     return make_float4(v.x, v.y, v.z, v.w);
 }
 
-template <bool PROJ, int NW, bool PEER, int LP = 16, bool POST = false>
+template <bool PROJ, int NW, bool PEER, int LP = 16, bool POST = false, bool DEC = false>
 __global__ __launch_bounds__(64 * NW) void gcn_tab_kernel(const uint2* __restrict__ pairs,
                                                           const dg_tab_desc* __restrict__ desc,
                                                           const uint2* __restrict__ ovf, const int S,
-                                                          const dg::PeerK P) {
+                                                          const dg::PeerK P, const float* __restrict__ decG,
+                                                          const float* __restrict__ decl) {
     static_assert(LP == 16 || (LP == 8 && !PROJ && !PEER), "gcn_tab_kernel: 32-float rows in the plain one-GPU form");
     static_assert(!POST || (LP == 16 && !PROJ && !PEER), "gcn_tab_kernel: the projecting tail follows a 64 -> 64 layer");
+    static_assert(!DEC || (LP == 8 && !POST), "gcn_tab_kernel: the decoder's row operands follow the 32 -> 32 layer");
     constexpr int DOUT4 = PROJ ? 8 : LP;
     [[maybe_unused]] constexpr int kFsForm = (PROJ || LP == 8) ? 1 : 0;
     __shared__ float4 ybuf[NW][16];
@@ -546,15 +548,29 @@
                  : "=&v"(first) : "v"(slot_lane_offset<LP>(lane, S)), "s"(pairs + wi * S) : "memory");
     asm volatile("" ::"s"(D.x), "s"(D.w), "s"(D.orow), "s"(D.cnt), "s"(D.x_ld), "s"(D.ovf), "s"(D.role), "s"(D.wr),
                  "s"(ovf));
-    if constexpr (POST) asm volatile("" ::"s"(D.pad[0]), "s"(D.pad[1]));
+    if constexpr (POST || DEC) asm volatile("" ::"s"(D.pad[0]), "s"(D.pad[1]));
 #ifdef DG_FSEG_PROF
     asm volatile("s_waitcnt vmcnt(0) lgkmcnt(0)" ::: "memory");
 #endif
     DG_FS_STAMP(1);
     if constexpr (!PROJ) DG_FS_STAMP(2);
+    const int ms = lane >> 3;
     const float4 res = tab_wave<PROJ, PROJ ? kTabUP : kTabU, LP>(D, first, ovf, ybuf[wave], S);
+    const bool djob = DEC && ((D.role >> 29) & 1u) && D.orow != nullptr;
+    float4 gv[DEC ? 4 : 1], lin, lout;
+    if constexpr (DEC) {
+        lin = lout = make_float4(1.f, 1.f, 1.f, 1.f);
+        if (djob) {
+            const float* gp = decG + 4 * ((4 * ms) * 8 + (lane & 7));
+#pragma unroll
+            for (int i = 0; i < 4; ++i) gv[i] = load4_global(gp + 4 * 8 * i);
+            if (decl != nullptr) {
+                lin = load4_global(decl + 4 * ms);
+                lout = load4_global(decl + 4 * (lane & 7));
+            }
+        }
+    }
     const bool pjob = POST && ((D.role >> 30) & 1u);
-    const int ms = lane >> 3;
     float4 wv[POST ? 8 : 1];
     if constexpr (POST) {
         if (pjob) {
@@ -598,9 +614,26 @@
             }
             reinterpret_cast<float4*>(D.orow)[lane] = tot;
             if constexpr (POST) hbuf[(D.wr >> 16) & (kFsMaxRpb - 1)][lane] = tot;
+            if constexpr (DEC) ybuf[wave][lane] = tot;
             if constexpr (PEER)
                 dg::peer_store4(P, reinterpret_cast<const float*>(reinterpret_cast<const char*>(D.orow) - D.pad[0]),
                                 (uint32_t)D.pad[1], (uint32_t)D.pad[0] + 16u * lane, tot);
+        }
+        if constexpr (DEC) {
+            if (djob) {
+                __builtin_amdgcn_wave_barrier();
+                const float4 e = ybuf[wave][ms];
+                float4 z = make_float4(0.f, 0.f, 0.f, 0.f);
+                dg::fma4(z, e.x * lin.x, gv[0]);
+                dg::fma4(z, e.y * lin.y, gv[1]);
+                dg::fma4(z, e.z * lin.z, gv[2]);
+                dg::fma4(z, e.w * lin.w, gv[3]);
+                z = dg::xor_sum4_from<8>(z);
+                if (lane < 8) {
+                    float4* qrow = reinterpret_cast<float4*>(((uint64_t)(uint32_t)D.pad[1] << 32) | (uint32_t)D.pad[0]);
+                    qrow[lane] = make_float4(z.x * lout.x, z.y * lout.y, z.z * lout.z, z.w * lout.w);
+                }
+            }
         }
     }
     if constexpr (POST) {
@@ -862,13 +895,15 @@
 
 namespace {
 int fused_tab_launch(const dg_wave_table* t, int32_t d_in, int32_t d_out, const dg_peer_xchg* xchg, bool post,
-                     void* stream) {
+                     void* stream, bool dec = false, const float* G = nullptr, const float* l = nullptr) {
     if (!t) return DG_EINVAL;
     bool proj = false;
     if (seg_shape(d_in, d_out, proj) != DG_OK) return DG_EINVAL;
     const bool narrow = !proj && d_in == 32;
     if (narrow && xchg) return DG_EINVAL;
     if (post && (xchg || proj || d_in != 64)) return DG_EINVAL;
+    if (dec && (!narrow || !G)) return DG_EINVAL;
+    if (dec && (!dg::aligned16(G) || !dg::aligned16(l))) return DG_EALIGN;
     if (t->n_blocks < 0 || t->nw < 1 || t->nw > 16 || t->nw_stride != (t->nw <= 8 ? 8 : 16)) return DG_EINVAL;
     if (t->n_blocks == 0) return xchg ? DG_EINVAL : DG_OK;
     if (!t->pairs || !t->desc || !dg::aligned16(t->pairs) || (reinterpret_cast<uintptr_t>(t->desc) & 63))
@@ -886,8 +921,11 @@
     hipStream_t st = reinterpret_cast<hipStream_t>(stream);
     dim3 grid(static_cast<unsigned>(t->n_blocks)), block(64 * t->nw);
 #define DG_TAB_LAUNCH(PR, NWV, PE, ...) \
-    hipLaunchKernelGGL((gcn_tab_kernel<PR, NWV, PE, ##__VA_ARGS__>), grid, block, 0, st, pr, t->desc, ov, S, P)
-    if (narrow) {
+    hipLaunchKernelGGL((gcn_tab_kernel<PR, NWV, PE, ##__VA_ARGS__>), grid, block, 0, st, pr, t->desc, ov, S, P, G, l)
+    if (narrow && dec) {
+        if (t->nw_stride == 8) DG_TAB_LAUNCH(false, 8, false, 8, false, true);
+        else DG_TAB_LAUNCH(false, 16, false, 8, false, true);
+    } else if (narrow) {
         if (t->nw_stride == 8) DG_TAB_LAUNCH(false, 8, false, 8); else DG_TAB_LAUNCH(false, 16, false, 8);
     } else if (post) {
         if (t->nw_stride == 8) DG_TAB_LAUNCH(false, 8, false, 16, true); else DG_TAB_LAUNCH(false, 16, false, 16, true);
@@ -915,6 +953,11 @@
 
 extern "C" int dg_gcn_fused_tab_post_f32(const dg_wave_table* t, int32_t d_in, int32_t d_out, void* stream) {
     return fused_tab_launch(t, d_in, d_out, nullptr, true, stream);
+}
+
+extern "C" int dg_gcn_fused_tab_dec_f32(const dg_wave_table* t, int32_t d_in, int32_t d_out, const float* G,
+                                        const float* l, void* stream) {
+    return fused_tab_launch(t, d_in, d_out, nullptr, false, stream, true, G, l);
 }
 
 extern "C" int dg_gcn_fused_tab_peer_f32(const dg_wave_table* t, int32_t d_in, int32_t d_out,
diff --git a/decagon_amd/engine.py b/decagon_amd/engine.py
--- a/decagon_amd/engine.py
+++ b/decagon_amd/engine.py
@@ -405,6 +405,9 @@
         self.keep_sums = keep_sums
         self.sums_mode = False
         self.launch_groups: Dict[int, List[EdgeType]] = {}
+        self.runs = 0
+        self._dec = None
+        self._dec_retired: list = []
         dev = dgraph.device
         f32 = dict(device=dev, dtype=torch.float32)
         self.edge_types = list(dgraph.edge_types)
@@ -515,6 +518,8 @@
 
         self.hidden1 = {i: out_buf(i, h1, 1) for i in self.targets}
         self.embeddings = {i: out_buf(i, h2, 2) for i in self.targets}
+        for i, e in self.embeddings.items():
+            kernels.register_row_producer(e, self, i)
 
         self.staged_proj = {et for et in self.edge_types
                             if dgraph.groups[et].staged and dgraph.groups[et].n_rels and h1 == 64
@@ -704,6 +709,7 @@
                                                          share_proj=L2_PREPROJECT_SHARE))
             elif WAVE_TABLE and self.preproj and d_in == d == 32 and _tab_groups_fit(tgts, d):
                 launches.append(kernels.PreparedFusedTab(tgts, d_in, d, balance=_tab_balance(d_in, d)))
+                self._l2_tab = (tgts, d_in, d, _tab_balance(d_in, d), list(fused_t), launches[-1])
             else:
                 launches.append(kernels.PreparedFusedSeg(tgts, d_in, d))
             self.launch_groups[id(launches[-1])] = [et for i in fused_t for et in self.targets[i]]
@@ -930,6 +936,52 @@
             self.peer.ensure_ok()
         self.run_layer1()
         self.run_layer2()
+        self.runs += 1
+
+    def attach_decoder_rows(self, node_type: int, G: torch.Tensor, l: Optional[torch.Tensor]):
+        if not knob("DG_DEC_PREPROJECT", True):
+            return None
+        tab = getattr(self, "_l2_tab", None)
+        if not self.preproj or tab is None or self.h2 != 32 or node_type not in tab[4]:
+            return None
+        if (G.dtype != torch.float32 or tuple(G.shape) != (32, 32) or not G.is_contiguous() or G.data_ptr() % 16
+                or G.device != self.embeddings[node_type].device):
+            return None
+        if l is not None and (l.dtype != torch.float32 or tuple(l.shape) != (32,) or l.data_ptr() % 16
+                              or l.device != G.device):
+            return None
+        key = (node_type, G.data_ptr(), None if l is None else l.data_ptr())
+        if self._dec is not None:
+            if self._dec["key"] != key:
+                return None
+            self._dec["users"] += 1
+            return self._dec["Q"]
+        tgts, d_in, d, balance, fused_t, plain = tab
+        E = self.embeddings[node_type]
+        Q = torch.zeros((E.shape[0], 32), dtype=torch.float32, device=E.device)
+        launch = kernels.PreparedFusedTab(tgts, d_in, d, balance=balance,
+                                          dec=kernels.TabDecSpec(fused_t.index(node_type), G, l, Q))
+        self._swap_l2(plain, launch)
+        self._dec = {"key": key, "Q": Q, "G": G, "l": l, "launch": launch, "users": 1, "runs": self.runs}
+        return Q
+
+    def release_decoder_rows(self, Q: torch.Tensor) -> None:
+        if self._dec is None or self._dec["Q"] is not Q:
+            return
+        self._dec["users"] -= 1
+        if self._dec["users"] > 0:
+            return
+        self._swap_l2(self._dec["launch"], self._l2_tab[5])
+        self._dec_retired.append(self._dec)
+        self._dec = None
+
+    def decoder_rows_valid(self, Q: torch.Tensor) -> bool:
+        return self._dec is not None and self._dec["Q"] is Q and self.runs > self._dec["runs"]
+
+    def _swap_l2(self, old, new) -> None:
+        L = self._layer2.launches
+        L[L.index(old)] = new
+        self.launch_groups[id(new)] = self.launch_groups[id(old)]
 
     def phases(self) -> List[Tuple[str, Callable[[], None]]]:
         out: List[Tuple[str, Callable[[], None]]] = []
@@ -995,6 +1047,8 @@
                     tot += 4 * pj.n_rels * (din * dout + pj.out.shape[1] * dout)
             if layer == 1:
                 tot += self._post_bytes(launch)
+            else:
+                tot += self._dec_bytes(launch)
         return tot
 
     @staticmethod
@@ -1004,6 +1058,13 @@
             K, din, dout = pj.w.shape
             tot += 4 * pj.n_rels * (din * dout + pj.out.shape[1] * dout)
         return tot
+
+    @staticmethod
+    def _dec_bytes(launch) -> int:
+        dec = getattr(launch, "dec", None)
+        if dec is None:
+            return 0
+        return 4 * (dec.G.numel() + (dec.l.numel() if dec.l is not None else 0) + dec.out.numel())
 
     def layer_bytes(self, layer: int) -> int:
         L = self._layer1 if layer == 1 else self._layer2
@@ -1029,6 +1090,9 @@
                         rows = pj.out.shape[1]
                         tot += 4 * pj.n_rels * (din * dout + rows * dout)
                 tot += self._post_bytes(f)
+        else:
+            for f in L.launches:
+                tot += self._dec_bytes(f)
         return tot
 
 
diff --git a/decagon_amd/kernels.py b/decagon_amd/kernels.py
--- a/decagon_amd/kernels.py
+++ b/decagon_amd/kernels.py
@@ -422,6 +422,35 @@
     slab: Optional[Sequence[int]] = None
 
 
+@dataclass
+class TabDecSpec:
+
+    target: int
+    G: torch.Tensor
+    l: Optional[torch.Tensor]
+    out: torch.Tensor
+
+
+DEC_ROLE_BIT = 29
+
+
+def _mark_dec_rows(desc: np.ndarray, plan, stride: int, target: int, n_rows: int, q_ptr: int) -> int:
+    done = 0
+    for b, (t, r0, rpb) in enumerate(plan):
+        if t != target:
+            continue
+        for w in range(rpb):
+            if r0 + w >= n_rows:
+                continue
+            i = b * stride + w
+            addr = q_ptr + (r0 + w) * 32 * 4
+            desc["role"][i] |= np.uint32(1 << DEC_ROLE_BIT)
+            desc["pad"][i, 0] = np.uint32(addr & 0xffffffff).astype(np.int32)
+            desc["pad"][i, 1] = np.uint32(addr >> 32).astype(np.int32)
+            done += 1
+    return done
+
+
 def _tab_geometry(waves_t: Sequence[int], balance: bool) -> Tuple[int, int, List[int]]:
     nw = max([1] + list(waves_t))
     stride = 8 if nw <= 8 else 16
@@ -454,10 +483,23 @@
 class PreparedFusedTab(PreparedFusedSeg):
 
     def __init__(self, targets, d_in: int, d_out: int, peer=None, balance: bool = False,
-                 projs: Sequence[TabProjSpec] = (), share_proj: bool = True):
+                 projs: Sequence[TabProjSpec] = (), share_proj: bool = True, dec: Optional[TabDecSpec] = None):
         super().__init__(targets, d_in, d_out, peer=peer)
         specs = self._keep[0]
         narrow = d_in == d_out == 32 and all(s.w is None for s in specs) and peer is None
+        self.dec = dec
+        if dec is not None:
+            _dev(dec.G, torch.float32, "G")
+            _dev(dec.out, torch.float32, "Q")
+            if dec.l is not None:
+                _dev(dec.l, torch.float32, "l")
+            if (not narrow or not 0 <= dec.target < len(targets) or tuple(dec.G.shape) != (32, 32)
+                    or tuple(dec.out.shape) != (targets[dec.target][1], 32) or not dec.out.is_contiguous()
+                    or not dec.G.is_contiguous() or (dec.l is not None and tuple(dec.l.shape) != (32,))
+                    or dec.G.data_ptr() % 16 or dec.out.data_ptr() % 16
+                    or (dec.l is not None and dec.l.data_ptr() % 16)):
+                raise ValueError("dg_gcn_fused_tab_dec_f32: a 32 -> 32 launch, G [32, 32], l [32] or None, "
+                                 "Q [target rows, 32], all 16-byte aligned")
         if not (_tab_shape(d_in, d_out, specs) or narrow):
             raise ValueError("dg_gcn_fused_tab_f32: d_in = d_out = 64, 64 -> 32 with weight stacks, or "
                              "d_in = d_out = 32 without an exchange")
@@ -539,9 +581,14 @@
                     tb.desc["pad"][i, 1] = np.uint32(addr >> 32).astype(np.int32)
         if not plan and peer is not None:
             raise ValueError("dg_gcn_fused_tab_peer_f32: the exchange needs at least one row a rank")
+        if dec is not None:
+            _mark_dec_rows(tb.desc, plan, stride, dec.target, targets[dec.target][1], dec.out.data_ptr())
         self._tab = tb.upload(self, len(plan), nw, stride, specs[0].x.device)
         self.n_blocks, self.nw = len(plan), nw
-        if self._xchg is not None:
+        if dec is not None:
+            self._keep = self._keep + (dec,)
+            self._tfn, self._tname = _lib.load().dg_gcn_fused_tab_dec_f32, "dg_gcn_fused_tab_dec_f32"
+        elif self._xchg is not None:
             self._tfn, self._tname = _lib.load().dg_gcn_fused_tab_peer_f32, "dg_gcn_fused_tab_peer_f32"
         elif self.projs:
             self._keep = self._keep + (self.projs,)
@@ -550,7 +597,11 @@
             self._tfn, self._tname = _lib.load().dg_gcn_fused_tab_f32, "dg_gcn_fused_tab_f32"
 
     def __call__(self, stream=None) -> None:
-        if self._xchg is not None:
+        if self.dec is not None:
+            check(self._tfn(ctypes.byref(self._tab), self.d_in, self.d_out, self.dec.G.data_ptr(),
+                            self.dec.l.data_ptr() if self.dec.l is not None else None, _stream_ptr(stream)),
+                  self._tname)
+        elif self._xchg is not None:
             check(self._tfn(ctypes.byref(self._tab), self.d_in, self.d_out, self._xchg, _stream_ptr(stream)),
                   self._tname)
         else:
@@ -1451,12 +1502,36 @@
     return torch.from_numpy(alias_table(degrees).view(np.int32)).to(device)
 
 
+_ROW_PRODUCERS: dict = {}
+
+
+def register_row_producer(tensor: torch.Tensor, plan, node_type) -> None:
+    import weakref
+
+    for k in [k for k, (ref, _) in _ROW_PRODUCERS.items() if ref() is None]:
+        del _ROW_PRODUCERS[k]
+    _ROW_PRODUCERS[tensor.data_ptr()] = (weakref.ref(plan), node_type)
+
+
+def row_producer(tensor: torch.Tensor):
+    hit = _ROW_PRODUCERS.get(tensor.data_ptr())
+    if hit is None:
+        return None
+    plan, node_type = hit[0](), hit[1]
+    if plan is None or plan.embeddings.get(node_type) is None:
+        return None
+    e = plan.embeddings[node_type]
+    if e.data_ptr() != tensor.data_ptr() or e.shape != tensor.shape or e.stride() != tensor.stride():
+        return None
+    return plan, node_type
+
+
 class PreparedDecoderHinge:
 
     def __init__(self, row_table: torch.Tensor, col_table: torch.Tensor, rows: torch.Tensor,
                  cols: torch.Tensor, G: torch.Tensor, l: Optional[torch.Tensor], margin: float,
                  alias: Optional[torch.Tensor] = None, neg_rows: Optional[torch.Tensor] = None,
-                 seed: int = 0, offset: int = 0):
+                 seed: int = 0, offset: int = 0, preproject: Optional[bool] = None):
         for t, nm, dt in ((row_table, "row_table", torch.float32), (col_table, "col_table", torch.float32),
                           (rows, "rows", torch.int32), (cols, "cols", torch.int32), (G, "G", torch.float32)):
             _dev(t, dt, nm)
@@ -1481,7 +1556,7 @@
         self.neg = torch.empty(n, device=dev)
         self.neg_rows = torch.empty(n, device=dev, dtype=torch.int32)
         self.loss = torch.empty(1, device=dev)
-        self._ws = torch.zeros(4 + -(-n // 32), device=dev)
+        self._ws = torch.zeros(4 + -(-n // 8), device=dev)
         self._keep = (row_table, col_table, rows, cols, G, l, alias, neg_rows)
         self.seed, self.offset = seed, offset
         self._args = [row_table.data_ptr(), row_table.shape[1], col_table.data_ptr(), col_table.shape[1],
@@ -1491,11 +1566,47 @@
                       self.pos.data_ptr(), self.neg.data_ptr(), self.neg_rows.data_ptr(), self.loss.data_ptr(),
                       self._ws.data_ptr()]
         self._fn = _lib.load().dg_decoder_hinge_f32
+        self.entry = "dg_decoder_hinge_f32"
+        self._plan = self.Q = None
+        if preproject is None:
+            preproject = knob("DG_DEC_PREPROJECT", True)
+        prod = row_producer(row_table) if preproject else None
+        if (prod is not None and d == 32 and 2 * n >= row_table.shape[0] and col_table.data_ptr() % 16 == 0
+                and col_table.is_contiguous()):
+            plan, node_type = prod
+            Q = plan.attach_decoder_rows(node_type, G, l)
+            if Q is not None:
+                self._plan, self.Q = plan, Q
+                self._rows_fn = _lib.load().dg_decoder_hinge_rows_f32
+                a = self._args
+                self._rows_args = [Q.data_ptr(), Q.shape[1]] + a[2:12] + [d] + a[15:]
+
+    @property
+    def attached(self) -> bool:
+        return self._plan is not None
+
+    def release(self) -> None:
+        if self._plan is not None:
+            self._plan.release_decoder_rows(self.Q)
+            self._plan = self.Q = None
+
+    def __del__(self):
+        try:
+            self.release()
+        except Exception:
+            pass
 
     def __call__(self, stream=None) -> None:
+        if self._plan is not None and self._plan.decoder_rows_valid(self.Q):
+            a = list(self._rows_args)
+            a[9], a[10] = self.seed & (2**64 - 1), self.offset & (2**64 - 1)
+            self.entry = "dg_decoder_hinge_rows_f32"
+            check(self._rows_fn(*a, _stream_ptr(stream)), self.entry)
+            return
         a = list(self._args)
         a[9], a[10] = self.seed & (2**64 - 1), self.offset & (2**64 - 1)
-        check(self._fn(*a, _stream_ptr(stream)), "dg_decoder_hinge_f32")
+        self.entry = "dg_decoder_hinge_f32"
+        check(self._fn(*a, _stream_ptr(stream)), self.entry)
 
 
 class PreparedDecoderGrad:
diff --git a/decagon_amd/optimizer.py b/decagon_amd/optimizer.py
--- a/decagon_amd/optimizer.py
+++ b/decagon_amd/optimizer.py
@@ -118,13 +118,14 @@
             negs = self._idx_dev(ctx, self.neg_samples, row_t.shape[0])
             if negs.numel() != rows.numel():
                 raise InvalidArgumentError("neg_samples must have one entry per batch edge")
-            op = kernels.PreparedDecoderHinge(row_t, col_t, rows, cols, G, l, self.margin, neg_rows=negs)
+            op = kernels.PreparedDecoderHinge(row_t, col_t, rows, cols, G, l, self.margin, neg_rows=negs,
+                                              preproject=False)
         else:
             s = self._sampler(ctx)
             if s.tables[e].shape[0] > row_t.shape[0]:
                 raise InvalidArgumentError("degrees list longer than the row embedding table")
             op = kernels.PreparedDecoderHinge(row_t, col_t, rows, cols, G, l, self.margin, alias=s.tables[e],
-                                              seed=self.seed, offset=s.counter)
+                                              seed=self.seed, offset=s.counter, preproject=False)
             s.counter += rows.numel()
         op()
         return op.pos, op.neg, op.loss[0], op.neg_rows
diff --git a/include/decagon_hip.h b/include/decagon_hip.h
--- a/include/decagon_hip.h
+++ b/include/decagon_hip.h
@@ -125,6 +125,9 @@
 int dg_gcn_fused_tab_f32(const dg_wave_table* table , int32_t d_in, int32_t d_out, void* stream);
 
 int dg_gcn_fused_tab_post_f32(const dg_wave_table* table , int32_t d_in, int32_t d_out, void* stream);
+
+int dg_gcn_fused_tab_dec_f32(const dg_wave_table* table , int32_t d_in, int32_t d_out, const float* G,
+                             const float* l, void* stream);
 
 struct dg_peer_xchg;
 int dg_gcn_fused_tab_peer_f32(const dg_wave_table* table , int32_t d_in, int32_t d_out,
@@ -307,6 +310,15 @@
                          const float* l, int32_t d, float margin, float* pos, float* neg,
                          int32_t* neg_rows_out, float* loss, void* workspace, void* stream);
 
+#ifndef DG_DEC_ROWS_PAIRS
+#define DG_DEC_ROWS_PAIRS 16
+#endif
+int dg_decoder_hinge_rows_f32(const float* Q, int64_t ld_q, const float* col_table, int64_t ld_col,
+                              const int32_t* rows, const int32_t* cols, const int32_t* neg_rows,
+                              const uint32_t* alias_table, int32_t range, uint64_t seed, uint64_t offset,
+                              int32_t n, int32_t d, float margin, float* pos, float* neg,
+                              int32_t* neg_rows_out, float* loss, void* workspace, void* stream);
+
 int dg_hinge_loss_f32(const float* pos, const float* neg, int32_t n, float margin,
                       float* loss, void* stream);
 
```

Measured after the change: 15.52 billion edges/s (median of 6 runs). +3.6%, better.
